# ChanghyeonKim93/bundle_adjustment_solver

Measured on AMD Instinct MI355X. Metric: lm_iterations_per_sec, higher is better.
Workload: dtype f64; 1 GPU; C4 stereo 6-DoF: 1000 poses / 500k landmarks / 5M obs; n_opt_poses=995, n_opt_landmarks=500000, n_observations=5000000, parallelism=single GPU, exchange=none

## Files before the change

bundle_adjustment_solver_amd/_lib.py:

```python
import ctypes as C
import os

_HERE = os.path.dirname(os.path.abspath(__file__))
LIB_PATH = os.environ.get("BA_HIP_LIB") or os.path.join(_HERE, "libba_hip.so")


class BaOptions(C.Structure):
    _fields_ = [
        ("threshold_step_size", C.c_float),
        ("threshold_cost_change", C.c_float),
        ("threshold_huber_loss", C.c_float),
        ("threshold_outlier_rejection", C.c_float),
        ("max_num_iterations", C.c_int),
        ("initial_lambda", C.c_float),
        ("decrease_ratio_lambda", C.c_float),
        ("increase_ratio_lambda", C.c_float),
        ("gauss_newton", C.c_int),
    ]


def make_options(max_iter=50, thr_step=1e-5, thr_cost=1e-5, huber=1.0,
                 outlier=2.0, lambda0=100.0, dec=0.33, inc=3.0,
                 gauss_newton=False):
    o = BaOptions()
# ... 75 lines not shown
    "ba_set_cameras": (C.c_int, [_P, C.c_int, _D, _D]),
    "ba_set_poses": (C.c_int, [_P, C.c_int, _D, _U8]),
    "ba_set_points": (C.c_int, [_P, C.c_int, _D, _U8]),
    "ba_set_observations": (C.c_int, [_P, C.c_int64, _I32, _I32, _I32, _D]),
    "ba_set_shard": (C.c_int, [_P, C.c_int, C.c_int]),
    "ba_finalize": (C.c_int, [_P]),
    "ba_update_values": (C.c_int, [_P, _D, _D]),
    "ba_set_relative": (C.c_int, [_P, C.c_int64, _I32, _I32, _D, _D]),
    "ba_update_relative": (C.c_int, [_P, _D, _D]),
    "ba_relative_check": (C.c_int, [C.c_int, _U8, C.c_int64, _I32, _I32, _D, _D]),
    "ba_relative_info": (C.c_int, [_P, _I64]),
    "ba_partition_points": (C.c_int, [C.c_int, _U8, C.c_int, _U8, C.c_int64,
                                      _I32, _I32, C.c_int, _I32]),
    "ba_set_allreduce": (C.c_int, [_P, ALLREDUCE_FN, _P]),
    "ba_reduce_buffer_size": (C.c_int64, [_P, C.c_int]),
    "ba_bind_reduce_buffer": (C.c_int, [_P, C.c_int, _P, C.c_int64]),
    "ba_gather_points": (C.c_int, [_P]),
    "ba_rccl_available": (C.c_int, []),
    "ba_rccl_get_unique_id": (C.c_int, [_U8]),
    "ba_rccl_comm_create": (C.c_int, [C.POINTER(_P), C.c_int, C.c_int, _U8, C.c_int]),
    "ba_rccl_comm_size": (C.c_int, [_P]),
    "ba_rccl_comm_calls": (C.c_int64, [_P]),
    "ba_rccl_comm_destroy": (None, [_P]),
    "ba_rccl_allreduce_hook": (C.c_int, [_P, C.c_int, _P, C.c_int64, _P]),
    "ba_stream_create": (C.c_int, [C.POINTER(_P), C.c_int, C.c_int, C.c_int64]),
    "ba_stream_destroy": (None, [_P]),
    "ba_stream_set_cameras": (C.c_int, [_P, C.c_int, _D, _D]),
    "ba_stream_set_poses": (C.c_int, [_P, C.c_int, _D, _U8]),
    "ba_stream_set_points": (C.c_int, [_P, C.c_int, _D, _U8]),
    "ba_stream_set_observations": (C.c_int, [_P, C.c_int64, _I32, _I32, _I32, _D]),
    "ba_stream_finalize": (C.c_int, [_P]),
    "ba_stream_solve": (C.c_int, [_P, C.POINTER(BaOptions), C.POINTER(BaIterInfo),
                                  C.c_int, C.POINTER(C.c_int), C.POINTER(C.c_int)]),
    "ba_stream_lm_begin": (C.c_int, [_P, C.POINTER(BaOptions)]),
    "ba_stream_lm_iterate": (C.c_int, [_P, C.c_int]),
    "ba_stream_lm_sync": (C.c_int, [_P, C.POINTER(BaIterInfo), C.c_int,
                                    C.POINTER(C.c_int), C.POINTER(C.c_int)]),
    "ba_stream_get_poses": (C.c_int, [_P, _D]),
    "ba_stream_get_points": (C.c_int, [_P, _D]),
    "ba_stream_info": (C.c_int, [_P, C.POINTER(C.c_int64)]),
    "ba_solve": (C.c_int, [_P, C.POINTER(BaOptions), C.POINTER(BaIterInfo),
                           C.c_int, C.POINTER(C.c_int), C.POINTER(C.c_int)]),
    "ba_lm_begin": (C.c_int, [_P, C.POINTER(BaOptions)]),
    "ba_lm_iterate": (C.c_int, [_P, C.c_int]),
    "ba_lm_sync": (C.c_int, [_P, C.POINTER(BaIterInfo), C.c_int,
                             C.POINTER(C.c_int), C.POINTER(C.c_int)]),
    "ba_gd_begin": (C.c_int, [_P, C.POINTER(BaOptions)]),
    "ba_gd_iterate": (C.c_int, [_P, C.c_int]),
    "ba_gd_sync": (C.c_int, [_P, C.POINTER(BaIterInfo), C.c_int,
                             C.POINTER(C.c_int), C.POINTER(C.c_int)]),
    "ba_solve_gd": (C.c_int, [_P, C.POINTER(BaOptions), C.POINTER(BaIterInfo),
                              C.c_int, C.POINTER(C.c_int), C.POINTER(C.c_int)]),
    "ba_gd_get_gradient": (C.c_int, [_P, _D, _D]),
    "ba_stage_cost": (C.c_int, [_P, _D]),
    "ba_stage_linearize": (C.c_int, [_P, C.c_double, C.c_double]),
    "ba_stage_schur": (C.c_int, [_P]),
    "ba_stage_solve_reduced": (C.c_int, [_P]),
    "ba_stage_backsub_update": (C.c_int, [_P]),
    "ba_stage_scalars": (C.c_int, [_P, _D, _D, _D, _D]),
    "ba_stage_commit": (C.c_int, [_P, C.c_int]),
    "ba_enable_stage_timing": (C.c_int, [_P, C.c_int]),
    "ba_get_stage_ms": (C.c_int, [_P, _D, C.c_int]),
    "ba_num_opt_poses": (C.c_int, [_P]),
    "ba_num_opt_points": (C.c_int, [_P]),
    "ba_num_pairs": (C.c_int64, [_P]),
    "ba_num_schur_blocks": (C.c_int64, [_P]),
    "ba_num_schur_triples": (C.c_int64, [_P]),
    "ba_get_poses": (C.c_int, [_P, _D]),
    "ba_get_points": (C.c_int, [_P, _D, _U8]),
    "ba_get_A": (C.c_int, [_P, _D, _D]),
    "ba_get_C": (C.c_int, [_P, _D, _D]),
    "ba_get_Cinv": (C.c_int, [_P, _D, _D]),
    "ba_get_pairs": (C.c_int, [_P, _I32, _I32, _D]),
    "ba_expand_pair_slim": (None, [_D, _D, _D, _D]),
    "ba_get_S": (C.c_int, [_P, _D, _D]),
    "ba_get_xy": (C.c_int, [_P, _D, _D]),
    "ba_kernel_count": (C.c_int, []),
    "ba_kernel_name": (C.c_char_p, [C.c_int]),
    "ba_get_kernel_ms": (C.c_int, [_P, _D, C.POINTER(C.c_int64), C.c_int]),
    "ba_get_dense_info": (C.c_int, [_P, _D]),
    "ba_get_schur_info": (C.c_int, [_P, C.POINTER(C.c_int64)]),
    "ba_get_lin_info": (C.c_int, [_P, C.POINTER(C.c_int64)]),
    "ba_get_pair_record_info": (C.c_int, [_P, C.POINTER(C.c_int64)]),
    "ba_get_mask_info": (C.c_int, [_P, C.POINTER(C.c_int64)]),
    "ba_get_dropped_pivots": (C.c_int, [_P, C.POINTER(C.c_int64), C.c_int]),
    "ba_dense_spd_solve": (C.c_int, [_P, C.c_int, _D, _D, _D, _D]),
    "ba_covariance": (C.c_int, [_P, C.c_double, C.c_int, _I32, _D, C.c_int, _I32, _D,
                                C.POINTER(C.c_int64)]),
    "ba_covariance_info": (C.c_int, [_P, C.POINTER(C.c_int64)]),
    "ba_covariance_check": (C.c_int, [C.c_int, C.c_int, C.c_int, C.c_int, _U8, C.c_int, _U8,
                                      C.c_int, _I32, _D, C.c_int, _I32, _D]),
    "ba_pose_only_mono6": (C.c_int, [_P, _F, _F, C.c_int, C.c_float, C.c_float,
                                     C.c_float, C.c_float, _F, _U8,
                                     C.POINTER(BaOptions), C.POINTER(BaPoIter),
                                     C.c_int, C.POINTER(C.c_int),
                                     C.POINTER(C.c_int), _F]),
    "ba_pose_only_stereo6": (C.c_int, [_P, _F, _F, _F, C.c_int, _F, _F, _F, _F,
                                       _U8, _U8, C.POINTER(BaOptions),
                                       C.POINTER(BaPoIter), C.c_int,
                                       C.POINTER(C.c_int), C.POINTER(C.c_int),
                                       _F]),
    "ba_pose_only_mono3": (C.c_int, [_P, _F, _F, C.c_int, C.c_float, C.c_float,
                                     C.c_float, C.c_float, _F, _F, _F, _U8,
                                     C.POINTER(BaOptions), C.POINTER(BaPoIter),
                                     C.c_int, C.POINTER(C.c_int),
                                     C.POINTER(C.c_int), _F]),
    "ba_pose_only_stereo3": (C.c_int, [_P, _F, _F, _F, C.c_int, _F, _F, _F, _F,
                                       _F, _F, _U8, _U8, C.POINTER(BaOptions),
                                       C.POINTER(BaPoIter), C.c_int,
                                       C.POINTER(C.c_int), C.POINTER(C.c_int),
                                       _F]),
    "ba_pose_only_mono6_batch": (C.c_int, [_P, C.c_int, _I32, _F, _F, _F, _F, _U8,
                                           C.POINTER(BaOptions), C.POINTER(BaPoIter),
                                           C.c_int, C.POINTER(BaPoResult), _F]),
    "ba_pose_only_stereo6_batch": (C.c_int, [_P, C.c_int, _I32, _F, _F, _F, _F, _F,
                                             _F, _F, _U8, _U8, C.POINTER(BaOptions),
                                             C.POINTER(BaPoIter), C.c_int,
                                             C.POINTER(BaPoResult), _F]),
    "ba_pose_only_mono6_batch_device": (C.c_int, [_P, C.c_int, _P, _P, _P, _P, _P, _P,
                                                  C.POINTER(BaOptions), _P, C.c_int,
                                                  _P, _P, _P]),
    "ba_pose_only_stereo6_batch_device": (C.c_int, [_P, C.c_int, _P, _P, _P, _P, _P, _P,
                                                    _P, _P, _P, C.POINTER(BaOptions),
                                                    _P, C.c_int, _P, _P, _P]),
    "ba_right_camera_record": (C.c_int, [_F, _F, _F]),
    "ba_pose_only_mono3_batch": (C.c_int, [_P, C.c_int, _I32, _F, _F, _F, _F, _F, _F, _U8,
                                           C.POINTER(BaOptions), C.POINTER(BaPoIter),
                                           C.c_int, C.POINTER(BaPoResult), _F]),
    "ba_pose_only_stereo3_batch": (C.c_int, [_P, C.c_int, _I32, _F, _F, _F, _F, _F, _F,
                                             _F, _F, _F, _U8, _U8, C.POINTER(BaOptions),
                                             C.POINTER(BaPoIter), C.c_int,
                                             C.POINTER(BaPoResult), _F]),
    "ba_pose_only_mono3_batch_device": (C.c_int, [_P, C.c_int, _P, _P, _P, _P, _P, _P, _P,
                                                  C.POINTER(BaOptions), _P, C.c_int,
                                                  _P, _P, _P]),
    "ba_pose_only_stereo3_batch_device": (C.c_int, [_P, C.c_int, _P, _P, _P, _P, _P, _P,
                                                    _P, _P, _P, C.POINTER(BaOptions),
                                                    _P, C.c_int, _P, _P, _P]),
    "ba_planar_record": (C.c_int, [_F, _F, _F, _F, _F, _F]),
    "ba_batch_create": (C.c_int, [C.POINTER(_P), _P, C.c_int, _I32, _I32, _I32, _I64,
                                  _D, _D, _D, _U8, _D, _U8, _I32, _I32, _I32, _D]),
    "ba_batch_destroy": (None, [_P]),
    "ba_batch_solve": (C.c_int, [_P, C.POINTER(BaOptions), C.POINTER(BaIterInfo),
                                 C.c_int, C.POINTER(BaBatchResult)]),
    "ba_batch_covariance": (C.c_int, [_P, C.c_double, _D, _D, C.POINTER(BaBatchCovResult)]),
    "ba_batch_marginalize": (C.c_int, [_P, C.c_double, _U8, _D, _D, _U8,
                                       C.POINTER(BaBatchMargResult)]),
    "ba_batch_marg_layout": (C.c_int, [_P, _U8, _I64, _I64]),
    "ba_batch_marg_plan_problem": (C.c_int, [C.c_int, _U8, _U8, C.c_int, _U8, C.c_int64,
                                             _I32, _I32, _I32, _U8]),
    "ba_batch_set_prior": (C.c_int, [_P, _I32, _I32, _D, _D, _D, _D]),
    "ba_batch_prior_check": (C.c_int, [C.c_int, _I32, _U8, _I32, _I32, _D, _D, _D, _D]),
    "ba_batch_prior_info": (C.c_int, [_P, _I64]),
    "ba_batch_set_relative": (C.c_int, [_P, _I32, _I32, _I32, _D, _D]),
    "ba_batch_relative_check": (C.c_int, [C.c_int, _I32, _U8, _I32, _I32, _I32, _D, _D]),
    "ba_batch_relative_info": (C.c_int, [_P, _I64]),
    "ba_batch_relative_marg_plan": (C.c_int, [_P, _U8, _U8]),
    "ba_batch_update_values": (C.c_int, [_P, _D, _D]),
    "ba_batch_get_poses": (C.c_int, [_P, _D]),
    "ba_batch_get_points": (C.c_int, [_P, _D]),
    "ba_batch_info": (C.c_int, [_P, _I64]),
    "ba_batch_scratch_bytes": (C.c_int, [_P, _I64]),
    "ba_batch_plan_problem": (C.c_int, [C.c_int, _U8, C.c_int, _U8, C.c_int64, _I32,
                                        _I32, _I32, _I32, _U8, _I32, _I32]),
    "ba_point_only": (C.c_int, [_P, C.c_int, _D, _D, C.c_int, _D, C.c_int, _I64, _I32, _I32,
                                _D, _U8, _D, C.POINTER(BaOptions), C.POINTER(BaIterInfo),
# ... 78 lines not shown
```

bundle_adjustment_solver_amd/csrc/ba_api.hip:

```cpp
#include <hip/hip_runtime.h>

#include <algorithm>
#include <chrono>
#include <cmath>
#include <cstdio>
#include <cstdlib>
#include <cstring>
#include <string>
#include <vector>

#include "ba_device_fn.h"
#include "ba_handle.h"
#include "ba_rel_host.h"

namespace {
thread_local std::string g_err;
}
void ba::set_last_error(const std::string &m) { g_err = m; }
int ba::fail(const std::string &m) {
  g_err = m;
  return -1;
}
using ba::fail;
using ba::Mem;
// ... 217 lines not shown
  if (h->upload(Mem::Resident, &d.cams, cams)) return -1;
  std::vector<double> poses((size_t)pl.n_pose * 12);
  for (int p = 0; p < pl.n_pose; ++p)
    std::memcpy(&poses[(size_t)p * 12], &h->pose_T[(size_t)pl.pose_user_of_int[p] * 12],
                12 * sizeof(double));
  if (h->upload(Mem::Resident, &d.poses[0], poses) || h->upload(Mem::Resident, &d.poses[1], poses)) return -1;
  std::vector<double> pts((size_t)pl.n_pt * 3);
  for (int q = 0; q < pl.n_pt; ++q)
    std::memcpy(&pts[(size_t)q * 3], &h->pt_X[(size_t)pl.pt_user_of_int[q] * 3],
                3 * sizeof(double));
  if (h->upload(Mem::ChunkState, &d.pts[0], pts) || h->upload(Mem::ChunkState, &d.pts[1], pts)) return -1;
  return 0;
}

std::vector<int32_t> make_blk_desc(const ba::Plan &pl) {
  std::vector<int32_t> bd((size_t)pl.B * 16, 0);
  for (int64_t bk = 0; bk < pl.B; ++bk) {
    int32_t *r = bd.data() + 16 * bk;
    const int64_t c0 = pl.blk_contrib_ptr[bk], c1 = pl.blk_contrib_ptr[bk + 1];
    r[0] = pl.sblk_j[bk];
    r[1] = pl.sblk_k[bk];
    r[2] = (int32_t)c0;
    r[3] = (int32_t)(c1 - c0);
    r[4] = pl.sblk_tchunk_ptr[bk];
    r[5] = pl.sblk_tchunk_ptr[bk + 1] - pl.sblk_tchunk_ptr[bk];
    for (int t = 0; t < 8; ++t) r[8 + t] = c0 + t < c1 ? pl.contrib_slot[c0 + t] : 0;
  }
  return bd;
}

std::vector<ba::DevProblem::LmChunk> make_lm_chunks(const ba::Plan &pl) {
  std::vector<ba::DevProblem::LmChunk> lc(pl.bchunk_lm.size() - 1);
  for (size_t c = 0; c < lc.size(); ++c) {
    const int l0 = pl.bchunk_lm[c], l1 = pl.bchunk_lm[c + 1];
    lc[c].pb = pl.lm_pair_ptr[l0];
    lc[c].ob = pl.lm_obs_ptr[l0];
    lc[c].l0 = l0;
    lc[c].nl = l1 - l0;
    lc[c].np = (int32_t)(pl.lm_pair_ptr[l1] - pl.lm_pair_ptr[l0]);
    lc[c].no = (int32_t)(pl.lm_obs_ptr[l1] - pl.lm_obs_ptr[l0]);
  }
  return lc;
}

int upload_observation_lists(ba_handle *h) {
  const ba::Plan &pl = h->plan;
  ba::DevProblem &d = h->d;
  static_assert(sizeof(int4) == 16 && sizeof(double2) == 16 && sizeof(int2) == 8, "layout");
  if (h->upload(Mem::ChunkConst, &d.obs_idx, pl.obs_idx.data(), (size_t)pl.n_obs) ||
      h->upload(Mem::ChunkConst, &d.obs_uv, pl.obs_uv.data(), (size_t)pl.n_obs))
    return -1;
  if (!pl.obs_cp.empty() && pl.n_obs > 0 && !h->knobs.run.cost_wide)
    if (h->upload(Mem::ChunkConst, &d.obs_cp, pl.obs_cp.data(), (size_t)pl.n_obs)) return -1;
  if (h->upload(Mem::ChunkConst, &d.pobs_idx, pl.pobs_idx.data(), (size_t)pl.n_pobs) ||
      h->upload(Mem::ChunkConst, &d.pobs_uv, pl.pobs_uv.data(), (size_t)pl.n_pobs) ||
      h->upload(Mem::ChunkConst, &d.lm_obs_ptr, pl.lm_obs_ptr) ||
      h->upload(Mem::ChunkConst, &d.lm_pair_ptr, pl.lm_pair_ptr) ||
      h->upload(Mem::ChunkConst, &d.pair_pose, pl.pair_pose) || h->upload(Mem::ChunkConst, &d.pair_lm, pl.pair_lm) ||
      h->upload(Mem::ChunkConst, &d.achunk_pose, pl.achunk_pose) ||
      h->upload(Mem::ChunkConst, &d.achunk_begin, pl.achunk_begin) ||
      h->upload(Mem::ChunkConst, &d.achunk_end, pl.achunk_end) ||
      h->upload(Mem::ChunkConst, &d.pose_achunk_ptr, pl.pose_achunk_ptr))
    return -1;
  if (h->upload(Mem::Resident, &d.sblk_j, pl.sblk_j) || h->upload(Mem::Resident, &d.diag_blk, pl.diag_blk) ||
      h->upload(Mem::Resident, &d.sblk_k, pl.sblk_k))
    return -1;
  if (pl.contrib_slot.size() >= (size_t)INT32_MAX) return fail("too many slot contributions for int32 indices");
  if (h->upload(Mem::ChunkConst, &d.tri_p, pl.tri_p) || h->upload(Mem::ChunkConst, &d.tri_q, pl.tri_q) ||
      h->upload(Mem::ChunkConst, &d.tchunk_blk, pl.tchunk_blk) ||
      h->upload(Mem::ChunkConst, &d.tchunk_begin, pl.tchunk_begin) ||
      h->upload(Mem::ChunkConst, &d.tchunk_end, pl.tchunk_end) ||
      h->upload(Mem::ChunkConst, &d.sblk_tchunk_ptr, pl.sblk_tchunk_ptr) ||
      h->upload(Mem::ChunkConst, &d.ltri, pl.ltri) || h->upload(Mem::ChunkConst, &d.chunk_sp, pl.chunk_sp) ||
      h->upload(Mem::ChunkConst, &d.sup_lane, pl.sup_lane) ||
      h->upload(Mem::ChunkConst, &d.blk_contrib_ptr, pl.blk_contrib_ptr) ||
      h->upload(Mem::ChunkConst, &d.contrib_slot, pl.contrib_slot) ||
      h->upload(Mem::ChunkConst, &d.blk_desc, make_blk_desc(pl)) ||
      h->upload(Mem::ChunkConst, &d.bchunk_lm, pl.bchunk_lm) ||
      h->upload(Mem::ChunkConst, &d.lm_chunk, make_lm_chunks(pl)))
    return -1;
  return 0;
}

int upload_descriptors_and_groups(ba_handle *h) {
  const ba::Plan &pl = h->plan;
  ba::DevProblem &d = h->d;
  d.n_sup = (int)pl.sup_desc.size();
  d.n_bchunk = (int)pl.bchunk_lm.size() - 1;
  d.n_slot = (int)pl.slot_blk.size();
  static_assert(sizeof(ba::Plan::SupDesc) == sizeof(ba::DevProblem::SupDesc), "desc layout");
  static_assert(sizeof(ba::Plan::ChunkDesc) == sizeof(ba::DevProblem::ChunkDesc), "desc layout");
  static_assert(sizeof(ba::Plan::GrpDesc) == sizeof(ba::DevProblem::GrpDesc) && sizeof(ba::Plan::GrpDesc) == 128,
                "group descriptor layout");
  static_assert(sizeof(ba::Plan::LinDesc) == sizeof(ba::DevProblem::LinDesc) && sizeof(ba::Plan::LinDesc) == 48,
                "group linearisation descriptor layout");
  d.n_grp32 = (int)pl.grp32.size();
  d.n_grp64 = (int)pl.grp64.size();
  d.n_grp128 = (int)pl.grp128.size();
  d.lin_chunk0 = pl.lin_groups ? pl.n_bchunk_grp : 0;
  d.n_lin_desc = (int)pl.lin_desc.size();
  d.n_lin_plain = pl.n_lin_plain;
  d.n_bs_grp = d.n_lin_desc;
  d.n_lm_part = d.n_bs_grp + (d.n_bchunk - d.lin_chunk0 + ba::kBsChunks - 1) / ba::kBsChunks;
  d.n_lin_cost = d.n_bchunk + d.n_lin_desc;
  d.pair_slim = h->knobs.layout.pair_slim && pl.lin_groups && d.n_lin_desc > 0 ? 1 : 0;
  d.P_slim = d.pair_slim ? pl.lm_pair_ptr[pl.M_grp] : 0;
  if (h->upload(Mem::ChunkConst, &d.sup_desc, pl.sup_desc.data(), pl.sup_desc.size()) ||
      h->upload(Mem::ChunkConst, &d.chunk_desc, pl.chunk_desc.data(), pl.chunk_desc.size()) ||
      h->dalloc(Mem::ChunkState, &d.spart2, (size_t)d.n_slot * ba::kSlotStride) ||
      h->upload(Mem::ChunkConst, &d.grp32, pl.grp32.data(), pl.grp32.size()) ||
      h->upload(Mem::ChunkConst, &d.grp64, pl.grp64.data(), pl.grp64.size()) ||
      h->upload(Mem::ChunkConst, &d.grp128, pl.grp128.data(), pl.grp128.size()) ||
      h->upload(Mem::ChunkConst, &d.lin_desc, pl.lin_desc.data(), pl.lin_desc.size()) ||
      h->upload(Mem::ChunkConst, &d.grp_pat, pl.grp_pat.data(), pl.grp_pat.size() / 2) ||
      h->upload(Mem::ChunkConst, &d.pose_gpart_ptr, pl.pose_gpart_ptr) ||
      h->upload(Mem::ChunkConst, &d.pose_gpart, pl.pose_gpart) ||
      h->dalloc(Mem::ChunkState, &d.Apart2, (size_t)pl.n_apart2 * 27) ||
      h->dalloc(Mem::ChunkState, &d.lin_dump, (size_t)ba::kLinDump))
    return -1;
  if (pl.n_apart2 > 0) HIP_TRY(hipMemset(d.Apart2, 0, (size_t)pl.n_apart2 * 27 * sizeof(double)));
  return 0;
}

int alloc_iteration_storage(ba_handle *h) {
  const ba::Plan &pl = h->plan;
  ba::DevProblem &d = h->d;
  for (int k = 0; k < 2; ++k) {
    if (h->dalloc(Mem::ChunkState, &d.Cu[k], (size_t)pl.M * 6) || h->dalloc(Mem::ChunkState, &d.b[k], (size_t)pl.M * 3) ||
        h->dalloc(Mem::ChunkState, &d.W[k], std::max<size_t>(2, (size_t)pl.P * ba::kWStride)) ||
        h->dalloc(Mem::Resident, &d.A[k], (size_t)pl.N * 36) || h->dalloc(Mem::Resident, &d.a[k], (size_t)pl.N * 6))
      return -1;
    HIP_TRY(hipMemset(d.W[k], 0, std::max<size_t>(1, (size_t)pl.P * ba::kWStride) * sizeof(double)));
    HIP_TRY(hipMemset(d.A[k], 0, std::max<size_t>(1, (size_t)pl.N * 36) * sizeof(double)));
    HIP_TRY(hipMemset(d.a[k], 0, std::max<size_t>(1, (size_t)pl.N * 6) * sizeof(double)));
  }
  d.n_obs_lm = pl.M > 0 ? pl.lm_obs_ptr[pl.M] : 0;
  if (h->dalloc(Mem::ChunkState, &d.Cd, (size_t)pl.M * 6) || h->dalloc(Mem::ChunkState, &d.Cinv, (size_t)pl.M * 6) ||
      h->dalloc(Mem::ChunkState, &d.lin_cost_part, (size_t)std::max(1, d.n_lin_cost)) ||
      h->dalloc(Mem::ChunkState, &d.Apart, (size_t)d.n_achunk * 27) ||
      h->dalloc(Mem::ChunkState, &d.spart, (size_t)d.n_tchunk * ba::kSlotStride) ||
      h->dalloc(Mem::ChunkState, &d.y, (size_t)pl.M * 3) ||
      h->dalloc(Mem::ChunkState, &d.lm_part, (size_t)std::max(1, d.n_lm_part) * 2))
    return -1;
  d.log_cap = 4096;
  if (h->dalloc(Mem::Resident, &d.x, (size_t)pl.N * 6 + 64) ||
      h->dalloc(Mem::Resident, &d.cost_part, (size_t)ba::kCostGrid) ||
      h->dalloc(Mem::Resident, &d.pose_part, (size_t)2 + 2 * ba::kPoseGrid) ||
      h->dalloc(Mem::Resident, &d.scal, (size_t)4) || h->dalloc(Mem::Resident, &d.ctrl, (size_t)1) ||
      h->dalloc(Mem::Resident, &d.log, (size_t)d.log_cap))
    return -1;
  HIP_TRY(hipMemset(d.lin_cost_part, 0, (size_t)std::max(1, d.n_lin_cost) * sizeof(double)));
  HIP_TRY(hipMemset(d.x, 0, ((size_t)pl.N * 6 + 64) * sizeof(double)));
  HIP_TRY(hipMemset(d.y, 0, std::max<size_t>(1, (size_t)pl.M * 3) * sizeof(double)));
  HIP_TRY(hipMemset(d.cost_part, 0, ba::kCostGrid * sizeof(double)));
  HIP_TRY(hipMemset(d.lm_part, 0, (size_t)std::max(1, d.n_lm_part) * 2 * sizeof(double)));
  HIP_TRY(hipMemset(d.pose_part, 0, (2 + 2 * ba::kPoseGrid) * sizeof(double)));
  HIP_TRY(hipMemset(d.scal, 0, 4 * sizeof(double)));
  return 0;
}

int alias_dense_owner(ba_handle *h) {
  const ba_handle *o = h->dense_owner;
  ba::DevProblem &d = h->d;
  if (!o->finalized || o->plan.N != h->plan.N || o->plan.B != h->plan.B)
    return fail("ba_finalize: the dense owner belongs to a different problem");
  h->sched = o->sched;
  h->ddev = o->ddev;
  h->pose_col_h = o->pose_col_h;
  d.nb = o->d.nb; d.npad = o->d.npad; d.ld = o->d.ld;
  d.L = o->d.L; d.Ldiag = o->d.Ldiag; d.pose_col = o->d.pose_col; d.col_x = o->d.col_x;
  d.zt_I = o->d.zt_I; d.zt_J = o->d.zt_J; d.n_zt = o->d.n_zt;
  d.x = o->d.x;
  return 0;
}

int build_dense_system(ba_handle *h) {
  const ba::Plan &pl = h->plan;
  ba::DevProblem &d = h->d;
  const ba::DenseKnobs &knobs = h->knobs.dense;
  ba::DenseSchedule cand[2];
  const int orders[2] = {32, 64};
  for (int k = 0; k < 2; ++k) {
    int ncb_k = 0;
    std::vector<uint8_t> adj;
    ba::tile_pattern(pl, ba::dense_poses_per_tile(orders[k]), ncb_k, adj);
    if (knobs.full) std::fill(adj.begin(), adj.end(), 1);
    ba::build_dense_schedule(ncb_k, adj, knobs.natural, orders[k], cand[k], knobs.order);
  }
  const bool stats = h->knobs.plan.stats;
// ... 885 lines not shown
  if (download(buf, h->d.pts[h->hc.cur], (size_t)h->plan.n_pt * 3, h->stream)) return -1;
  if (owned_mask) std::memset(owned_mask, 0, (size_t)h->plan.n_pt_global);
  for (int q = 0; q < h->plan.n_pt; ++q) {
    const int u = h->plan.pt_user_of_int[q];
    std::memcpy(X3 + (size_t)u * 3, &buf[(size_t)q * 3], 3 * sizeof(double));
    if (owned_mask) owned_mask[u] = 1;
  }
  return 0;
}

int ba_get_A(ba_handle *h, double *A36, double *a6) {
  if (!h || !h->finalized) return fail("ba_get_A: not finalized");
  if (use_device(h)) return -1;
  join_side(h);
  if (pull_ctrl(h)) return -1;
  const int lb = h->hc.lcur;
  if (A36) {
    HIP_TRY(hipMemcpy(A36, h->d.A[lb], (size_t)h->plan.N * 36 * sizeof(double), hipMemcpyDeviceToHost));
    const double lp1 = 1.0 + h->hc.lambda;
    for (int j = 0; j < h->plan.N; ++j)
      for (int r = 0; r < 6; ++r) A36[(size_t)j * 36 + r * 7] *= lp1;
  }
  if (a6) HIP_TRY(hipMemcpy(a6, h->d.a[lb], (size_t)h->plan.N * 6 * sizeof(double), hipMemcpyDeviceToHost));
  return 0;
}

static void expand_sym3(const double *s6, double *f9) {
  f9[0] = s6[0]; f9[1] = s6[1]; f9[2] = s6[2];
  f9[3] = s6[1]; f9[4] = s6[3]; f9[5] = s6[4];
  f9[6] = s6[2]; f9[7] = s6[4]; f9[8] = s6[5];
}

static int get_sym_vec(ba_handle *h, const double *dS6, const double *dV3,
                       double *out9, double *out3) {
  const ba::Plan &pl = h->plan;
  std::vector<double> s6, v3;
  if (download(s6, dS6, (size_t)pl.M * 6, h->stream)) return -1;
  if (download(v3, dV3, (size_t)pl.M * 3, h->stream)) return -1;
  for (int i = 0; i < pl.M; ++i) {
    const int g = pl.iopt_of_user[pl.pt_user_of_int[i]];
    if (out9) expand_sym3(&s6[(size_t)i * 6], out9 + (size_t)g * 9);
    if (out3) std::memcpy(out3 + (size_t)g * 3, &v3[(size_t)i * 3], 3 * sizeof(double));
  }
  return 0;
}

int ba_get_C(ba_handle *h, double *C9, double *b3) {
  if (!h || !h->finalized) return fail("ba_get_C: not finalized");
  if (use_device(h)) return -1;
  join_side(h);
  if (pull_ctrl(h)) return -1;
  ba::launch_damp_invert_export(h->d, h->stream);
  return get_sym_vec(h, h->d.Cd, h->d.b[h->hc.lcur], C9, b3);
}

int ba_get_Cinv(ba_handle *h, double *Cinv9, double *Cinvb3) {
  if (!h || !h->finalized) return fail("ba_get_Cinv: not finalized");
  if (use_device(h)) return -1;
  const ba::Plan &pl = h->plan;
  std::vector<double> s6, b3;
  join_side(h);
  if (pull_ctrl(h)) return -1;
  ba::launch_damp_invert_export(h->d, h->stream);
  if (download(s6, h->d.Cinv, (size_t)pl.M * 6, h->stream)) return -1;
  if (download(b3, h->d.b[h->hc.lcur], (size_t)pl.M * 3, h->stream)) return -1;
  for (int i = 0; i < pl.M; ++i) {
    const int g = pl.iopt_of_user[pl.pt_user_of_int[i]];
    const double *ci = &s6[(size_t)i * 6], *b = &b3[(size_t)i * 3];
    if (Cinv9) expand_sym3(ci, Cinv9 + (size_t)g * 9);
    if (Cinvb3) {
      double *o = Cinvb3 + (size_t)g * 3;
      o[0] = ci[0] * b[0] + ci[1] * b[1] + ci[2] * b[2];
      o[1] = ci[1] * b[0] + ci[3] * b[1] + ci[4] * b[2];
      o[2] = ci[2] * b[0] + ci[4] * b[1] + ci[5] * b[2];
    }
  }
  return 0;
}

void ba_expand_pair_slim(const double *rec8, const double *T12, const double *X3, double *k12) {
  ba::pair_from_G(rec8, rec8[6], T12, X3[0], X3[1], X3[2], k12, k12 + 9);
}

int ba_get_pairs(ba_handle *h, int32_t *pair_i, int32_t *pair_j, double *W18) {
  if (!h || !h->finalized) return fail("ba_get_pairs: not finalized");
  if (use_device(h)) return -1;
  const ba::Plan &pl = h->plan;
  auto padded = [&](int64_t p) { return !pl.pair_pad.empty() && pl.pair_pad[p]; };
  {
    int64_t o = 0;
    for (int64_t p = 0; p < pl.P; ++p) {
      if (padded(p)) continue;
      if (pair_i) pair_i[o] = pl.iopt_of_user[pl.pt_user_of_int[pl.pair_lm[p]]];
      if (pair_j) pair_j[o] = pl.pair_pose[p];
      ++o;
    }
  }
  if (W18) {
    if (pull_ctrl(h)) return -1;
    std::vector<double> w12((size_t)pl.P * ba::kWStride);
    if (pl.P > 0)
      HIP_TRY(hipMemcpy(w12.data(), h->d.W[h->hc.lcur], w12.size() * sizeof(double), hipMemcpyDeviceToHost));
    const int64_t P_slim = h->d.P_slim;
    std::vector<double> Th, Xh;
    if (P_slim > 0) {
      Th.resize((size_t)pl.n_pose * 12);
      Xh.resize((size_t)pl.M * 3);
      HIP_TRY(hipMemcpy(Th.data(), h->d.poses[h->hc.cur], Th.size() * sizeof(double), hipMemcpyDeviceToHost));
      HIP_TRY(hipMemcpy(Xh.data(), h->d.pts[h->hc.cur], Xh.size() * sizeof(double), hipMemcpyDeviceToHost));
    }
    int64_t o = 0;
    for (int64_t p = 0; p < pl.P; ++p) {
      if (padded(p)) continue;
      double k12[12];
      const double *k = &w12[(size_t)p * ba::kWStride];
      if (p < P_slim) {
        ba_expand_pair_slim(&w12[(size_t)p * ba::kWSlim], &Th[(size_t)pl.pair_pose[p] * 12], &Xh[(size_t)pl.pair_lm[p] * 3], k12);
        k = k12;
      }
      double *W = W18 + (size_t)o * 18;
      for (int e = 0; e < 9; ++e) W[e] = k[e];
      for (int c = 0; c < 3; ++c) {
        W[9 + c] = k[10] * k[6 + c] - k[11] * k[3 + c];
        W[12 + c] = k[11] * k[c] - k[9] * k[6 + c];
        W[15 + c] = k[9] * k[3 + c] - k[10] * k[c];
      }
      ++o;
    }
  }
  return 0;
}

int ba_get_S(ba_handle *h, double *S, double *rhs) {
  if (!h || !h->finalized) return fail("ba_get_S: not finalized");
  if (use_device(h)) return -1;
  const ba::DevProblem &d = h->d;
  const int n6 = 6 * h->plan.N;
  std::vector<double> L;
  ba::launch_scatter(d, h->stream);
  if (download(L, d.L, (size_t)d.npad * d.ld, h->stream)) return -1;
  auto colof = [&](int e) { return h->pose_col_h[e / 6] + e % 6; };
  for (int c = 0; c < n6; ++c) {
    for (int r = c; r < n6; ++r) {
      int rr = colof(r), cc = colof(c);
      if (rr < cc) std::swap(rr, cc);
      const double v = L[(size_t)cc * d.ld + rr];
      if (S) {
        S[(size_t)r * n6 + c] = v;
        S[(size_t)c * n6 + r] = v;
      }
    }
    if (rhs) rhs[c] = L[(size_t)colof(c) * d.ld + d.npad];
  }
  return 0;
}

int ba_get_xy(ba_handle *h, double *x6, double *y3) {
  if (!h || !h->finalized) return fail("ba_get_xy: not finalized");
  if (use_device(h)) return -1;
  const ba::Plan &pl = h->plan;
  HIP_TRY(hipStreamSynchronize(h->stream));
  if (x6 && pl.N > 0)
    HIP_TRY(hipMemcpy(x6, h->d.x, (size_t)pl.N * 6 * sizeof(double), hipMemcpyDeviceToHost));
  if (y3) {
    std::vector<double> y;
    if (download(y, h->d.y, (size_t)pl.M * 3, h->stream)) return -1;
    for (int i = 0; i < pl.M; ++i) {
      const int g = pl.iopt_of_user[pl.pt_user_of_int[i]];
      std::memcpy(y3 + (size_t)g * 3, &y[(size_t)i * 3], 3 * sizeof(double));
    }
  }
  return 0;
}

int ba_kernel_count(void) { return ba::K_COUNT; }

const char *ba_kernel_name(int id) {
  static const char *names[ba::K_COUNT] = {
      "k_cost", "k_lin_landmarks", "k_lin_poses", "k_pose_finalize", "k_dense_init",
      "k_schur_lds", "k_schur_partial", "k_schur_final", "k_scatter",
      "k_chol_diag", "k_chol_trsm", "k_chol_update", "k_chol_back", "k_chol_diag_trsm", "k_chol_tail", "k_backsub_update",
      "k_pose_update", "k_scalars", "k_control", "k_damp_invert", "k_schur_grp", "k_lin_grp",
      "k_rel_lin", "k_rel_gather", "k_rel_offdiag",
// ... 194 lines not shown
  out4[0] = bw;
  out4[1] = ba::kCovGroupCols;
  out4[2] = (int64_t)h->d.npad * bw * (int64_t)sizeof(double);
  out4[3] = h->cov_batches;
  return 0;
}

int ba_covariance(ba_handle *h, double huber, int n_pose_sel, const int32_t *pose_sel, double *cov_pose36,
                  int n_pt_sel, const int32_t *pt_sel, double *cov_pt9, int64_t *dropped_pivots) {
  if (!h) return fail("ba_covariance: null handle");
  if (ba_covariance_check(h->finalized, h->world > 1 || h->ar_fn != nullptr,
                          h->arena != nullptr || h->dense_owner != nullptr, h->n_pose,
                          h->pose_fixed.data(), h->n_pt, h->pt_fixed.data(), n_pose_sel, pose_sel,
                          cov_pose36, n_pt_sel, pt_sel, cov_pt9))
    return -1;
  if (use_device(h)) return -1;
  const ba::Plan &pl = h->plan;
  const ba::DevProblem &d = h->d;
  const ba::DenseSchedule &sc = h->sched;
  const int nb = d.nb, ncb = sc.ncb;
  struct Item {
    int t0, key, idx;
  };
  auto distinct = [](std::vector<Item> &v) {
    std::sort(v.begin(), v.end(), [](const Item &a, const Item &b) {
      return a.t0 != b.t0 ? a.t0 < b.t0 : a.key != b.key ? a.key < b.key : a.idx < b.idx;
    });
    v.erase(std::unique(v.begin(), v.end(), [](const Item &a, const Item &b) { return a.idx == b.idx; }), v.end());
  };
  std::vector<Item> poses, pts;
  for (int s = 0; s < n_pose_sel; ++s) {
    const int j = pl.jopt_of_user[pose_sel[s]];
    poses.push_back({h->pose_col_h[j] / nb, h->pose_col_h[j], j});
  }
  for (int s = 0; s < n_pt_sel; ++s) {
    const int i = pl.pt_int_of_user[pt_sel[s]];
    if (i < 0 || i >= pl.M) return fail("ba_covariance: pt_sel[" + std::to_string(s) + "] is not an optimisable point of this handle");
    int t0 = ncb;
    for (int64_t p = pl.lm_pair_ptr[i]; p < pl.lm_pair_ptr[i + 1]; ++p)
      t0 = std::min(t0, h->pose_col_h[pl.pair_pose[p]] / nb);
    pts.push_back({t0, i, i});
  }
  distinct(poses);
  distinct(pts);
  std::vector<int> slot_pose(pl.N, -1), slot_pt(pl.M, -1);
  std::vector<ba::CovGroup> groups;
  auto make_groups = [&](const std::vector<Item> &v, int kind, int per, std::vector<int> &slot) {
    for (size_t k = 0; k < v.size(); k += per) {
      ba::CovGroup g{};
      g.kind = kind;
      g.n = (int)std::min<size_t>(per, v.size() - k);
      g.t0 = v[k].t0;
      for (int a = 0; a < g.n; ++a) {
        g.item[a] = v[k + a].idx;
        g.slot[a] = slot[v[k + a].idx] = (int)(k + a);
      }
      groups.push_back(g);
    }
  };
  make_groups(poses, 0, 2, slot_pose);
  make_groups(pts, 1, 5, slot_pt);
  std::vector<int> trow_ptr((size_t)ncb + 1, 0), trow;
  {
    std::vector<std::vector<int>> by_row((size_t)ncb);
    for (int p = 0; p < ncb; ++p)
      for (int a = sc.row_ptr[p]; a < sc.row_ptr[p + 1]; ++a)
        if (sc.rows[a] < ncb) by_row[sc.rows[a]].push_back(p);
    for (int t = 0; t < ncb; ++t) {
      trow.insert(trow.end(), by_row[t].begin(), by_row[t].end());
      trow_ptr[t + 1] = (int)trow.size();
    }
  }
  join_side(h);
  if (pull_ctrl(h)) return -1;
  const ba::DevCtrl keep = h->hc;
  h->hc.done = 0;
  h->hc.lambda = 0.0;
  h->hc.huber = huber;
  if (push_ctrl(h)) return -1;
  int bad_keep = 0, bad_now = 0;
  HIP_TRY(hipMemcpy(&bad_keep, h->ddev.bad_pivots, sizeof(int), hipMemcpyDeviceToHost));
  HIP_TRY(hipMemsetAsync(h->ddev.bad_pivots, 0, sizeof(int), h->stream));
  enqueue_linearize(h, 0);
  if (h->rel.F > 0) {
    ba::launch_rel_lin(d, h->rel, 0, 1, h->stream);
    ba::launch_rel_gather(d, h->rel, 0, 1, h->stream);
  }
  ba::launch_damp_invert_export(d, h->stream);
  ba::launch_schur(d, false, true, h->stream);
  if (h->rel.F > 0) ba::launch_rel_offdiag(d, h->rel, false, h->stream);
  ba::launch_scatter(d, h->stream);
  {
    const ba::DenseDev &dd = h->ddev;
    ba::dense_factor_solve(d.L, d.npad, d.ld, d.Ldiag, d.x, &d.ctrl->done, sc, dd,
                           ba::dense_launch_plan_no_tail(sc, h->knobs.dense, dd.flow_ok, dd.plan[1], h->knobs.cone.want), h->stream);
  }
  HIP_TRY(hipStreamSynchronize(h->stream));
  HIP_TRY(hipMemcpy(&bad_now, h->ddev.bad_pivots, sizeof(int), hipMemcpyDeviceToHost));
  HIP_TRY(hipMemcpy(h->ddev.bad_pivots, &bad_keep, sizeof(int), hipMemcpyHostToDevice));
  h->hc = keep;
  if (push_ctrl(h)) return -1;
  ba::ScratchAllocs scratch(h);
  const int bw_max = cov_batch_cols(d.npad, h->knobs.run);
  const int gpb = bw_max / ba::kCovGroupCols;
  const int bw = (int)std::min<size_t>(gpb, std::max<size_t>(1, groups.size())) * ba::kCovGroupCols;
  int *d_trow_ptr = nullptr, *d_trow = nullptr;
  ba::CovGroup *d_groups = nullptr;
  double *Zw = nullptr, *d_pose = nullptr, *d_pt = nullptr;
  if (h->upload(Mem::Resident, &d_trow_ptr, trow_ptr) || h->upload(Mem::Resident, &d_trow, trow) ||
      h->upload(Mem::Resident, &d_groups, groups) ||
      h->dalloc(Mem::Resident, &Zw, (size_t)d.npad * bw) || h->dalloc(Mem::Resident, &d_pose, poses.size() * 36) ||
      h->dalloc(Mem::Resident, &d_pt, pts.size() * 9))
    return -1;
  h->cov_batches = 0;
  for (size_t g0 = 0; g0 < groups.size(); g0 += gpb) {
    const int ng = (int)std::min<size_t>(gpb, groups.size() - g0);
    ba::launch_cov_batch(d, keep.lcur, keep.cur, ncb, d_trow_ptr, d_trow, d_groups + g0, ng, Zw, bw, d_pose, d_pt, h->stream);
    ++h->cov_batches;
  }
  std::vector<double> hp, hq;
  if (download(hp, d_pose, poses.size() * 36, h->stream) || download(hq, d_pt, pts.size() * 9, h->stream)) return -1;
  HIP_TRY(hipStreamSynchronize(h->stream));
  HIP_TRY(hipGetLastError());
  if (bad_now >= ba::kFlowTimeout) return fail("ba_covariance: a dataflow hand-off of the factorisation timed out");
  for (int s = 0; s < n_pose_sel; ++s)
    std::memcpy(cov_pose36 + (size_t)s * 36, &hp[(size_t)slot_pose[pl.jopt_of_user[pose_sel[s]]] * 36], 36 * sizeof(double));
  for (int s = 0; s < n_pt_sel; ++s)
    std::memcpy(cov_pt9 + (size_t)s * 9, &hq[(size_t)slot_pt[pl.pt_int_of_user[pt_sel[s]]] * 9], 9 * sizeof(double));
  if (dropped_pivots) *dropped_pivots = bad_now;
  return 0;
}

}

namespace {
struct PoLayout {
  size_t X, uv, uvr, camr, T, mask, maskr, gsw, h2d_end, meta, iters, dbg, end;
};
PoLayout po_layout(int n, int icap, bool stereo) {
  auto al = [](size_t v) { return (v + 15) & ~(size_t)15; };
  PoLayout L;
  size_t o = 0;
  L.X = o;      o = al(o + (size_t)n * 3 * sizeof(float));
  L.uv = o;     o = al(o + (size_t)n * 2 * sizeof(float));
  L.uvr = o;    o = al(o + (stereo ? (size_t)n * 2 * sizeof(float) : 0));
  L.camr = o;   o = al(o + 16 * sizeof(float));
  L.T = o;      o = al(o + 12 * sizeof(float));
  L.mask = o;   o = al(o + (size_t)n);
  L.maskr = o;  o = al(o + (stereo ? (size_t)n : 0));
  L.gsw = o;    o = al(o + sizeof(int) * (size_t)ba::pose_only_sync_ints());
  L.h2d_end = o;
  L.meta = o;   o = al(o + 4 * sizeof(int));
  L.iters = o;  o = al(o + (size_t)icap * sizeof(ba::PoIter));
  L.dbg = o;    o = al(o + (size_t)icap * 12 * sizeof(float));
  L.end = o;
  return L;
}

int po_reserve(ba_handle *h, size_t bytes) {
  if (bytes <= h->po_cap) return 0;
  if (h->po_dev) (void)hipFree(h->po_dev);
  if (h->po_host) (void)hipHostFree(h->po_host);
  h->po_dev = h->po_host = nullptr;
  h->po_cap = 0;
  HIP_TRY(hipMalloc((void **)&h->po_dev, bytes));
  HIP_TRY(hipHostMalloc((void **)&h->po_host, bytes, hipHostMallocDefault));
// ... 457 lines not shown
```

bundle_adjustment_solver_amd/csrc/ba_device.h:

```cpp
#ifndef BA_DEVICE_H_
#define BA_DEVICE_H_

#include <hip/hip_runtime.h>
#include <stdint.h>
#include <stdlib.h>

#include <vector>

#include "ba_dense_sched.h"

namespace ba {

struct DevCtrl {
  double lambda;
  double prev_cost;
  double huber;
  double thr_step;
  double thr_cost;
  double dec_ratio;
  double inc_ratio;
  unsigned long long t_last;
  int cur;
  int done;
  int iter;
  int converged;
  int max_iter;
  int gn;
  int lcur;
  int tcur, tlcur;
  int pad_;
};

struct DevIterRec {
  double cost, cost_change, average_reprojection_error, abs_gradient, abs_step,
      damping_term, iter_time_ms;
  int iteration_status, pad_;
  double rho, model_change, trial_cost;
};

constexpr int kWStride = 12;
constexpr int kWSlim = 8;

struct DevProblem {
  int n_cam, n_pose, N, n_pt, M, M_global;
  int64_t n_obs, n_obs_opt, n_obs_global, P, n_pobs, T, B;
  int n_achunk, n_tchunk;
  double *cams;
  double *poses[2];
  double *pts[2];
  int4 *obs_idx;
  double2 *obs_uv;
  int64_t *lm_obs_ptr;
  int64_t *lm_pair_ptr;
  int32_t *pair_pose;
  int32_t *pair_lm;
  int2 *pobs_idx;
  int2 *obs_cp;
  double2 *pobs_uv;
  int32_t *achunk_pose;
  int64_t *achunk_begin, *achunk_end;
  int32_t *pose_achunk_ptr;
  int32_t *sblk_j, *sblk_k;
  int32_t *diag_blk;
  int64_t *tri_p, *tri_q;
  int32_t *tchunk_blk;
  int64_t *tchunk_begin, *tchunk_end;
  int32_t *sblk_tchunk_ptr;
  int n_sup, n_slot;
  struct SupDesc {
    int32_t s0, ns, chunk_begin, chunk_end;
  };
  struct ChunkDesc {
    int64_t p0, tb, sp;
    int32_t l0, nl, np, nt;
  };
  struct GrpDesc {
    int64_t p0;
    int32_t l0, nl, d, s0;
    int32_t pose[20];
    int32_t pad_[6];
  };
  struct LinDesc {
    int64_t p0, o0;
    int32_t l0, nl, d, no;
    int32_t pat0;
    int32_t apart0, cost_idx;
    int32_t pad_;
  };
  LinDesc *lin_desc;
  int n_lin_desc;
  int n_lin_plain;
  GrpDesc *grp32, *grp64, *grp128;
  int n_grp32, n_grp64, n_grp128;
  int2 *grp_pat;
  double *Apart2;
  double *lin_dump;
  int32_t *pose_gpart_ptr, *pose_gpart;
  int lin_chunk0;
  int n_lin_cost;
  int n_bs_grp;
  int n_lm_part;
  int pair_slim;
  int64_t P_slim;
  SupDesc *sup_desc;
  uint32_t *sup_lane;
  ChunkDesc *chunk_desc;
  uint16_t *chunk_sp;
  uint32_t *ltri;
  int64_t *blk_contrib_ptr;
  int32_t *contrib_slot;
  int32_t *blk_desc;
  double *spart2;
  double *Cu[2];
  double *b[2];
  double *W[2];
  double *A[2];
  double *a[2];
  double *Cinv;
  double *Cd;
  double *Apart;
  double *spart;
  double *x;
  double *y;
  double *cost_part;
  double *lin_cost_part;
  int64_t n_obs_lm;
  double *lm_part;
  double *pose_part;
  double *scal;
  DevCtrl *ctrl;
  DevIterRec *log;
  int log_cap;
  double *Spk;
  double *L;
  int npad, ld;
  double *Ldiag;
  int nb;
  int *pose_col;
  int *col_x;
  int32_t *bchunk_lm;
  struct LmChunk {
    int64_t pb, ob;
    int32_t l0, nl, np, no;
  };
  LmChunk *lm_chunk;
  int n_bchunk;
  int *zt_I, *zt_J;
  int n_zt;
};

constexpr int kLinDump = 64 * 4 * 4;
constexpr int kFlowTimeout = 1 << 20;
constexpr int kBsChunks = 4;
constexpr int kCostGrid = 1792;
constexpr int kLmGrid = 1024;
constexpr int kPoseGrid = 16;
constexpr int kGdFixGrid = 1024;
constexpr int kGdChunk = 512;
constexpr int kSlotStride = 42;

enum KernelId {
  K_COST = 0, K_LIN_LANDMARKS, K_LIN_POSES, K_POSE_FINALIZE, K_DENSE_INIT,
  K_SCHUR_LDS, K_SCHUR_PARTIAL, K_SCHUR_FINAL, K_SCATTER,
  K_CHOL_DIAG, K_CHOL_TRSM, K_CHOL_UPDATE, K_CHOL_BACK, K_CHOL_DIAG_TRSM, K_CHOL_TAIL, K_BACKSUB_UPDATE,
  K_POSE_UPDATE, K_SCALARS, K_CONTROL, K_DAMP_INVERT, K_SCHUR_GRP, K_LIN_GRP,
  K_REL_LIN, K_REL_GATHER, K_REL_OFFDIAG,
  K_PG_LIN_ROBUST, K_PG_ASSEMBLE_ROBUST,
  K_PG_LIN, K_PG_ASSEMBLE, K_PG_TRIAL, K_PG_CONTROL, K_COUNT
};
struct KernelTimer {
  bool on = false;
  std::vector<hipEvent_t> pool;
  std::vector<int> ids;
  double ms[K_COUNT] = {0};
  long calls[K_COUNT] = {0};
  void begin(int id, hipStream_t s);
  void end(hipStream_t s);
  void collect();
  void reset();
};
extern thread_local KernelTimer *g_ktimer;
#define BA_LAUNCH(id, kernel, grid, block, stream, ...)                     \
  do {                                                                      \
    if (::ba::g_ktimer && ::ba::g_ktimer->on) ::ba::g_ktimer->begin(id, stream); \
    hipLaunchKernelGGL(kernel, grid, block, 0, stream, __VA_ARGS__);        \
    if (::ba::g_ktimer && ::ba::g_ktimer->on) ::ba::g_ktimer->end(stream);  \
  } while (0)

#define BA_KEEP_S(x) asm volatile("" ::"s"(x))

void launch_cost(const DevProblem &d, int sel, int64_t begin, hipStream_t s);
void launch_lin_poses(const DevProblem &d, int sel, hipStream_t s);
void launch_lin_landmarks(const DevProblem &d, int sel, hipStream_t s);
void launch_damp_invert(const DevProblem &d, hipStream_t s);
void launch_schur(const DevProblem &d, bool direct, bool with_init, hipStream_t s);
void launch_schur_accumulate(const DevProblem &d, hipStream_t s);
void launch_schur_final(const DevProblem &d, bool direct, hipStream_t s);
void launch_backsub_update(const DevProblem &d, hipStream_t s, bool zero_tiles = false);
void launch_scatter(const DevProblem &d, hipStream_t s);
void launch_scalars_cost_only(const DevProblem &d, int cost_src, hipStream_t s);
void launch_scalars(const DevProblem &d, int cost_src, hipStream_t s);
void launch_scalars_and_control(const DevProblem &d, int cost_src, hipStream_t s,
                                int finalize_sel = -1);
void launch_control(const DevProblem &d, hipStream_t s);
void launch_init_ctrl_cost(const DevProblem &d, hipStream_t s);

constexpr int kRelFpb = 64;
constexpr int kRelScrDoubles = 126;
struct RelDev {
  int F;
  int nblk;
  int n_part;
  int pad_;
  const int4 *jk;
  const double *val;
  const int32_t *pptr, *plist;
  const int32_t *blk;
  const int32_t *bptr, *blist;
  double *scr[2];
  double *part;
};
void launch_rel_lin(const DevProblem &d, const RelDev &r, int sel, int mode, hipStream_t s);
void launch_rel_gather(const DevProblem &d, const RelDev &r, int sel, int flags, hipStream_t s);
void launch_rel_offdiag(const DevProblem &d, const RelDev &r, bool direct, hipStream_t s);

struct PgCtrl {
  double lambda;
  double chi2;
  double thr_step, thr_cost, dec_ratio, inc_ratio;
  double aux;
  unsigned long long t_last;
  int cur;
  int done;
  int iter, converged, max_iter, gn;
  int relin;
  int pad_;
};
constexpr int kPgFpb = 64;
constexpr int kPgRec = 84;
constexpr int kPgOr = 0, kPgGk = 6, kPgOA = 12, kPgBk = 48;
struct PgDev {
  int n_pose, N, F, nblk;
  int n_part;
  int n_tpart;
  int npad, ld;
  double *poses[2];
  const int4 *jk;
  const double *val;
  const int32_t *pptr, *plist;
  const int2 *blk;
  const int32_t *bptr, *blist;
  const int32_t *opt_pose;
  const int *pose_col;
  double *rec;
  double *dH, *g;
  double *x;
  double *part[2];
  double *tpart;
  double *L;
  PgCtrl *ctrl;
  DevIterRec *log;
  int log_cap;
};
struct PgRobust {
  const int32_t *kind;
  const double *scale;
  double *s, *w;
};
void launch_pg_lin(const PgDev &p, int cost_only, hipStream_t s);
void launch_pg_lin_robust(const PgDev &p, const PgRobust &rb, int cost_only, hipStream_t s);
void launch_pg_assemble_robust(const PgDev &p, const PgRobust &rb, double *Hout, double *gout, hipStream_t s);
void launch_pg_assemble(const PgDev &p, double *Hout, double *gout, hipStream_t s);
void launch_pg_trial(const PgDev &p, hipStream_t s);
void launch_pg_control(const PgDev &p, int mode, hipStream_t s);

struct GdDev {
  int2 *pobs;
// ... 107 lines not shown
```

bundle_adjustment_solver_amd/csrc/ba_device_fn.h:

```cpp
#ifndef BA_DEVICE_FN_H_
#define BA_DEVICE_FN_H_

#include "ba_device.h"

namespace ba {

template <int CTRL>
__device__ __forceinline__ double dpp_f64(double v) {
  union { double d; int i[2]; } u, r;
  u.d = v;
  r.i[0] = __builtin_amdgcn_update_dpp(0, u.i[0], CTRL, 0xf, 0xf, false);
  r.i[1] = __builtin_amdgcn_update_dpp(0, u.i[1], CTRL, 0xf, 0xf, false);
  return r.d;
}
__device__ __forceinline__ double lane_f64(double v, int src) {
  union { double d; int i[2]; } u;
  u.d = v;
  u.i[0] = __builtin_amdgcn_readlane(u.i[0], src);
  u.i[1] = __builtin_amdgcn_readlane(u.i[1], src);
  return u.d;
}
__device__ __forceinline__ double wave_sum(double v) {
  v += dpp_f64<0xB1>(v);
  v += dpp_f64<0x4E>(v);
// ... 57 lines not shown
    g.Xc[r] = (Rc[r * 3 + 0] * g.Xij[0] + Rc[r * 3 + 1] * g.Xij[1] +
               Rc[r * 3 + 2] * g.Xij[2]) +
              tc[r];
  const double invz = 1.0 / g.Xc[2];
  g.r0 = cam[0] * (g.Xc[0] * invz) + cam[2] - u;
  g.r1 = cam[1] * (g.Xc[1] * invz) + cam[3] - v;
}

__device__ __forceinline__ void weight_and_G(const double *__restrict__ cam,
                                             const ObsGeom &g, double huber,
                                             double &w, double G[6]) {
#pragma clang fp contract(fast)
  const double invz = 1.0 / g.Xc[2];
  const double fxinvz = cam[0] * invz, fyinvz = cam[1] * invz;
  const double xinvz = g.Xc[0] * invz, yinvz = g.Xc[1] * invz;
  const double fx_xinvz2 = fxinvz * xinvz, fy_yinvz2 = fyinvz * yinvz;
  const double absr = fabs(g.r0) + fabs(g.r1);
  w = (absr > huber) ? (huber / absr) : 1.0;
  const double *Rc = cam + 4;
  G[0] = fxinvz * Rc[0] + (-fx_xinvz2) * Rc[6];
  G[1] = fxinvz * Rc[1] + (-fx_xinvz2) * Rc[7];
  G[2] = fxinvz * Rc[2] + (-fx_xinvz2) * Rc[8];
  G[3] = fyinvz * Rc[3] + (-fy_yinvz2) * Rc[6];
  G[4] = fyinvz * Rc[4] + (-fy_yinvz2) * Rc[7];
  G[5] = fyinvz * Rc[5] + (-fy_yinvz2) * Rc[8];
}

__device__ __forceinline__ void make_Q(const double G[6], const double Xij[3],
                                       double Q[12]) {
#pragma clang fp contract(fast)
#pragma unroll
  for (int r = 0; r < 2; ++r) {
    const double g0 = G[r * 3 + 0], g1 = G[r * 3 + 1], g2 = G[r * 3 + 2];
    Q[r * 6 + 0] = g0;
    Q[r * 6 + 1] = g1;
    Q[r * 6 + 2] = g2;
    Q[r * 6 + 3] = g2 * Xij[1] - g1 * Xij[2];
    Q[r * 6 + 4] = g0 * Xij[2] - g2 * Xij[0];
    Q[r * 6 + 5] = g1 * Xij[0] - g0 * Xij[1];
  }
}

__device__ __forceinline__ void make_R(const double G[6],
                                       const double *__restrict__ T,
                                       double Rm[6]) {
#pragma clang fp contract(fast)
#pragma unroll
  for (int r = 0; r < 2; ++r)
#pragma unroll
    for (int c = 0; c < 3; ++c)
      Rm[r * 3 + c] = G[r * 3 + 0] * T[0 * 3 + c] + G[r * 3 + 1] * T[1 * 3 + c] +
                      G[r * 3 + 2] * T[2 * 3 + c];
}

__device__ __forceinline__ void expand_W(const double *__restrict__ k12, double W[18]) {
#pragma unroll
  for (int e = 0; e < 9; ++e) W[e] = k12[e];
  const double X0 = k12[9], X1 = k12[10], X2 = k12[11];
#pragma unroll
  for (int c = 0; c < 3; ++c) {
    W[9 + c] = X1 * k12[6 + c] - X2 * k12[3 + c];
    W[12 + c] = X2 * k12[c] - X0 * k12[6 + c];
    W[15 + c] = X0 * k12[3 + c] - X1 * k12[c];
  }
}

__host__ __device__ __forceinline__ void pair_from_G(const double G[6], const double w, const double *__restrict__ T,
                                                     const double X0, const double X1, const double X2, double K[9],
                                                     double Xij[3]) {
#pragma clang fp contract(off)
#pragma unroll
  for (int r = 0; r < 3; ++r)
    Xij[r] = fma(T[r * 3 + 2], X2, fma(T[r * 3 + 0], X0, T[r * 3 + 1] * X1)) + T[9 + r];
  double wR[6];
#pragma unroll
  for (int m = 0; m < 2; ++m)
#pragma unroll
    for (int c = 0; c < 3; ++c)
      wR[m * 3 + c] = w * fma(G[m * 3 + 2], T[6 + c], fma(G[m * 3 + 0], T[c], G[m * 3 + 1] * T[3 + c]));
#pragma unroll
  for (int r = 0; r < 3; ++r)
#pragma unroll
    for (int c = 0; c < 3; ++c) K[r * 3 + c] = fma(G[r], wR[c], G[3 + r] * wR[3 + c]);
}

__device__ __forceinline__ void ldlt3_inverse(const double c[6], double o[6]) {
  double a00 = c[0], a01 = c[1], a02 = c[2], a11 = c[3], a12 = c[4], a22 = c[5];
  int s0 = 0;
  {
    double m = fabs(a00);
    if (fabs(a11) > m) {
      m = fabs(a11);
      s0 = 1;
    }
    if (fabs(a22) > m) s0 = 2;
  }
  double t;
  if (s0 == 1) {
    t = a00; a00 = a11; a11 = t;
    t = a02; a02 = a12; a12 = t;
  } else if (s0 == 2) {
    t = a00; a00 = a22; a22 = t;
    t = a01; a01 = a12; a12 = t;
  }
  const bool s1 = fabs(a22) > fabs(a11);
  if (s1) {
    t = a11; a11 = a22; a22 = t;
    t = a01; a01 = a02; a02 = t;
  }
  double b00 = 0, b01 = 0, b02 = 0, b11 = 0, b12 = 0, b22 = 0;
  const double d0 = a00;
  if (fabs(d0) > 0.0) {
    const double l10 = a01 / d0, l20 = a02 / d0;
    const double tmp0 = d0 * l10;
    const double d1 = a11 - l10 * tmp0;
    double l21 = a12 - l20 * tmp0;
    if (fabs(d1) > 0.0) l21 /= d1;
    const double d2 = a22 - (l20 * (d0 * l20) + l21 * (d1 * l21));
    const double tol = 2.2250738585072014e-308;
    const double i0 = (fabs(d0) > tol) ? 1.0 / d0 : 0.0;
    const double i1 = (fabs(d1) > tol) ? 1.0 / d1 : 0.0;
    const double i2 = (fabs(d2) > tol) ? 1.0 / d2 : 0.0;
    {
      const double z0 = 1.0, z1 = -l10 * z0, z2 = -l20 * z0 - l21 * z1;
      const double w0 = z0 * i0, w1 = z1 * i1, w2 = z2 * i2;
      const double x2 = w2, x1 = w1 - l21 * x2, x0 = w0 - l10 * x1 - l20 * x2;
      b00 = x0;
      (void)x1;
      (void)x2;
    }
    {
      const double z1 = 1.0, z2 = -l21 * z1;
      const double w1 = z1 * i1, w2 = z2 * i2;
      const double x2 = w2, x1 = w1 - l21 * x2, x0 = -l10 * x1 - l20 * x2;
      b01 = x0;
      b11 = x1;
    }
    {
      const double w2 = i2;
      const double x2 = w2, x1 = -l21 * x2, x0 = -l10 * x1 - l20 * x2;
      b02 = x0;
      b12 = x1;
      b22 = x2;
    }
  }
  if (s1) {
    t = b11; b11 = b22; b22 = t;
    t = b01; b01 = b02; b02 = t;
  }
  if (s0 == 1) {
    t = b00; b00 = b11; b11 = t;
    t = b02; b02 = b12; b12 = t;
  } else if (s0 == 2) {
    t = b00; b00 = b22; b22 = t;
    t = b01; b01 = b12; b12 = t;
  }
  o[0] = b00; o[1] = b01; o[2] = b02; o[3] = b11; o[4] = b12; o[5] = b22;
}

__device__ __forceinline__ double rcp_newton(double d) {
  double r = __builtin_amdgcn_rcp(d);
  r = fma(fma(-d, r, 1.0), r, r);
  r = fma(fma(-d, r, 1.0), r, r);
  return r;
}
__device__ __forceinline__ void spd3_inverse(const double c[6], double o[6]) {
// ... 155 lines not shown
```

bundle_adjustment_solver_amd/csrc/ba_kernels.hip:

```cpp
#include "ba_device.h"
#include "ba_device_fn.h"
#include "ba_plan.h"

#if defined(__HIP_DEVICE_COMPILE__) && !defined(__gfx950__) && !defined(__gfx942__) && !defined(__gfx90a__)
#error "ba_kernels.hip relies on gfx9-family behaviour (LDS-only barriers): build for gfx950"
#endif

namespace ba {

thread_local KernelTimer *g_ktimer = nullptr;

void KernelTimer::begin(int id, hipStream_t s) {
  const size_t k = ids.size();
  while (pool.size() < 2 * (k + 1)) {
    hipEvent_t e;
    if (hipEventCreate(&e) != hipSuccess) return;
    pool.push_back(e);
  }
  ids.push_back(id);
  (void)hipEventRecord(pool[2 * k], s);
}
void KernelTimer::end(hipStream_t s) {
  if (ids.empty()) return;
  (void)hipEventRecord(pool[2 * (ids.size() - 1) + 1], s);
// ... 230 lines not shown
      }
    }
    LL_STAMP()
    __syncthreads();
    LL_STAMP()
    {
      const int o0 = (int)(t0 - ob);
#pragma unroll
      for (int k = 0; k < kSumIt; ++k) {
        const int t = tid + k * kBlock;
        if (t < lc.nl * 9) {
          const int li = t / 9, v = t - li * 9;
          const int a = max(lq[li], o0), b = min(lq[li + 1], o0 + kBlock);
          double sacc = 0.0;
          const double *cp = Cb + (a - o0) * 9 + v;
          int n = b - a;
          for (; n >= 4; n -= 4, cp += 36) {
            const double v0 = cp[0], v1 = cp[9], v2 = cp[18], v3 = cp[27];
            sacc = (((sacc + v0) + v1) + v2) + v3;
          }
          for (; n > 0; --n, cp += 9) sacc += cp[0];
          csum[k] += sacc;
        }
      }
    }
    LL_STAMP()
    __syncthreads();
    LL_STAMP()
  }
#pragma unroll
  for (int k = 0; k < kSumIt; ++k) {
    const int t = tid + k * kBlock;
    if (t < lc.nl * 9) Cb[t] = csum[k];
  }
  __syncthreads();
  double c00 = 0, c01 = 0, c02 = 0, c11 = 0, c12 = 0, c22 = 0;
  double b0 = 0, b1 = 0, b2 = 0;
  if (own) {
    const double *cs = Cb + tid * 9;
    c00 = cs[0]; c01 = cs[1]; c02 = cs[2];
    c11 = cs[3]; c12 = cs[4]; c22 = cs[5];
    b0 = -cs[6]; b1 = -cs[7]; b2 = -cs[8];
  }
  {
    const int n2 = min(npair, kSchurPairs) * (kWStride / 2);
    const double2 *src = (const double2 *)Wst;
    double2 *dst = (double2 *)(Wg + (size_t)pb * kWStride);
    constexpr int kIt = (kSchurPairs * (kWStride / 2) + kBlock - 1) / kBlock;
    double2 wv[kIt];
#pragma unroll
    for (int k = 0; k < kIt; ++k) {
      const int t = tid + k * kBlock;
      wv[k] = src[t < n2 ? t : 0];
    }
#pragma unroll
    for (int k = 0; k < kIt; ++k) {
      const int t = tid + k * kBlock;
      if (t < n2) dst[t] = wv[k];
    }
  }
  LL_STAMP()
#ifdef BA_LL_DBG
  if (ll_on) { for (int q = 0; q < 32; ++q) g_ll_dbg[q] = q < ll_n ? ll_s[q] : 0; }
#endif
  {
    const double tot = block_sum(cost_acc, smc);
    if (tid == 0) d.lin_cost_part[chunk] = tot;
  }
  if (!own) return;
  double *Co = d.Cu[lb] + (size_t)i * 6;
  Co[0] = c00; Co[1] = c01; Co[2] = c02; Co[3] = c11; Co[4] = c12; Co[5] = c22;
  double *bo = d.b[lb] + (size_t)i * 3;
  bo[0] = b0;
  bo[1] = b1;
  bo[2] = b2;
}

#ifdef BA_LG_DBG
__device__ long long g_lg_dbg[64];
#define LG_STAMP() { if (lg_on && lg_n < 64) lg_s[lg_n++] = clock64(); }
#else
#define LG_STAMP()
#endif
template <bool SLIM>
constexpr int kLgArea = 64 * 9 + 7 * 10 * (SLIM ? kWSlim : kWStride);
template <bool LDSCAM, bool MASKED, bool SLIM>
__device__ __forceinline__ void lin_grp_body(const DevProblem &d, const int sel, const int bid, double *red,
                                             double *cams_s, double *smc, int *slot_b, int *slot_e) {
#ifdef BA_LG_DBG
  __shared__ long long lg_s[64];
  const bool lg_on = blockIdx.x == 300 && threadIdx.x == 0;
  int lg_n = 0;
#endif
  LG_STAMP()
  const DevProblem::LinDesc *gp = d.lin_desc + bid;
  const int64_t p0 = gp->p0, o0 = gp->o0;
  const int l0 = gp->l0, nl = gp->nl, dd = gp->d, no = gp->no, pat0 = gp->pat0;
  const int apart0 = gp->apart0, cost_idx = gp->cost_idx;
  const int done = d.ctrl->done;
  const int buf = sel ? d.ctrl->tcur : d.ctrl->cur;
  const int lb = sel ? d.ctrl->tlcur : d.ctrl->lcur;
  const double huber = d.ctrl->huber;
  if (LDSCAM) stage_cams(d, cams_s);
  const int tid = threadIdx.x, lane = tid & 63;
  const int wv = __builtin_amdgcn_readfirstlane(tid >> 6);
  const int nlw = 64 / no < 7 ? 64 / no : 7;
  const int ilw = lane / no, oo = lane - ilw * no;
  const bool lane_on = ilw < nlw;
  const int2 pat = d.grp_pat[pat0 + oo];
  if (done) return;
  const int cam_id = pat.y & 0xffff, jj = (pat.y >> 16) & 0xff;
  const bool opt = (pat.y >> 29) & 1, lastw = (pat.y >> 30) & 1;
  {
    const int pose_prev = __shfl_up(pat.x, 1), pose_next = __shfl_down(pat.x, 1);
    if (tid < no && opt) {
      if (oo == 0 || pose_prev != pat.x) slot_b[jj] = oo;
      if (oo == no - 1 || pose_next != pat.x) slot_e[jj] = oo + 1;
    }
  }
  const double *__restrict__ pts = d.pts[buf];
#define LING_LDX(p_) (*(p_))
  double T[12], cam[16];
  {
    const double *Tp = d.poses[buf] + (size_t)pat.x * 12;
#pragma unroll
    for (int k = 0; k < 12; ++k)
      T[k] = Tp[k];
  }
  __syncthreads();
  load_cam<LDSCAM>(d, cams_s, cam_id, cam);
  unsigned later_bits = 0u, pose_bits = 0u;
  if (MASKED && opt) {
    const int sb_l = slot_b[jj], se_l = slot_e[jj];
    const unsigned upto_e = se_l >= 32 ? 0xffffffffu : ((1u << se_l) - 1u);
    pose_bits = upto_e & ~((1u << sb_l) - 1u);
    later_bits = oo + 1 >= 32 ? 0u : (upto_e & ~((1u << (oo + 1)) - 1u));
  }
  double *__restrict__ Wg = d.W[lb];
  double *__restrict__ Cg = d.Cu[lb];
  double *__restrict__ bg = d.b[lb];
  double *cbw = red + wv * kLgArea<SLIM>;
  double acc[27];
#pragma unroll
  for (int k = 0; k < 27; ++k) acc[k] = 0.0;
  double cost_acc = 0.0;
  const int per_step = 4 * nlw;
  const int nstep = (nl + per_step - 1) / per_step;
  auto il_of = [&](int st) { return (st * 4 + wv) * nlw + ilw; };
  auto clampi = [&](int il) { return min(il, nl - 1); };
  double2 uvq[3];
  double Xq[3][3];
#pragma unroll
  for (int u = 0; u < 2; ++u) {
    const int ilc = clampi(il_of(u));
    uvq[u] = d.obs_uv[o0 + (int64_t)ilc * no + oo];
    const double *Xp = pts + (size_t)(l0 + ilc) * 3;
    Xq[u][0] = LING_LDX(&Xp[0]);
    Xq[u][1] = LING_LDX(&Xp[1]);
    Xq[u][2] = LING_LDX(&Xp[2]);
  }
  const int sum_li = lane / 9, sum_v = lane - sum_li * 9;
  const bool sum_on = lane < nlw * 9, sum_neg = sum_v >= 6;
  const double *sum_p = cbw + (sum_on ? sum_li * no * 9 + sum_v : 0);
  double *sum_g = sum_v < 6 ? Cg + (size_t)l0 * 6 + sum_v : bg + (size_t)l0 * 3 + (sum_v - 6);
  const int sum_stride = sum_v < 6 ? 6 : 3;
  double2 *dumpW = (double2 *)(d.lin_dump + (size_t)((bid & 63) * 4 + wv) * 4);
  double *dumpC = (double *)dumpW + 2;
  constexpr int RW = (SLIM ? kWSlim : kWStride) / 2;
  double2 *stgW = (double2 *)(cbw + 64 * 9);
  double2 *stgW_mine = stgW + (ilw * dd + jj) * RW;
  constexpr int kLgPass = (7 * 10 * RW + 63) / 64;
  int il0p = nl;
  double vv[8];
  double2 wvv[kLgPass];
  int lastp = 0;
  double2 *dstWp = dumpW;
#define LING_FLUSH_ISSUE()                                                          \
  {                                                                                 \
    _Pragma("unroll") for (int u_ = 0; u_ < 8; ++u_) vv[u_] = sum_p[(u_ < no ? u_ : 0) * 9]; \
    const int nls_ = nl - il0p < nlw ? nl - il0p : nlw;                             \
    const int n2_ = nls_ * dd * RW;                                                 \
    dstWp = n2_ > 0 ? (double2 *)(Wg + (size_t)(p0 + (int64_t)il0p * dd) * (2 * RW)) : dumpW; \
    lastp = n2_ > 0 ? n2_ - 1 : 0;                                                  \
    _Pragma("unroll") for (int k_ = 0; k_ < kLgPass; ++k_) wvv[k_] = stgW[min(lane + 64 * k_, lastp)]; \
  }
#define LING_FLUSH_FINISH()                                                         \
  {                                                                                 \
    double sacc_ = 0.0;                                                             \
    _Pragma("unroll") for (int u_ = 0; u_ < 8; ++u_) sacc_ += (u_ < no) ? vv[u_] : 0.0; \
    for (int q_ = 8; q_ < no; ++q_) sacc_ += sum_p[q_ * 9];                         \
    const int ils_ = il0p + sum_li;                                                 \
    double *dst_ = (sum_on && ils_ < nl) ? sum_g + (size_t)ils_ * sum_stride : dumpC; \
    *dst_ = sum_neg ? -sacc_ : sacc_;                                               \
    _Pragma("unroll") for (int k_ = 0; k_ < kLgPass; ++k_) dstWp[min(lane + 64 * k_, lastp)] = wvv[k_]; \
  }
#define LING_STEP(CUR, NXT2)                                                        \
  {                                                                                 \
    _Pragma("clang fp contract(fast)")                                              \
    LG_STAMP()                                                                      \
    LING_FLUSH_ISSUE()                                                              \
    {                                                                               \
      const int ilc_ = clampi(il_of(st + 2));                                       \
      uvq[NXT2] = d.obs_uv[o0 + (int64_t)ilc_ * no + oo];                           \
      const double *Xp_ = pts + (size_t)(l0 + ilc_) * 3;                            \
      Xq[NXT2][0] = LING_LDX(&Xp_[0]);                                              \
      Xq[NXT2][1] = LING_LDX(&Xp_[1]);                                              \
      Xq[NXT2][2] = LING_LDX(&Xp_[2]);                                              \
    }                                                                               \
    const int il0_ = (st * 4 + wv) * nlw;                                           \
    const int il_ = il0_ + ilw;                                                     \
    const bool valid_ = lane_on && il_ < nl && (!MASKED || uvq[CUR].x == uvq[CUR].x); \
    bool wr_ = lastw;                                                               \
    if (MASKED) {                                                                   \
      const unsigned long long vb_ = __ballot(valid_);                              \
      const unsigned mine_ = (unsigned)(vb_ >> (lane - oo));                        \
      wr_ = opt && (valid_ ? (mine_ & later_bits) == 0u : (lastw && (mine_ & pose_bits) == 0u)); \
    }                                                                               \
    ObsGeom g;                                                                      \
    project(cam, T, Xq[CUR][0], Xq[CUR][1], Xq[CUR][2], uvq[CUR].x, uvq[CUR].y, g); \
    if (MASKED) {                                                                   \
      g.r0 = valid_ ? g.r0 : 0.0;                                                   \
      g.r1 = valid_ ? g.r1 : 0.0;                                                   \
    }                                                                               \
    cost_acc += valid_ ? sqrt(g.r0 * g.r0 + g.r1 * g.r1) : 0.0;                     \
    double w, G[6], Rm[6], Q[12], cbv[9], kk[12];                                   \
    weight_and_G(cam, g, huber, w, G);                                              \
    w = valid_ ? w : 0.0;                                                           \
    make_R(G, T, Rm);                                                               \
    {                                                                               \
                      \
      double wR[6];                                                                 \
      _Pragma("unroll") for (int e_ = 0; e_ < 6; ++e_) wR[e_] = w * Rm[e_];         \
      cbv[0] = Rm[0] * wR[0] + Rm[3] * wR[3];                                       \
      cbv[1] = Rm[0] * wR[1] + Rm[3] * wR[4];                                       \
      cbv[2] = Rm[0] * wR[2] + Rm[3] * wR[5];                                       \
      cbv[3] = Rm[1] * wR[1] + Rm[4] * wR[4];                                       \
      cbv[4] = Rm[1] * wR[2] + Rm[4] * wR[5];                                       \
      cbv[5] = Rm[2] * wR[2] + Rm[5] * wR[5];                                       \
      cbv[6] = wR[0] * g.r0 + wR[3] * g.r1;                                         \
      cbv[7] = wR[1] * g.r0 + wR[4] * g.r1;                                         \
      cbv[8] = wR[2] * g.r0 + wR[5] * g.r1;                                         \
       \
       \
       \
      if (SLIM) {                                                                   \
        _Pragma("unroll") for (int e_ = 0; e_ < 6; ++e_) kk[e_] = (!MASKED || valid_) ? G[e_] : 0.0; \
        kk[6] = w;                                                                  \
        kk[7] = 0.0;                                                                \
      } else {                                                                      \
        _Pragma("unroll") for (int r = 0; r < 3; ++r)                               \
        _Pragma("unroll") for (int c = 0; c < 3; ++c)                               \
          kk[r * 3 + c] = G[r] * wR[c] + G[3 + r] * wR[3 + c];                      \
        _Pragma("unroll") for (int r = 0; r < 3; ++r) kk[9 + r] = g.Xij[r];         \
      }                                                                             \
    }                                                                               \
    {                                                                               \
             \
      const double wq = opt ? w : 0.0;                                              \
      make_Q(G, g.Xij, Q);                                                          \
      int k = 0;                                                                    \
      _Pragma("unroll") for (int r = 0; r < 6; ++r) {                               \
        const double q0 = wq * Q[r], q1 = wq * Q[6 + r];                            \
        _Pragma("unroll") for (int c = r; c < 6; ++c)                               \
          { acc[k] = fma(q0, Q[c], fma(q1, Q[6 + c], acc[k])); ++k; }               \
      }                                                                             \
      const double ar0 = wq * g.r0, ar1 = wq * g.r1;                                \
      _Pragma("unroll") for (int c = 0; c < 6; ++c)                                 \
        acc[21 + c] = fma(Q[c], ar0, fma(Q[6 + c], ar1, acc[21 + c]));              \
    }                                                                               \
    LG_STAMP()                                                                      \
    LING_FLUSH_FINISH()                                                             \
    LG_STAMP()                                                                      \
                           \
    __builtin_amdgcn_fence(__ATOMIC_RELEASE, "wavefront");                          \
    __builtin_amdgcn_wave_barrier();                                                \
    __builtin_amdgcn_fence(__ATOMIC_ACQUIRE, "wavefront");                          \
    {                                                                               \
      double *cb = cbw + lane * 9;                                                  \
      _Pragma("unroll") for (int e_ = 0; e_ < 9; ++e_) cb[e_] = cbv[e_];            \
      if (wr_ && lane_on) {                                                         \
        _Pragma("unroll") for (int r = 0; r < RW; ++r)                              \
          stgW_mine[r] = make_double2(kk[2 * r], kk[2 * r + 1]);                    \
      }                                                                             \
    }                                                                               \
    il0p = il0_;                                                                    \
    __builtin_amdgcn_fence(__ATOMIC_RELEASE, "wavefront");                          \
    __builtin_amdgcn_wave_barrier();                                                \
    __builtin_amdgcn_fence(__ATOMIC_ACQUIRE, "wavefront");                          \
  }
  int st = 0;
  while (st < nstep) {
    LING_STEP(0, 2)
    if (++st >= nstep) break;
    LING_STEP(1, 0)
    if (++st >= nstep) break;
    LING_STEP(2, 1)
    ++st;
  }
  LING_FLUSH_ISSUE()
  LING_FLUSH_FINISH()
#undef LING_STEP
#undef LING_LDX
#undef LING_FLUSH_ISSUE
#undef LING_FLUSH_FINISH
  LG_STAMP()
  {
    const double tot = block_sum(cost_acc, smc);
    if (tid == 0) d.lin_cost_part[cost_idx] = tot;
  }
#pragma unroll
  for (int half = 0; half < 2; ++half) {
    __syncthreads();
#pragma unroll
    for (int k = 0; k < 14; ++k)
      if (half * 14 + k < 27) cbw[k * 64 + lane] = acc[half * 14 + k];
    __syncthreads();
    for (int t = tid; t < dd * 14; t += kBlock) {
      const int pj = t / 14, k = t - pj * 14, e = half * 14 + k;
      if (e >= 27) continue;
      const int sb = slot_b[pj], se = slot_e[pj];
      double sacc = 0.0;
      for (int w4 = 0; w4 < 4; ++w4)
        for (int li = 0; li < nlw; ++li)
          for (int q = sb; q < se; ++q) sacc += red[w4 * kLgArea<SLIM> + k * 64 + li * no + q];
      d.Apart2[(size_t)(apart0 + pj) * 27 + e] = sacc;
    }
  }
  LG_STAMP()
#ifdef BA_LG_DBG
  if (lg_on) { for (int q = 0; q < 64; ++q) g_lg_dbg[q] = q < lg_n ? lg_s[q] : 0; }
#endif
}

template <bool LDSCAM, bool MASKED, bool SLIM>
__global__ __launch_bounds__(kBlock, 2) void k_lin_grp(DevProblem d, int sel, int piece0) {
  __shared__ __attribute__((aligned(16))) double red[4 * kLgArea<SLIM>];
  __shared__ double cams_s[kCamLds * 16];
  __shared__ double smc[4];
  __shared__ int slot_b[kGrpMaxPoses], slot_e[kGrpMaxPoses];
  lin_grp_body<LDSCAM, MASKED, SLIM>(d, sel, piece0 + blockIdx.x, red, cams_s, smc, slot_b, slot_e);
}

__global__ __launch_bounds__(kBlock) void k_damp_invert(DevProblem d, int store_cd) {
  const int i = blockIdx.x * kBlock + threadIdx.x;
  const int ic = i < d.M ? i : 0;
  const double lp1 = 1.0 + d.ctrl->lambda;
  const int lb = d.ctrl->lcur;
  const int done = d.ctrl->done;
  const double *c = d.Cu[lb] + (size_t)ic * 6;
  double cd[6];
#pragma unroll
  for (int k = 0; k < 6; ++k) cd[k] = c[k];
  if (done || i >= d.M) return;
  cd[0] *= lp1;
  cd[3] *= lp1;
  cd[5] *= lp1;
  double ci[6];
  spd3_inverse(cd, ci);
  double *Io = d.Cinv + (size_t)i * 6;
#pragma unroll
  for (int k = 0; k < 6; ++k) Io[k] = ci[k];
  if (store_cd) {
    double *Do = d.Cd + (size_t)i * 6;
#pragma unroll
    for (int k = 0; k < 6; ++k) Do[k] = cd[k];
  }
}

#define LINP_STEP(XC, XN)                                                       \
  {                                                                             \
    const double *Xp_ = pts + (size_t)idn.y * 3;                                \
    _Pragma("unroll") for (int k_ = 0; k_ < 3; ++k_) XN[k_] = Xp_[k_];          \
    const int ncam_ = idn.x;                                                    \
    const double2 nuv_ = uvn;                                                   \
    {                                                                           \
      const int64_t s2_ = s + 128 < e ? s + 128 : e - 1;                        \
      idn = d.pobs_idx[s2_];                                                    \
      uvn = d.pobs_uv[s2_];                                                     \
    }                                                                           \
    double cam_[16];                                                            \
    load_cam<LDSCAM>(d, cams_s, ccam, cam_);                                    \
    ObsGeom g;                                                                  \
    project(cam_, Tl, XC[0], XC[1], XC[2], cuv.x, cuv.y, g);                    \
    double w, G[6], Q[12];                                                      \
    weight_and_G(cam_, g, huber, w, G);                                         \
    make_Q(G, g.Xij, Q);                                                        \
                                                        \
    int k = 0;                                                                  \
    _Pragma("unroll") for (int r = 0; r < 6; ++r)                               \
    _Pragma("unroll") for (int c = r; c < 6; ++c)                               \
      { acc[k] = fma(w * Q[r], Q[c], fma(w * Q[6 + r], Q[6 + c], acc[k])); ++k; } \
    const double wr0 = w * g.r0, wr1 = w * g.r1;                                \
    _Pragma("unroll") for (int c = 0; c < 6; ++c)                               \
      acc[21 + c] = fma(Q[c], wr0, fma(Q[6 + c], wr1, acc[21 + c]));            \
    ccam = ncam_;                                                               \
    cuv = nuv_;                                                                 \
  }

template <bool LDSCAM>
__global__ __launch_bounds__(kBlock) void k_lin_poses(DevProblem d, int sel) {
  __shared__ double cams_s[kCamLds * 16];
  if (LDSCAM) stage_cams(d, cams_s);
  const int lane = threadIdx.x & 63;
  const int ch = __builtin_amdgcn_readfirstlane(blockIdx.x * (kBlock / 64) + (threadIdx.x >> 6));
  const bool live = ch < d.n_achunk;
  const int chc = live ? ch : 0;
  const int64_t b = d.achunk_begin[chc], e = d.achunk_end[chc];
  const int j = d.achunk_pose[chc];
  const int done = d.ctrl->done;
  const int buf = sel ? d.ctrl->tcur : d.ctrl->cur;
  const double huber = d.ctrl->huber;
  BA_KEEP_S(__builtin_amdgcn_readfirstlane((int)b));
  BA_KEEP_S(__builtin_amdgcn_readfirstlane(j));
  BA_KEEP_S(done);
  __syncthreads();
  if (done || !live || b >= e) {
    if (!done && live) {
      for (int k = lane; k < 27; k += 64) d.Apart[(size_t)ch * 27 + k] = 0.0;
    }
    return;
  }
  const double *__restrict__ pts = d.pts[buf];
  const double *T = d.poses[buf] + (size_t)j * 12;
// ... 239 lines not shown
    }
    DBG_STAMP()
    __syncthreads();
    DBG_STAMP()
    if (owner) {
      const int t1 = (int)Sp[slot + 1];
      int t = (int)Sp[slot] + sub2;
      uint32_t pq = Ts[t < kSchurTri ? t : kSchurTri - 1];
      while (t < t1) {
        const int tn = t + tps2;
        const uint32_t pqn = Ts[tn < kSchurTri ? tn : kSchurTri - 1];
        __builtin_amdgcn_sched_barrier(0);
        const uint32_t pp = pq >> 16, qq = pq & 0xffu;
        const double *vp = Vs + pp * 18 + h * 9;
        const double2 *wp = (const double2 *)(Ws + qq * kWLds);
        const double *bp = Bs + ((pq >> 8) & 0xffu) * 3;
        const double bm = (pp == qq) ? 1.0 : 0.0;
        const double b0 = bp[0] * bm, b1 = bp[1] * bm, b2 = bp[2] * bm;
        double w[12];
#pragma unroll
        for (int k = 0; k < 6; ++k) {
          const double2 b2 = wp[k];
          w[2 * k] = b2.x;
          w[2 * k + 1] = b2.y;
        }
        const double X0 = w[9], X1 = w[10], X2 = w[11];
#pragma unroll
        for (int r = 0; r < 3; ++r) {
          const double v0 = vp[r * 3 + 0], v1 = vp[r * 3 + 1], v2 = vp[r * 3 + 2];
          const double t0 = fma(v2, w[2], fma(v1, w[1], v0 * w[0]));
          const double t1 = fma(v2, w[5], fma(v1, w[4], v0 * w[3]));
          const double t2 = fma(v2, w[8], fma(v1, w[7], v0 * w[6]));
          acc[r * 6 + 0] += t0;
          acc[r * 6 + 1] += t1;
          acc[r * 6 + 2] += t2;
          acc[r * 6 + 3] = fma(-X2, t1, fma(X1, t2, acc[r * 6 + 3]));
          acc[r * 6 + 4] = fma(-X0, t2, fma(X2, t0, acc[r * 6 + 4]));
          acc[r * 6 + 5] = fma(-X1, t0, fma(X0, t1, acc[r * 6 + 5]));
          racc[r] = fma(v2, b2, fma(v1, b1, fma(v0, b0, racc[r])));
        }
        pq = pqn;
        t = tn;
      }
    }
    DBG_STAMP()
    __syncthreads();
    DBG_STAMP()
  }
  DBG_STAMP()
#pragma unroll
  for (int k = 0; k < 21; ++k) {
    double a2 = k < 18 ? acc[k] : racc[k - 18];
    int w = tps2;
#pragma unroll
    for (int off = 8; off >= 1; off >>= 1) {
      const double o2 = __shfl_down(a2, 2 * off, 64);
      if (sub2 + off < w) a2 += o2;
      w = w < off ? w : off;
    }
    if (k < 18) acc[k] = a2; else racc[k - 18] = a2;
  }
#ifdef BA_SCHUR_DBG
  if (dbg_on)
    for (int k = 0; k < 160; ++k) g_schur_dbg[dbg_slot][k] = k < dbg_n ? dbg_s[k] : 0;
#endif
  if (owner && sub2 == 0) {
    double *o = d.spart2 + (size_t)(sd.s0 + slot) * kSlotStride;
#pragma unroll
    for (int k = 0; k < 18; ++k) o[h * 18 + k] = acc[k];
#pragma unroll
    for (int k = 0; k < 3; ++k) o[36 + h * 3 + k] = racc[k];
  }
}

#ifndef BA_GRP_KRW
#define BA_GRP_KRW 36
#endif
#ifdef BA_GRP_DBG
__device__ long long g_grp_dbg[256];
#define GRP_STAMP() { if (gdbg_on && gdbg_n < 256) gdbg_s[gdbg_n++] = clock64(); }
#else
#define GRP_STAMP()
#endif
template <int NT, bool SLIM>
__global__ __launch_bounds__(kBlock, (NT == 2 && BA_GRP_KRW <= 24) ? 3 : 2) void k_schur_grp(DevProblem d, const DevProblem::GrpDesc *grps) {
  constexpr int TW = 16 * NT;
#ifndef BA_GRP_KRW
#define BA_GRP_KRW 36
#endif
  constexpr int KRW = NT == 2 ? BA_GRP_KRW : 20;
  constexpr int NTILE = NT * (NT + 1) / 2;
  constexpr int RS = 2 * TW + (NT == 2 ? 6 : 0);
  constexpr int IMG = (KRW / 2) * RS;
  __shared__ __attribute__((aligned(16))) double VA[4][IMG];
  __shared__ __attribute__((aligned(16))) double WB[4][IMG];
  static_assert(IMG >= 256, "the final reduction uses VA as 4 x 256 doubles");
#ifdef BA_GRP_DBG
  __shared__ long long gdbg_s[256];
  const bool gdbg_on = blockIdx.x == 600 && threadIdx.x == 0;
  int gdbg_n = 0;
#endif
  const int tid = threadIdx.x, lane = tid & 63, wv = tid >> 6;
  const int lr = lane & 15, lk = lane >> 4;
  const DevProblem::GrpDesc gd = grps[blockIdx.x];
  const int done = d.ctrl->done;
  const int lb = d.ctrl->lcur;
  BA_KEEP_S(gd.l0);
  BA_KEEP_S(done);
  if (done) return;
  const double *__restrict__ Wg = d.W[lb];
  const double *__restrict__ bg = d.b[lb];
  const double *__restrict__ Cug = d.Cu[lb];
  const double lp1 = 1.0 + d.ctrl->lambda;
  const int dd = gd.d;
  const int nlw = min(64 / dd, KRW / 3);
  const int il = lane / dd, jj = lane - il * dd;
  const int nch = (gd.nl + nlw - 1) / nlw;
  double *va = VA[wv], *wb = WB[wv];
  for (int e = lane; e < IMG; e += 64) {
    va[e] = 0.0;
    wb[e] = 0.0;
  }
  constexpr int RD = (SLIM && NT == 4) ? 1 : 2;
  constexpr int RW = (SLIM ? kWSlim : kWStride) / 2;
  double2 rw[2][6], rc[2][3];
  double rb[2][3], rx[2][3];
  double T[12];
  const double *__restrict__ ptg = d.pts[d.ctrl->cur];
  if (SLIM) {
    const double *Tp = d.poses[d.ctrl->cur] + (size_t)grps[blockIdx.x].pose[jj] * 12;
#pragma unroll
    for (int k = 0; k < 12; ++k) T[k] = Tp[k];
  }
#define GRP_PREFETCH(B, ch_)                                                        \
  {                                                                                 \
    const int c0_ = (ch_) * nlw;                                                    \
    const bool on_ = il < min(nlw, gd.nl - c0_);                                    \
    const double2 *wp_ = (const double2 *)(Wg + (size_t)(gd.p0 + (int64_t)c0_ * dd + (on_ ? lane : 0)) * (2 * RW)); \
    const int lm_ = gd.l0 + c0_ + (on_ ? il : 0);                                   \
    const double2 *cp_ = (const double2 *)(Cug + (size_t)lm_ * 6);                  \
    _Pragma("unroll") for (int k_ = 0; k_ < RW; ++k_) rw[B][k_] = wp_[k_];          \
    _Pragma("unroll") for (int k_ = 0; k_ < 3; ++k_) rc[B][k_] = cp_[k_];           \
    _Pragma("unroll") for (int k_ = 0; k_ < 3; ++k_) rb[B][k_] = bg[(size_t)lm_ * 3 + k_]; \
    if (SLIM) {                                                                     \
      _Pragma("unroll") for (int k_ = 0; k_ < 3; ++k_) rx[B][k_] = ptg[(size_t)lm_ * 3 + k_]; \
    }                                                                               \
  }
  v4f64 acc[NTILE];
#pragma unroll
  for (int t = 0; t < NTILE; ++t) acc[t] = (v4f64){0.0, 0.0, 0.0, 0.0};
  if (wv < nch) GRP_PREFETCH(0, wv)
  if (RD == 2 && wv + 4 < nch) GRP_PREFETCH(1, wv + 4)
#define GRP_IDX(k_, col_) (((k_) >> 1) * RS + (col_) * 2 + ((k_) & 1))
#define GRP_STAGE(B)                                                                \
  if (ch < nch) {                                                                   \
    GRP_STAMP()                                                                     \
    const int nlc = min(nlw, gd.nl - ch * nlw);                                     \
    if (il < nlc) {                                                                 \
       \
      _Pragma("clang fp contract(fast)")                                            \
      double k9[9], xij[3];                                                         \
      if (SLIM) {                                                                   \
        const double G_[6] = {rw[B][0].x, rw[B][0].y, rw[B][1].x, rw[B][1].y, rw[B][2].x, rw[B][2].y}; \
        pair_from_G(G_, rw[B][3].x, T, rx[B][0], rx[B][1], rx[B][2], k9, xij);      \
      } else {                                                                      \
        k9[0] = rw[B][0].x; k9[1] = rw[B][0].y; k9[2] = rw[B][1].x; k9[3] = rw[B][1].y; k9[4] = rw[B][2].x; \
        k9[5] = rw[B][2].y; k9[6] = rw[B][3].x; k9[7] = rw[B][3].y; k9[8] = rw[B][4].x; \
        xij[0] = rw[B][4].y; xij[1] = rw[B][5].x; xij[2] = rw[B][5].y;              \
      }                                                                             \
      const double x0 = xij[0], x1 = xij[1], x2 = xij[2];                           \
          \
      const double cd_[6] = {rc[B][0].x * lp1, rc[B][0].y, rc[B][1].x, rc[B][1].y * lp1, rc[B][2].x, rc[B][2].y * lp1}; \
      double c6[6];                                                                 \
      spd3_inverse(cd_, c6);                                                        \
      double w[18];                                                                 \
      _Pragma("unroll") for (int e = 0; e < 9; ++e) w[e] = k9[e];                   \
      _Pragma("unroll") for (int c = 0; c < 3; ++c) {                               \
        w[9 + c] = x1 * k9[6 + c] - x2 * k9[3 + c];                                 \
        w[12 + c] = x2 * k9[c] - x0 * k9[6 + c];                                    \
        w[15 + c] = x0 * k9[3 + c] - x1 * k9[c];                                    \
      }                                                                             \
      const int kb = 3 * il, cb = 6 * jj;                                           \
      const int i0 = GRP_IDX(kb, cb), i1 = GRP_IDX(kb + 1, cb), i2 = GRP_IDX(kb + 2, cb); \
      _Pragma("unroll") for (int r = 0; r < 6; ++r) {                               \
        const double w0 = w[r * 3], w1 = w[r * 3 + 1], w2 = w[r * 3 + 2];           \
        va[i0 + 2 * r] = w0 * c6[0] + w1 * c6[1] + w2 * c6[2];                      \
        va[i1 + 2 * r] = w0 * c6[1] + w1 * c6[3] + w2 * c6[4];                      \
        va[i2 + 2 * r] = w0 * c6[2] + w1 * c6[4] + w2 * c6[5];                      \
        wb[i0 + 2 * r] = w0;                                                        \
        wb[i1 + 2 * r] = w1;                                                        \
        wb[i2 + 2 * r] = w2;                                                        \
      }                                                                             \
      if (jj == 0) {                           \
        wb[GRP_IDX(kb, 6 * dd)] = rb[B][0];                                         \
        wb[GRP_IDX(kb + 1, 6 * dd)] = rb[B][1];                                     \
        wb[GRP_IDX(kb + 2, 6 * dd)] = rb[B][2];                                     \
      }                                                                             \
    }                                                                               \
    const int nks = (3 * nlc + 3) >> 2;                                             \
    if (nlc < nlw) {  \
      for (int e = lane; e < (4 * nks - 3 * nlc) * TW; e += 64) {                   \
        const int k_ = 3 * nlc + e / TW, c_ = e - (e / TW) * TW;                    \
        va[GRP_IDX(k_, c_)] = 0.0;                                                  \
        wb[GRP_IDX(k_, c_)] = 0.0;                                                  \
      }                                                                             \
    }                                                                               \
    GRP_STAMP()                                                                     \
    if (ch + 4 * RD < nch) GRP_PREFETCH(B, ch + 4 * RD)                             \
    GRP_STAMP()                                                                     \
    __builtin_amdgcn_fence(__ATOMIC_RELEASE, "wavefront");                          \
    __builtin_amdgcn_wave_barrier();                                                \
    __builtin_amdgcn_fence(__ATOMIC_ACQUIRE, "wavefront");                          \
    {                                                                               \
       \
      const double *ap = va + (lk >> 1) * RS + lr * 2 + (lk & 1);                   \
      const double *bp = wb + (lk >> 1) * RS + lr * 2 + (lk & 1);                   \
      double a[NT], b[NT], an[NT], bn[NT];                                          \
      _Pragma("unroll") for (int t = 0; t < NT; ++t) {                              \
        a[t] = ap[32 * t];                                                          \
        b[t] = bp[32 * t];                                                          \
      }                                                                             \
      for (int ks = 0; ks < nks; ++ks) {                                            \
        const int kn = ks + 1 < nks ? ks + 1 : ks;  \
        _Pragma("unroll") for (int t = 0; t < NT; ++t) {                            \
          an[t] = ap[kn * 2 * RS + 32 * t];                                         \
          bn[t] = bp[kn * 2 * RS + 32 * t];                                         \
        }                                                                           \
        int tile = 0;                                                               \
        _Pragma("unroll") for (int ti = 0; ti < NT; ++ti)                           \
        _Pragma("unroll") for (int tj = ti; tj < NT; ++tj) {                        \
          acc[tile] = __builtin_amdgcn_mfma_f64_16x16x4f64(a[ti], b[tj], acc[tile], 0, 0, 0); \
          ++tile;                                                                   \
        }                                                                           \
        _Pragma("unroll") for (int t = 0; t < NT; ++t) {                            \
          a[t] = an[t];                                                             \
          b[t] = bn[t];                                                             \
        }                                                                           \
      }                                                                             \
    }                                                                               \
    __builtin_amdgcn_fence(__ATOMIC_RELEASE, "wavefront");                          \
    __builtin_amdgcn_wave_barrier();                                                \
    __builtin_amdgcn_fence(__ATOMIC_ACQUIRE, "wavefront");                          \
    GRP_STAMP()                                                                     \
    ch += 4;                                                                        \
  }
// ... 557 lines not shown
        const int npn = r_np < kSchurPairs ? r_np : kSchurPairs;
        BACKSUB_ISSUE(r_pb, npn)
      }
      BS_STAMP()
      __syncthreads();
      BS_STAMP()
      for (int t = tid; t < np * 3; t += kBlock) {
        const int lp = t / 3, c = t - lp * 3;
        const double *xj = Xs + lp * 6;
        const double *w = Ws + lp * kWStride;
        const double X0 = w[9], X1 = w[10], X2 = w[11];
        const double e0 = xj[0] + (xj[4] * X2 - xj[5] * X1);
        const double e1 = xj[1] + (xj[5] * X0 - xj[3] * X2);
        const double e2 = xj[2] + (xj[3] * X1 - xj[4] * X0);
        Us[t] = fma(w[6 + c], e2, fma(w[3 + c], e1, w[c] * e0));
      }
      BS_STAMP()
      __syncthreads();
      BS_STAMP()
      if (own) {
        const int64_t a = max(q0, t0), b = min(q1, t0 + np);
        for (int64_t p = a; p < b; ++p) {
          const double *u = Us + (p - t0) * 3;
          bx0 += u[0];
          bx1 += u[1];
          bx2 += u[2];
        }
      }
      BS_STAMP()
      if (last_tile) break;
      t0 += kSchurPairs;
      np = (int)min((int64_t)kSchurPairs, pe - t0);
      __syncthreads();
      BACKSUB_ISSUE(t0, np)
      BACKSUB_GATHER(np)
    }
    if (k + 1 < nk) {
      const int npn = r_np < kSchurPairs ? r_np : kSchurPairs;
      BACKSUB_GATHER(npn)
    }
    double est = 0.0, nrm = 0.0;
    if (own) {
      {
        const double cdm[6] = {C[0] * lp1, C[1], C[2], C[3] * lp1, C[4], C[5] * lp1};
        ldlt3_inverse(cdm, ci);
      }
      const double cb0 = ci[0] * bi[0] + ci[1] * bi[1] + ci[2] * bi[2];
      const double cb1 = ci[1] * bi[0] + ci[3] * bi[1] + ci[4] * bi[2];
      const double cb2 = ci[2] * bi[0] + ci[4] * bi[1] + ci[5] * bi[2];
      const double y0 = cb0 - (ci[0] * bx0 + ci[1] * bx1 + ci[2] * bx2);
      const double y1 = cb1 - (ci[1] * bx0 + ci[3] * bx1 + ci[4] * bx2);
      const double y2 = cb2 - (ci[2] * bx0 + ci[4] * bx1 + ci[5] * bx2);
      double *yo = d.y + (size_t)i * 3;
      yo[0] = y0; yo[1] = y1; yo[2] = y2;
      double *Xo = Xt + (size_t)i * 3;
      Xo[0] = Xi[0] + y0;
      Xo[1] = Xi[1] + y1;
      Xo[2] = Xi[2] + y2;
      const double C0 = C[0] * lp1, C3 = C[3] * lp1, C5 = C[5] * lp1;
      double e = bi[0] * y0 + bi[1] * y1 + bi[2] * y2;
      const double r0 = y0 * C0 + y1 * C[1] + y2 * C[2];
      const double r1 = y0 * C[1] + y1 * C3 + y2 * C[4];
      const double r2 = y0 * C[2] + y1 * C[4] + y2 * C5;
      e += r0 * y0 + r1 * y1 + r2 * y2;
      e += 2.0 * (y0 * bx0 + y1 * bx1 + y2 * bx2);
      est = e;
      nrm = sqrt(y0 * y0 + y1 * y1 + y2 * y2);
    }
    BS_STAMP()
    est_acc += est;
    nrm_acc += nrm;
  }
  block_sum2(est_acc, nrm_acc, sm);
  if (tid == 0) {
    d.lm_part[2 * part + 0] = est_acc;
    d.lm_part[2 * part + 1] = nrm_acc;
  }
  BS_STAMP()
#ifdef BA_BS_DBG
  if (bs_on) for (int q = 0; q < 96; ++q) g_bs_dbg[q] = q < bs_n ? bs_s[q] : 0;
#endif
}

template <bool SLIM>
__device__ __forceinline__ void backsub_grp_body(const DevProblem &d, const int piece, const int part, double *lds,
                                                 double *sm) {
  const DevProblem::LinDesc *gp = d.lin_desc + piece;
  const int64_t p0 = gp->p0;
  const int l0 = gp->l0, nl = gp->nl, dd = gp->d;
  const int done = d.ctrl->done;
  const int cur = d.ctrl->cur;
  const int lbs = d.ctrl->lcur;
  const double lp1 = 1.0 + d.ctrl->lambda;
  const int tid = threadIdx.x, lane = tid & 63, wv = tid >> 6;
  const int ddv = dd > 0 ? dd : 1;
  const int nlwb = 64 / ddv < kBgLm ? 64 / ddv : kBgLm;
  const int ilw = lane / ddv, jj = lane - ilw * ddv;
  const bool lane_on = dd > 0 && ilw < nlwb;
  const int pose = dd > 0 ? d.pair_pose[p0 + jj] : 0;
  if (done) return;
  double xj[6];
  {
    const double2 *xp = (const double2 *)(d.x + (size_t)pose * 6);
    const double2 a0 = xp[0], a1 = xp[1], a2 = xp[2];
    xj[0] = a0.x; xj[1] = a0.y; xj[2] = a1.x; xj[3] = a1.y; xj[4] = a2.x; xj[5] = a2.y;
  }
  double *__restrict__ Xt = d.pts[cur ^ 1];
  const double2 *__restrict__ Wg2 = (const double2 *)d.W[lbs];
  constexpr int RW = (SLIM ? kWSlim : kWStride) / 2;
  double T[12];
  if (SLIM) {
    const double *Tp = d.poses[cur] + (size_t)pose * 12;
#pragma unroll
    for (int k = 0; k < 12; ++k) T[k] = Tp[k];
  }
  double *Wim = lds + wv * kBgArea;
  double *Us = Wim + 64 * 2 * RW;
  double *Lm = Us + 64 * 3;
  double *Bx = Lm + 64 * 12;
  const int S = 64 / nlwb;
  const int per_step = 4 * nlwb;
  const int nstep = (nl + per_step - 1) / per_step;
  auto il0_of = [&](int st) { return (st * 4 + wv) * nlwb; };
  const double *lm_p[3];
  int lm_l[3], lm_e[3], lm_m[3], lm_q[3];
#pragma unroll
  for (int k = 0; k < 3; ++k) {
    const int q = min(lane + 64 * k, nlwb * 12 - 1);
    const int nc = nlwb * 6, nb = nlwb * 9;
    const int a = q < nc ? 0 : (q < nb ? 1 : 2);
    const int r = q - (a == 0 ? 0 : (a == 1 ? nc : nb));
    lm_m[k] = a == 0 ? 6 : 3;
    lm_l[k] = r / lm_m[k];
    lm_e[k] = r - lm_l[k] * lm_m[k];
    lm_p[k] = (a == 0 ? d.Cu[lbs] : (a == 1 ? d.b[lbs] : d.pts[cur])) + (size_t)l0 * lm_m[k] + lm_e[k];
    lm_q[k] = q;
  }
  double2 rwA0, rwA1, rwA2, rwA3, rwA4, rwA5, rwB0, rwB1, rwB2, rwB3, rwB4, rwB5;
  double lmA0, lmA1, lmA2, lmB0, lmB1, lmB2;
#define BSG_ISSUE(R, L, ST)                                                         \
  {                                                                                 \
    const int il0_ = il0_of(ST);                                                    \
    const int nls_ = max(0, min(nlwb, nl - il0_));                                  \
    const int last_ = max(0, nls_ * dd * RW - 1);                                   \
    const int ilb_ = nls_ > 0 ? il0_ : 0;                                           \
    const int lml_ = max(0, nls_ - 1);                                              \
    const double2 *src_ = Wg2 + (dd > 0 ? (size_t)(p0 + (int64_t)ilb_ * dd) * RW : (size_t)0); \
    R##0 = src_[min(lane, last_)];                                                  \
    R##1 = src_[min(lane + 64, last_)];                                             \
    R##2 = src_[min(lane + 128, last_)];                                            \
    R##3 = src_[min(lane + 192, last_)];                                            \
    if (!SLIM) {                                                                    \
      R##4 = src_[min(lane + 256, last_)];                                          \
      R##5 = src_[min(lane + 320, last_)];                                          \
    }                                                                               \
    L##0 = lm_p[0][(size_t)(ilb_ + min(lm_l[0], lml_)) * lm_m[0]];                  \
    L##1 = lm_p[1][(size_t)(ilb_ + min(lm_l[1], lml_)) * lm_m[1]];                  \
    L##2 = lm_p[2][(size_t)(ilb_ + min(lm_l[2], lml_)) * lm_m[2]];                  \
  }
#define BSG_WAVE_SYNC()                                                             \
  {                                                                                 \
    __builtin_amdgcn_fence(__ATOMIC_RELEASE, "wavefront");                          \
    __builtin_amdgcn_wave_barrier();                                                \
    __builtin_amdgcn_fence(__ATOMIC_ACQUIRE, "wavefront");                          \
  }
  double est_acc = 0.0, nrm_acc = 0.0;
  double *dump = d.lin_dump + (size_t)((blockIdx.x & 63) * 4 + wv) * 4;
  int sb = 0, st_b0 = 0;
  const int ls_ = lane / nlwb, lli = lane - ls_ * nlwb;
  const int sli = lane / 3, slc = lane - sli * 3;
#define BSG_STEP(R, L, TAG)                                                         \
  {                                                                                 \
                                  \
    asm volatile("; k_backsub_update group step " TAG);                             \
                                   \
    ((double2 *)Wim)[lane] = R##0;                                                  \
    ((double2 *)Wim)[lane + 64] = R##1;                                             \
    ((double2 *)Wim)[lane + 128] = R##2;                                            \
    ((double2 *)Wim)[lane + 192] = R##3;                                            \
    if (!SLIM) {                                                                    \
      ((double2 *)Wim)[lane + 256] = R##4;                                          \
      ((double2 *)Wim)[lane + 320] = R##5;                                          \
    }                                                                               \
    Lm[sb * nlwb * 12 + lm_q[0]] = L##0;                                            \
    Lm[sb * nlwb * 12 + lm_q[1]] = L##1;                                            \
    Lm[sb * nlwb * 12 + lm_q[2]] = L##2;                                            \
    BSG_ISSUE(R, L, st + 2)                                                         \
    BSG_WAVE_SYNC()                                                                 \
    if (SLIM && lane_on) {                                                          \
       \
      const double2 *w2 = (const double2 *)(Wim + lane * kWSlim);                   \
      const double2 g01 = w2[0], g23 = w2[1], g45 = w2[2], w_ = w2[3];              \
      const double G_[6] = {g01.x, g01.y, g23.x, g23.y, g45.x, g45.y};              \
      const double *Xi_ = Lm + sb * nlwb * 12 + nlwb * 9 + ilw * 3;                 \
      double k_[9], x_[3];                                                          \
      pair_from_G(G_, w_.x, T, Xi_[0], Xi_[1], Xi_[2], k_, x_);                     \
      const double X0 = x_[0], X1 = x_[1], X2 = x_[2];                              \
      const double e0 = xj[0] + (xj[4] * X2 - xj[5] * X1);                          \
      const double e1 = xj[1] + (xj[5] * X0 - xj[3] * X2);                          \
      const double e2 = xj[2] + (xj[3] * X1 - xj[4] * X0);                          \
      double *u = Us + lane * 3;                                                    \
      u[0] = fma(k_[6], e2, fma(k_[3], e1, k_[0] * e0));                            \
      u[1] = fma(k_[7], e2, fma(k_[4], e1, k_[1] * e0));                            \
      u[2] = fma(k_[8], e2, fma(k_[5], e1, k_[2] * e0));                            \
    }                                                                               \
    if (!SLIM && lane_on) {                                                         \
                   \
      const double2 *w2 = (const double2 *)(Wim + lane * kWStride);                 \
      const double2 k01 = w2[0], k23 = w2[1], k45 = w2[2], k67 = w2[3], k8x = w2[4], xx = w2[5]; \
      const double X0 = k8x.y, X1 = xx.x, X2 = xx.y;                                \
      const double e0 = xj[0] + (xj[4] * X2 - xj[5] * X1);                          \
      const double e1 = xj[1] + (xj[5] * X0 - xj[3] * X2);                          \
      const double e2 = xj[2] + (xj[3] * X1 - xj[4] * X0);                          \
      double *u = Us + lane * 3;                                                    \
      u[0] = fma(k67.x, e2, fma(k23.y, e1, k01.x * e0));                            \
      u[1] = fma(k67.y, e2, fma(k45.x, e1, k01.y * e0));                            \
      u[2] = fma(k8x.x, e2, fma(k45.y, e1, k23.x * e0));                            \
    }                                                                               \
    BSG_WAVE_SYNC()                                                                 \
         \
    if (lane < nlwb * 3) {                                                          \
      const double *u = Us + sli * dd * 3 + slc;                                    \
      double bx_ = 0.0;                                                             \
      for (int q_ = 0; q_ < dd; ++q_) bx_ += u[q_ * 3];                             \
      Bx[(sb * nlwb + sli) * 3 + slc] = bx_;                                        \
    }                                                                               \
    BSG_WAVE_SYNC()                                                                 \
     \
     \
     \
     \
    const bool do_lm_ = (sb + 1 == S) || (st + 1 >= nstep);                         \
    double y0 = 0.0, y1 = 0.0, y2 = 0.0, xn0 = 0.0, xn1 = 0.0, xn2 = 0.0;           \
    bool lm_on_ = false;                                                            \
    size_t i_ = 0;                                                                  \
    if (do_lm_) {                                                                   \
      const int il_ = il0_of(st_b0 + ls_) + lli;                                    \
      lm_on_ = ls_ <= sb && il_ < nl;                                               \
      i_ = (size_t)l0 + il_;                                                        \
      const double *lmp = Lm + ls_ * nlwb * 12;                                     \
      double C[6], bi[3], Xi[3];                                                    \
      _Pragma("unroll") for (int e_ = 0; e_ < 6; ++e_) C[e_] = lmp[lli * 6 + e_];   \
      _Pragma("unroll") for (int e_ = 0; e_ < 3; ++e_) bi[e_] = lmp[nlwb * 6 + lli * 3 + e_]; \
      _Pragma("unroll") for (int e_ = 0; e_ < 3; ++e_) Xi[e_] = lmp[nlwb * 9 + lli * 3 + e_]; \
      const double bx0 = Bx[lane * 3], bx1 = Bx[lane * 3 + 1], bx2 = Bx[lane * 3 + 2]; \
      double ci[6];                                                                 \
      {                                                                             \
        const double cdm[6] = {C[0] * lp1, C[1], C[2], C[3] * lp1, C[4], C[5] * lp1}; \
        spd3_inverse(cdm, ci);                                                      \
      }                                                                             \
      const double cb0 = ci[0] * bi[0] + ci[1] * bi[1] + ci[2] * bi[2];             \
      const double cb1 = ci[1] * bi[0] + ci[3] * bi[1] + ci[4] * bi[2];             \
      const double cb2 = ci[2] * bi[0] + ci[4] * bi[1] + ci[5] * bi[2];             \
      y0 = cb0 - (ci[0] * bx0 + ci[1] * bx1 + ci[2] * bx2);                         \
      y1 = cb1 - (ci[1] * bx0 + ci[3] * bx1 + ci[4] * bx2);                         \
      y2 = cb2 - (ci[2] * bx0 + ci[4] * bx1 + ci[5] * bx2);                         \
      xn0 = Xi[0] + y0;                                                             \
      xn1 = Xi[1] + y1;                                                             \
      xn2 = Xi[2] + y2;                                                             \
            \
      const double C0 = C[0] * lp1, C3 = C[3] * lp1, C5 = C[5] * lp1;               \
      double e = bi[0] * y0 + bi[1] * y1 + bi[2] * y2;                              \
      const double r0 = y0 * C0 + y1 * C[1] + y2 * C[2];                            \
      const double r1 = y0 * C[1] + y1 * C3 + y2 * C[4];                            \
      const double r2 = y0 * C[2] + y1 * C[4] + y2 * C5;                            \
      e += r0 * y0 + r1 * y1 + r2 * y2;                                             \
      e += 2.0 * (y0 * bx0 + y1 * bx1 + y2 * bx2);                                  \
      est_acc += lm_on_ ? e : 0.0;                                                  \
      nrm_acc += lm_on_ ? sqrt(y0 * y0 + y1 * y1 + y2 * y2) : 0.0;                  \
    }                                                                               \
    {                                                                               \
      double *yo = lm_on_ ? d.y + i_ * 3 : dump;                                    \
      yo[0] = y0; yo[1] = y1; yo[2] = y2;                                           \
      double *Xo = lm_on_ ? Xt + i_ * 3 : dump;                                     \
      Xo[0] = xn0; Xo[1] = xn1; Xo[2] = xn2;                                        \
    }                                                                               \
    if (do_lm_) {                                                                   \
      sb = 0;                                                                       \
      st_b0 = st + 1;                                                               \
    } else {                                                                        \
      ++sb;                                                                         \
    }                                                                               \
    BSG_WAVE_SYNC()                                                                 \
  }
  BSG_ISSUE(rwA, lmA, 0)
  BSG_ISSUE(rwB, lmB, 1)
  int st = 0;
  while (st < nstep) {
    BSG_STEP(rwA, lmA, "A")
    if (++st >= nstep) break;
    BSG_STEP(rwB, lmB, "B")
    ++st;
  }
#undef BSG_STEP
#undef BSG_ISSUE
#undef BSG_WAVE_SYNC
  block_sum2(est_acc, nrm_acc, sm);
  if (tid == 0) {
    d.lm_part[2 * part + 0] = est_acc;
    d.lm_part[2 * part + 1] = nrm_acc;
  }
}

template <bool GROUPS, bool SLIM>
__global__ __launch_bounds__(kBlock, GROUPS ? 2 : 4) void k_backsub_update(DevProblem d) {
  __shared__ __attribute__((aligned(16))) double lds[GROUPS ? kBsLds : kSchurPairs * (kWStride + 6 + 3)];
  __shared__ double sm[8];
  __shared__ int recs[kBsChunks * 8];
  if (blockIdx.x < kPoseGrid) {
    if (d.ctrl->done) return;
    pose_update_body(d, blockIdx.x, sm);
    return;
  }
  const int part = blockIdx.x - kPoseGrid;
  if (part >= d.n_lm_part) {
    if (d.ctrl->done) return;
    const int z = part - d.n_lm_part;
    const int I = d.zt_I[z], J = d.zt_J[z], nb = d.nb;
    for (int e = threadIdx.x; e < nb * nb; e += kBlock) {
      const int c = J * nb + e / nb, r = I * nb + e % nb;
      d.L[(size_t)c * d.ld + r] = (r == c && d.col_x[c] < 0) ? 1.0 : 0.0;
    }
    return;
  }
  if (GROUPS && part < d.n_bs_grp)
    backsub_grp_body<SLIM>(d, part, part, lds, sm);
  else
    backsub_chunk_body(d, part - d.n_bs_grp, part, lds, sm, recs);
}

#ifdef BA_BS_DBG
extern "C" int ba_debug_read_bs(long long *out) {
  return (int)hipMemcpyFromSymbol(out, HIP_SYMBOL(g_bs_dbg), sizeof(long long) * 96);
}
#endif

__device__ void control_step(const DevProblem &d);
__device__ void control_step_vals(const DevProblem &d, double current_cost, double model_est, double sum_y, double sum_x);

constexpr int kScalBlock = 1024;
__global__ __launch_bounds__(kScalBlock) void k_scalars(DevProblem d, int mode, int cost_src, int fin_sel) {
  if (blockIdx.x > 0) {
    pose_finalize_body(d, fin_sel, (blockIdx.x - 1) * kScalBlock + threadIdx.x);
    return;
  }
  if (d.ctrl->done) return;
  double c = 0.0, e = 0.0, n = 0.0, pe = 0.0, pn = 0.0;
  if (cost_src == 0 || d.n_obs_lm < d.n_obs) {
    static_assert(kCostGrid <= 2 * kScalBlock, "two loads per thread");
    const int k1 = threadIdx.x + kScalBlock;
    const double c0 = d.cost_part[threadIdx.x < kCostGrid ? threadIdx.x : 0];
    const double c1 = d.cost_part[k1 < kCostGrid ? k1 : 0];
    c = (threadIdx.x < kCostGrid ? c0 : 0.0) + (k1 < kCostGrid ? c1 : 0.0);
  }
  if (cost_src == 1) {
    const double *lp = d.lin_cost_part;
    for (int k0 = threadIdx.x; k0 < d.n_lin_cost; k0 += 8 * kScalBlock) {
      double v[8];
#pragma unroll
      for (int u = 0; u < 8; ++u) {
        const int k = k0 + u * kScalBlock;
        v[u] = k < d.n_lin_cost ? lp[k] : 0.0;
      }
#pragma unroll
      for (int u = 0; u < 8; ++u) c += v[u];
    }
  }
  if (mode >= 1) {
    const double2 *lp = (const double2 *)d.lm_part;
    const int n_lp = d.n_lm_part;
    for (int k0 = threadIdx.x; k0 < n_lp; k0 += 8 * kScalBlock) {
      double2 v[8];
#pragma unroll
      for (int u = 0; u < 8; ++u) {
        const int k = k0 + u * kScalBlock;
        v[u] = k < n_lp ? lp[k] : make_double2(0.0, 0.0);
      }
#pragma unroll
      for (int u = 0; u < 8; ++u) {
        e += v[u].x;
        n += v[u].y;
      }
    }
    if (threadIdx.x < kPoseGrid) {
      pe = d.pose_part[2 + 2 * threadIdx.x + 0];
      pn = d.pose_part[2 + 2 * threadIdx.x + 1];
    }
  }
  __shared__ double sm5[5][kScalBlock / 64];
  {
    const double w0 = wave_sum(c), w1 = wave_sum(e), w2 = wave_sum(n), w3 = wave_sum(pe),
                 w4 = wave_sum(pn);
    const int lane = threadIdx.x & 63, wv = threadIdx.x >> 6;
    if (lane == 0) {
      sm5[0][wv] = w0;
      sm5[1][wv] = w1;
      sm5[2][wv] = w2;
      sm5[3][wv] = w3;
      sm5[4][wv] = w4;
    }
  }
  __syncthreads();
  double tc = 0.0, te = 0.0, tn = 0.0, tpe = 0.0, tpn = 0.0;
  if (threadIdx.x == 0) {
    for (int w = 0; w < kScalBlock / 64; ++w) {
      tc += sm5[0][w];
      te += sm5[1][w];
      tn += sm5[2][w];
      tpe += sm5[3][w];
      tpn += sm5[4][w];
    }
// ... 240 lines not shown
  DevCtrl *ctl = d.ctrl;
  if (ctl->done) return;
  double c = 0.0, sp = 0.0, sq = 0.0;
  for (int k = threadIdx.x; k < gd.n_cost_part; k += kGdCtrlBlock) c += gd.cost_part[k];
  if (mode == 1)
    for (int k = threadIdx.x; k < gd.n_upd_blk; k += kGdCtrlBlock) {
      sp += gd.step_part[2 * k + 0];
      sq += gd.step_part[2 * k + 1];
    }
  __shared__ double sm3[3][kGdCtrlBlock / 64];
  {
    const double w0 = wave_sum(c), w1 = wave_sum(sp), w2 = wave_sum(sq);
    const int lane = threadIdx.x & 63, wv = threadIdx.x >> 6;
    if (lane == 0) {
      sm3[0][wv] = w0;
      sm3[1][wv] = w1;
      sm3[2][wv] = w2;
    }
  }
  __syncthreads();
  if (threadIdx.x != 0) return;
  double cost = 0.0, sum_a = 0.0, sum_b = 0.0;
  for (int w = 0; w < kGdCtrlBlock / 64; ++w) {
    cost += sm3[0][w];
    sum_a += sm3[1][w];
    sum_b += sm3[2][w];
  }
  const unsigned long long now = wall_clock64();
  if (mode == 0) {
    ctl->prev_cost = cost;
    ctl->t_last = now;
    return;
  }
  const double previous_cost = ctl->prev_cost;
  const double n_obs = (double)d.n_obs_global;
  const double cost_change = fabs(cost - previous_cost);
  const double step_pose = 0.01 + sum_a, step_point = 0.01 + sum_b;
  const double avg_step = (step_point + step_pose) / (double)(d.N + d.M_global);
  bool conv = (avg_step < ctl->thr_step) || (cost_change < ctl->thr_cost);
  if (ctl->iter >= ctl->max_iter - 1) conv = false;
  if (ctl->iter < d.log_cap) {
    DevIterRec &I = d.log[ctl->iter];
    I.cost = cost;
    I.cost_change = cost_change;
    I.average_reprojection_error = cost / n_obs;
    I.abs_gradient = 0.0;
    I.abs_step = avg_step;
    I.damping_term = ctl->lambda;
    I.iter_time_ms = (double)(now - ctl->t_last) * 1e-5;
    I.iteration_status = 0;
    I.pad_ = 0;
    I.rho = 0.0;
    I.model_change = 0.0;
    I.trial_cost = cost;
  }
  ctl->t_last = now;
  ctl->prev_cost = cost;
  ctl->iter += 1;
  ctl->converged = conv ? 1 : 0;
  if (conv || ctl->iter >= ctl->max_iter) ctl->done = 1;
}

inline int cdiv(int64_t a, int64_t b) { return (int)((a + b - 1) / b); }

}

void launch_cost(const DevProblem &d, int sel, int64_t begin, hipStream_t s) {
  if (begin >= d.n_obs) return;
  const bool lds = d.n_cam <= kCamLds, slim = d.obs_cp != nullptr;
  if (lds && slim) {
    BA_LAUNCH(K_COST, (k_cost<true, true>), dim3(kCostGrid), dim3(kBlock), s, d, sel, begin);
  } else if (lds) {
    BA_LAUNCH(K_COST, (k_cost<true, false>), dim3(kCostGrid), dim3(kBlock), s, d, sel, begin);
  } else if (slim) {
    BA_LAUNCH(K_COST, (k_cost<false, true>), dim3(kCostGrid), dim3(kBlock), s, d, sel, begin);
  } else {
    BA_LAUNCH(K_COST, (k_cost<false, false>), dim3(kCostGrid), dim3(kBlock), s, d, sel, begin);
  }
}

void launch_lin_landmarks(const DevProblem &d, int sel, hipStream_t s) {
  if (d.lin_chunk0 > 0) {
    const int n_plain = d.n_lin_plain, n_mask = d.n_lin_desc - d.n_lin_plain;
#define BA_LIN_GRP_LAUNCH(LDS, SLIM)                                                                                  \
  {                                                                                                                   \
    if (n_plain > 0) BA_LAUNCH(K_LIN_GRP, (k_lin_grp<LDS, false, SLIM>), dim3(n_plain), dim3(kBlock), s, d, sel, 0);   \
    if (n_mask > 0) BA_LAUNCH(K_LIN_GRP, (k_lin_grp<LDS, true, SLIM>), dim3(n_mask), dim3(kBlock), s, d, sel, n_plain); \
  }
    if (d.n_cam <= kCamLds) {
      if (d.pair_slim) BA_LIN_GRP_LAUNCH(true, true) else BA_LIN_GRP_LAUNCH(true, false)
    } else {
      if (d.pair_slim) BA_LIN_GRP_LAUNCH(false, true) else BA_LIN_GRP_LAUNCH(false, false)
    }
#undef BA_LIN_GRP_LAUNCH
  }
  const int nch = d.n_bchunk - d.lin_chunk0;
  if (nch <= 0) return;
  if (d.n_cam <= kCamLds)
    BA_LAUNCH(K_LIN_LANDMARKS, k_lin_landmarks<true>, dim3(nch), dim3(kBlock), s, d, sel);
  else
    BA_LAUNCH(K_LIN_LANDMARKS, k_lin_landmarks<false>, dim3(nch), dim3(kBlock), s, d, sel);
}

void launch_lin_poses(const DevProblem &d, int sel, hipStream_t s) {
  if (d.n_achunk > 0) {
    if (d.n_cam <= kCamLds)
      BA_LAUNCH(K_LIN_POSES, k_lin_poses<true>, dim3(cdiv(d.n_achunk, kBlock / 64)), dim3(kBlock), s, d, sel);
    else
      BA_LAUNCH(K_LIN_POSES, k_lin_poses<false>, dim3(cdiv(d.n_achunk, kBlock / 64)), dim3(kBlock), s, d, sel);
  }
  if (d.N > 0)
    BA_LAUNCH(K_POSE_FINALIZE, k_pose_finalize, dim3(cdiv((int64_t)d.N * 27, kBlock)), dim3(kBlock), s, d, sel);
}

void launch_damp_invert(const DevProblem &d, hipStream_t s) {
  if (d.M > 0 && (d.n_sup > 0 || d.n_tchunk > 0))
    BA_LAUNCH(K_DAMP_INVERT, k_damp_invert, dim3(cdiv(d.M, kBlock)), dim3(kBlock), s, d, 0);
}
void launch_damp_invert_export(const DevProblem &d, hipStream_t s) {
  if (d.M > 0)
    hipLaunchKernelGGL(k_damp_invert, dim3(cdiv(d.M, kBlock)), dim3(kBlock), 0, s, d, 1);
}

#ifdef BA_LL_DBG
extern "C" int ba_debug_read_ll(long long *out) {
  return (int)hipMemcpyFromSymbol(out, HIP_SYMBOL(g_ll_dbg), sizeof(long long) * 32);
}
#endif
#ifdef BA_LG_DBG
extern "C" int ba_debug_read_lg(long long *out) {
  return (int)hipMemcpyFromSymbol(out, HIP_SYMBOL(g_lg_dbg), sizeof(long long) * 64);
}
#endif
#ifdef BA_GRP_DBG
extern "C" int ba_debug_read_grp(long long *out) {
  return (int)hipMemcpyFromSymbol(out, HIP_SYMBOL(g_grp_dbg), sizeof(long long) * 256);
}
#endif
#ifdef BA_SCHUR_DBG
extern "C" int ba_debug_read(long long *out) {
  return (int)hipMemcpyFromSymbol(out, HIP_SYMBOL(g_schur_dbg), sizeof(long long) * 4 * 160);
}
#endif
void launch_schur_accumulate(const DevProblem &d, hipStream_t s) {
  if (d.pair_slim) {
    if (d.n_grp32 > 0)
      BA_LAUNCH(K_SCHUR_GRP, (k_schur_grp<2, true>), dim3(d.n_grp32), dim3(kBlock), s, d, d.grp32);
    if (d.n_grp64 > 0)
      BA_LAUNCH(K_SCHUR_GRP, (k_schur_grp<4, true>), dim3(d.n_grp64), dim3(kBlock), s, d, d.grp64);
    if (d.n_grp128 > 0)
      BA_LAUNCH(K_SCHUR_GRP, k_schur_grp_wide<true>, dim3(d.n_grp128), dim3(kBlock), s, d, d.grp128);
  } else {
    if (d.n_grp32 > 0)
      BA_LAUNCH(K_SCHUR_GRP, (k_schur_grp<2, false>), dim3(d.n_grp32), dim3(kBlock), s, d, d.grp32);
    if (d.n_grp64 > 0)
      BA_LAUNCH(K_SCHUR_GRP, (k_schur_grp<4, false>), dim3(d.n_grp64), dim3(kBlock), s, d, d.grp64);
    if (d.n_grp128 > 0)
      BA_LAUNCH(K_SCHUR_GRP, k_schur_grp_wide<false>, dim3(d.n_grp128), dim3(kBlock), s, d, d.grp128);
  }
  if (d.n_sup > 0)
    BA_LAUNCH(K_SCHUR_LDS, k_schur_lds, dim3(d.n_sup), dim3(kBlock), s, d);
  if (d.n_tchunk > 0)
    BA_LAUNCH(K_SCHUR_PARTIAL, k_schur_partial, dim3(d.n_tchunk), dim3(64), s, d);
}

void launch_schur_final(const DevProblem &d, bool direct, hipStream_t s) {
  if (d.B <= 0) return;
  if (direct)
    BA_LAUNCH(K_SCHUR_FINAL, k_schur_final_direct, dim3((unsigned)d.B), dim3(kBlock), s, d);
  else
    BA_LAUNCH(K_SCHUR_FINAL, k_schur_final, dim3((unsigned)d.B), dim3(kBlock), s, d);
}

void launch_schur(const DevProblem &d, bool direct, bool with_init, hipStream_t s) {
  if (with_init)
    launch_dense_init(d.L, d.ld, d.col_x, d.zt_I, d.zt_J, d.n_zt, d.nb, &d.ctrl->done, s);
  launch_schur_accumulate(d, s);
  launch_schur_final(d, direct, s);
}

void launch_scatter(const DevProblem &d, hipStream_t s) {
  const int64_t n = d.B * 36 + 6 * (int64_t)d.N;
  if (n > 0)
    BA_LAUNCH(K_SCATTER, k_scatter, dim3(cdiv(n, kBlock)), dim3(kBlock), s, d);
}

void launch_backsub_update(const DevProblem &d, hipStream_t s, bool zero_tiles) {
  const dim3 grid(kPoseGrid + d.n_lm_part + (zero_tiles ? d.n_zt : 0));
  if (d.n_bs_grp > 0 && d.pair_slim)
    BA_LAUNCH(K_BACKSUB_UPDATE, (k_backsub_update<true, true>), grid, dim3(kBlock), s, d);
  else if (d.n_bs_grp > 0)
    BA_LAUNCH(K_BACKSUB_UPDATE, (k_backsub_update<true, false>), grid, dim3(kBlock), s, d);
  else
    BA_LAUNCH(K_BACKSUB_UPDATE, (k_backsub_update<false, false>), grid, dim3(kBlock), s, d);
}

void launch_scalars(const DevProblem &d, int cost_src, hipStream_t s) {
  BA_LAUNCH(K_SCALARS, k_scalars, dim3(1), dim3(kScalBlock), s, d, 1, cost_src, -1);
}

void launch_scalars_and_control(const DevProblem &d, int cost_src, hipStream_t s, int finalize_sel) {
  const int nfin = finalize_sel >= 0 ? cdiv((int64_t)d.N * 27, kScalBlock) : 0;
  BA_LAUNCH(K_SCALARS, k_scalars, dim3(1 + nfin), dim3(kScalBlock), s, d, 2, cost_src, finalize_sel);
}

void launch_control(const DevProblem &d, hipStream_t s) {
  BA_LAUNCH(K_CONTROL, k_control, dim3(1), dim3(64), s, d);
}

void launch_init_ctrl_cost(const DevProblem &d, hipStream_t s) {
  BA_LAUNCH(K_CONTROL, k_init_ctrl_cost, dim3(1), dim3(64), s, d);
}

void launch_scalars_cost_only(const DevProblem &d, int cost_src, hipStream_t s) {
  BA_LAUNCH(K_SCALARS, k_scalars, dim3(1), dim3(kScalBlock), s, d, 0, cost_src, -1);
}

void launch_gd_pass(const DevProblem &d, const GdDev &g, hipStream_t s) {
  const bool lds = d.n_cam <= kCamLds;
  const int nb = d.n_bchunk + g.n_fix_blk;
  if (nb > 0) {
    if (lds)
      hipLaunchKernelGGL(k_gd_points<true>, dim3(nb), dim3(kBlock), 0, s, d, g);
    else
      hipLaunchKernelGGL(k_gd_points<false>, dim3(nb), dim3(kBlock), 0, s, d, g);
  }
  if (g.n_chunk > 0) {
    const dim3 grid(cdiv(g.n_chunk, kBlock / 64));
    if (lds)
      hipLaunchKernelGGL(k_gd_poses<true>, grid, dim3(kBlock), 0, s, d, g);
    else
      hipLaunchKernelGGL(k_gd_poses<false>, grid, dim3(kBlock), 0, s, d, g);
  }
}

void launch_gd_control(const DevProblem &d, const GdDev &g, int mode, hipStream_t s) {
  hipLaunchKernelGGL(k_gd_control, dim3(1 + cdiv((int64_t)d.N * 6, kGdCtrlBlock)), dim3(kGdCtrlBlock), 0, s, d, g,
                     mode);
}

void launch_gd_update(const DevProblem &d, const GdDev &g, hipStream_t s) {
  if (g.n_upd_blk > 0) hipLaunchKernelGGL(k_gd_update, dim3(g.n_upd_blk), dim3(kBlock), 0, s, d, g);
}

}
```

bundle_adjustment_solver_amd/csrc/ba_knobs.h:

```cpp
#ifndef BA_KNOBS_H_
#define BA_KNOBS_H_

#include <algorithm>
#include <cstdlib>

#include "ba_dense_sched.h"

namespace ba {

struct PlanKnobs {
  bool groups = true;
  bool lin_groups = true;
  bool superset = true;
  bool interleave = true;
  bool split = true;
  int sup_cap = 0;
  int lin_steps = 0;
  int threads = 0;
  bool stats = false;
  bool times = false;
};

struct RunKnobs {
  bool force_side = false;
  bool overlap = true;
  bool graph = false;
  bool cost_wide = false;
  int cov_batch = 0;
  bool stream_sync = false;
};

struct LayoutKnobs {
  bool pair_slim = true;
};

struct Knobs {
  PlanKnobs plan;
  DenseKnobs dense;
  ConeKnobs cone;
  RunKnobs run;
  LayoutKnobs layout;
  static Knobs from_env();
};

inline Knobs Knobs::from_env() {
  auto is_one = [](const char *name) { const char *v = getenv(name); return v && v[0] == '1'; };
  auto is_set = [](const char *name) { return getenv(name) != nullptr; };
  auto number = [](const char *name, long long lo, long long hi) {
    const char *v = getenv(name);
    return v ? (int)std::max(lo, std::min(hi, atoll(v))) : 0;
  };
  Knobs k;
  k.plan.groups = !is_one("BA_NO_GROUPS");
  k.plan.lin_groups = !is_one("BA_NO_LINGRP");
  k.plan.superset = !is_one("BA_NO_SUPERSET");
  k.plan.interleave = !is_one("BA_NO_INTERLEAVE");
  k.plan.split = !is_one("BA_NO_SPLIT");
  k.plan.sup_cap = number("BA_SUP_CAP", 1, 1 << 30);
  k.plan.lin_steps = number("BA_LIN_STEPS", 1, 1 << 30);
  k.plan.threads = number("BA_PLAN_THREADS", 1, 16);
  k.plan.stats = is_set("BA_PLAN_STATS");
  k.plan.times = is_set("BA_PLAN_TIMES");
  k.dense = DenseKnobs::from_env();
  k.cone = ConeKnobs::from_env();
  k.run.force_side = is_one("BA_FORCE_SIDE");
  k.run.overlap = !is_one("BA_NO_OVERLAP");
  k.run.graph = is_one("BA_GRAPH");
  k.run.cost_wide = is_one("BA_COST_WIDE");
  k.run.cov_batch = number("BA_COV_BATCH", 1, 1 << 30);
  k.run.stream_sync = is_one("BA_STREAM_SYNC");
  {
    const char *v = getenv("BA_PAIR_SLIM");
    k.layout.pair_slim = !(v && v[0] == '0');
  }
  return k;
}

}
#endif
```

bundle_adjustment_solver_amd/solver.py:

```python
import ctypes as C
import enum
import sys
import time

import numpy as np

from . import _lib
from ._lib import (BaIterInfo, BaOptions, BaPointResult, BaPoIter, BaPoResult,
                   check)

SCALER = 0.01
INVERSE_SCALER = 1.0 / SCALER


class SolverType(enum.IntEnum):
    UNDEFINED = -1
    GRADIENT_DESCENT = 0
    GAUSS_NEWTON = 1
    LEVENBERG_MARQUARDT = 2


class IterationStatus(enum.IntEnum):
    UNDEFINED = -1
    UPDATE = 0
# ... 470 lines not shown
        return out

    def get_points(self, into=None):
        out = np.zeros((self.n_pt, 3)) if into is None else into
        mask = np.zeros(self.n_pt, np.uint8)
        check(self.lib.ba_get_points(self.h, _dp(out), _up(mask)),
              "ba_get_points")
        return out, mask.astype(bool)

    def get_A(self):
        A = np.zeros((self.N, 6, 6))
        a = np.zeros((self.N, 6))
        check(self.lib.ba_get_A(self.h, _dp(A), _dp(a)), "ba_get_A")
        return A, a

    def get_C(self):
        Cm = np.zeros((self.M_global, 3, 3))
        b = np.zeros((self.M_global, 3))
        check(self.lib.ba_get_C(self.h, _dp(Cm), _dp(b)), "ba_get_C")
        return Cm, b

    def get_Cinv(self):
        Ci = np.zeros((self.M_global, 3, 3))
        cb = np.zeros((self.M_global, 3))
        check(self.lib.ba_get_Cinv(self.h, _dp(Ci), _dp(cb)), "ba_get_Cinv")
        return Ci, cb

    def get_pairs(self):
        P = int(self.P)
        pi = np.zeros(P, np.int32)
        pj = np.zeros(P, np.int32)
        W = np.zeros((P, 6, 3))
        check(self.lib.ba_get_pairs(self.h, _ip(pi), _ip(pj), _dp(W)),
              "ba_get_pairs")
        return pi, pj, W

    def get_S(self):
        n6 = 6 * self.N
        S = np.zeros((n6, n6))
        rhs = np.zeros(n6)
        check(self.lib.ba_get_S(self.h, _dp(S), _dp(rhs)), "ba_get_S")
        return S, rhs

    def get_xy(self):
        x = np.zeros((self.N, 6))
        y = np.zeros((self.M_global, 3))
        check(self.lib.ba_get_xy(self.h, _dp(x), _dp(y)), "ba_get_xy")
        return x, y

    def get_kernel_ms(self, reset=True):
        n = self.lib.ba_kernel_count()
        ms = np.zeros(n)
        calls = np.zeros(n, np.int64)
        check(self.lib.ba_get_kernel_ms(
            self.h, _dp(ms), calls.ctypes.data_as(C.POINTER(C.c_int64)),
            int(reset)), "ba_get_kernel_ms")
        return {self.lib.ba_kernel_name(k).decode(): (float(ms[k]), int(calls[k]))
                for k in range(n)}

    def get_dense_info(self):
        out = np.zeros(4)
        check(self.lib.ba_get_dense_info(self.h, _dp(out)),
              "ba_get_dense_info")
        return dict(fill=out[0], flops=out[1], levels=int(out[2]),
                    npad=int(out[3]))

    def get_schur_info(self):
        v = (C.c_int64 * 8)()
        check(self.lib.ba_get_schur_info(self.h, v), "ba_get_schur_info")
        return dict(groups32=int(v[0]), groups64=int(v[1]), grouped_landmarks=int(v[2]),
                    super_runs=int(v[3]), grouped_pairs=int(v[4]), grouped_triples=int(v[5]),
                    group_mfma=int(v[6]), list_triples=int(v[7]))

    def get_lin_info(self):
        v = (C.c_int64 * 4)()
        check(self.lib.ba_get_lin_info(self.h, v), "ba_get_lin_info")
        return dict(group_pieces=int(v[0]), group_observations=int(v[1]), chunks=int(v[2]),
                    pose_major_observations=int(v[3]))

    def get_pair_record_info(self):
        v = (C.c_int64 * 2)()
        check(self.lib.ba_get_pair_record_info(self.h, v), "ba_get_pair_record_info")
        return dict(slim_pairs=int(v[0]), pairs=int(v[1]))

    def get_mask_info(self):
        v = (C.c_int64 * 4)()
        check(self.lib.ba_get_mask_info(self.h, v), "ba_get_mask_info")
        return dict(masked_pieces=int(v[0]), masked_landmarks=int(v[1]),
                    padded_observation_slots=int(v[2]), padded_pairs=int(v[3]))

    def get_dropped_pivots(self, reset=False):
        v = C.c_int64(0)
        check(self.lib.ba_get_dropped_pivots(self.h, C.byref(v), int(reset)),
              "ba_get_dropped_pivots")
        return int(v.value)

    def covariance(self, pose_sel, pt_sel, huber):
        ps = np.ascontiguousarray(pose_sel, np.int32).reshape(-1)
        qs = np.ascontiguousarray(pt_sel, np.int32).reshape(-1)
        cp = np.zeros((ps.size, 6, 6))
        cq = np.zeros((qs.size, 3, 3))
        dropped = C.c_int64(0)
        check(self.lib.ba_covariance(self.h, float(huber), ps.size, _ip(ps) if ps.size else None,
                                     _dp(cp) if ps.size else None, qs.size,
                                     _ip(qs) if qs.size else None, _dp(cq) if qs.size else None,
                                     C.byref(dropped)), "ba_covariance")
        return cp, cq, int(dropped.value)

    def covariance_info(self):
        v = (C.c_int64 * 4)()
        check(self.lib.ba_covariance_info(self.h, v), "ba_covariance_info")
        return dict(batch_cols=int(v[0]), cols_per_wave=int(v[1]), workspace_bytes=int(v[2]),
                    last_batches=int(v[3]))

    def dense_spd_solve(self, A, b):
        A = np.ascontiguousarray(A, np.float64)
        b = np.ascontiguousarray(b, np.float64)
        n = A.shape[0]
        x = np.zeros(n)
        ms = C.c_double(0)
        check(self.lib.ba_dense_spd_solve(self.h, n, _dp(A), _dp(b), _dp(x),
                                          C.byref(ms)), "ba_dense_spd_solve")
        return x, ms.value

    def pose_only_mono6(self, X3, uv2, fx, fy, cx, cy, T12, mask, opt,
                        cap=None, want_debug=False):
        X = np.ascontiguousarray(X3, np.float32).reshape(-1, 3)
        uv = np.ascontiguousarray(uv2, np.float32).reshape(-1, 2)
        n = X.shape[0]
        T = np.ascontiguousarray(T12, np.float32).reshape(12).copy()
        m = np.ascontiguousarray(mask, np.uint8).copy()
        cap = cap or max(1, opt.max_num_iterations)
        rows = (BaPoIter * cap)()
        n_it = C.c_int(0)
        conv = C.c_int(0)
        dbg = np.zeros((cap, 12), np.float32) if want_debug else None
        rc = check(self.lib.ba_pose_only_mono6(
            self.h, _fp(X), _fp(uv), n, fx, fy, cx, cy, _fp(T), _up(m),
            C.byref(opt), rows, cap, C.byref(n_it), C.byref(conv),
            _fp(dbg) if want_debug else None), "ba_pose_only_mono6")
        nrows = n_it.value - 1 if conv.value else n_it.value
        nrows = max(0, min(nrows, cap))
        return dict(T12=T, mask=m.astype(bool), n_iter=n_it.value,
                    converged=bool(conv.value), success=(rc == 0),
                    rows=[(rows[i].cost, rows[i].cost_change,
                           rows[i].abs_step) for i in range(nrows)],
                    debug=dbg[:min(n_it.value, cap)] if want_debug else None)


    def pose_only_stereo6(self, X3, uvl2, uvr2, intr_l, intr_r, T_lr12, T12,
                          mask_l, mask_r, opt, cap=None, want_debug=False):
        X = np.ascontiguousarray(X3, np.float32).reshape(-1, 3)
        ul = np.ascontiguousarray(uvl2, np.float32).reshape(-1, 2)
        ur = np.ascontiguousarray(uvr2, np.float32).reshape(-1, 2)
        if ul.shape[0] != X.shape[0] or ur.shape[0] != X.shape[0]:
            raise RuntimeError(
                "In PoseOnlyBundleAdjustmentSolver::"
                "SolveStereoPoseOnlyBundleAdjustment6Dof(), "
                "world_position_list.size() != current_pixel_list.size()")
        n = X.shape[0]
        il = np.ascontiguousarray(intr_l, np.float32).reshape(4)
        ir = np.ascontiguousarray(intr_r, np.float32).reshape(4)
        Tlr = np.ascontiguousarray(T_lr12, np.float32).reshape(12)
        T = np.ascontiguousarray(T12, np.float32).reshape(12).copy()
        ml = np.ascontiguousarray(mask_l, np.uint8).copy()
        mr = np.ascontiguousarray(mask_r, np.uint8).copy()
# ... 1944 lines not shown
```

include/ba_hip.h:

```cpp
#ifndef BA_HIP_H_
#define BA_HIP_H_

#include <stdint.h>

#ifdef __cplusplus
extern "C" {
#endif

typedef struct ba_handle ba_handle;

typedef struct {
  float threshold_step_size;
  float threshold_cost_change;
  float threshold_huber_loss;
  float threshold_outlier_rejection;
  int max_num_iterations;
  float initial_lambda;
  float decrease_ratio_lambda;
  float increase_ratio_lambda;
  int gauss_newton;
} ba_options;

typedef struct {
  double cost;
// ... 34 lines not shown
int ba_update_relative(ba_handle *h, const double *Z12, const double *Omega36);
int ba_relative_check(int n_pose, const uint8_t *pose_fixed, int64_t n_rel, const int32_t *rel_j,
                      const int32_t *rel_k, const double *Z12, const double *Omega36);
int ba_relative_info(ba_handle *h, int64_t out4[4]);

int ba_partition_points(int n_pose, const uint8_t *pose_fixed, int n_pt,
                        const uint8_t *pt_fixed, int64_t n_obs,
                        const int32_t *obs_pose, const int32_t *obs_pt,
                        int world, int32_t *owner_out);

typedef int (*ba_allreduce_fn)(void *user, int which, void *dev_ptr,
                               int64_t n_doubles, void *hip_stream);
int ba_set_allreduce(ba_handle *h, ba_allreduce_fn fn, void *user);
int64_t ba_reduce_buffer_size(ba_handle *h, int which);
int ba_bind_reduce_buffer(ba_handle *h, int which, void *dev_ptr,
                          int64_t n_doubles);

int ba_gather_points(ba_handle *h);

typedef struct ba_rccl_comm ba_rccl_comm;
int ba_rccl_available(void);
int ba_rccl_get_unique_id(uint8_t id128[128]);
int ba_rccl_comm_create(ba_rccl_comm **out, int rank, int world,
                        const uint8_t id128[128], int device_id);
int ba_rccl_comm_size(ba_rccl_comm *c);
int64_t ba_rccl_comm_calls(ba_rccl_comm *c);
void ba_rccl_comm_destroy(ba_rccl_comm *c);
int ba_rccl_allreduce_hook(void *user, int which, void *dev_ptr,
                           int64_t n_doubles, void *hip_stream);

int ba_solve(ba_handle *h, const ba_options *opt, ba_iter_info *out, int cap,
             int *n_iter, int *converged);
int ba_lm_begin(ba_handle *h, const ba_options *opt);
int ba_lm_iterate(ba_handle *h, int n);
int ba_lm_sync(ba_handle *h, ba_iter_info *out, int cap, int *n_iter,
               int *converged);

int ba_gd_begin(ba_handle *h, const ba_options *opt);
int ba_gd_iterate(ba_handle *h, int n);
int ba_gd_sync(ba_handle *h, ba_iter_info *out, int cap, int *n_iter,
               int *converged);
int ba_solve_gd(ba_handle *h, const ba_options *opt, ba_iter_info *out,
                int cap, int *n_iter, int *converged);
int ba_gd_get_gradient(ba_handle *h, double *a6, double *b3);

int ba_stage_cost(ba_handle *h, double *cost);
int ba_stage_linearize(ba_handle *h, double lambda,
                       double huber);
int ba_stage_schur(ba_handle *h);
int ba_stage_solve_reduced(ba_handle *h);
int ba_stage_backsub_update(ba_handle *h);
int ba_stage_scalars(ba_handle *h, double *trial_cost, double *model_change,
                     double *pose_step_sum, double *point_step_sum);
int ba_stage_commit(ba_handle *h, int accept);

int ba_enable_stage_timing(ba_handle *h, int on);
int ba_get_stage_ms(ba_handle *h, double out8[8], int reset);

int ba_num_opt_poses(ba_handle *h);
int ba_num_opt_points(ba_handle *h);
int64_t ba_num_pairs(ba_handle *h);
int64_t ba_num_schur_blocks(ba_handle *h);
int64_t ba_num_schur_triples(ba_handle *h);
int ba_get_poses(ba_handle *h, double *T_jw12 );
int ba_get_points(ba_handle *h, double *X3 , uint8_t *owned_mask);
int ba_get_A(ba_handle *h, double *A36, double *a6);
int ba_get_C(ba_handle *h, double *C9, double *b3);
int ba_get_Cinv(ba_handle *h, double *Cinv9, double *Cinvb3);
int ba_get_pairs(ba_handle *h, int32_t *pair_i, int32_t *pair_j, double *W18);
void ba_expand_pair_slim(const double *rec8, const double *T12, const double *X3, double *k12);
int ba_get_S(ba_handle *h, double *S, double *rhs);
int ba_get_xy(ba_handle *h, double *x6, double *y3);

int ba_kernel_count(void);
const char *ba_kernel_name(int id);
int ba_get_kernel_ms(ba_handle *h, double *ms_out, int64_t *calls_out, int reset);

int ba_get_dense_info(ba_handle *h, double out4[4]);

int ba_get_schur_info(ba_handle *h, int64_t out8[8]);

int ba_get_lin_info(ba_handle *h, int64_t out4[4]);
int ba_get_pair_record_info(ba_handle *h, int64_t out2[2]);

int ba_get_mask_info(ba_handle *h, int64_t out4[4]);

int ba_get_dropped_pivots(ba_handle *h, int64_t *count, int reset);

typedef struct ba_stream ba_stream;
int ba_stream_create(ba_stream **out, int device_id, int n_chunks, int64_t arena_bytes);
void ba_stream_destroy(ba_stream *s);
int ba_stream_set_cameras(ba_stream *s, int n_cam, const double *intr4, const double *T_cj12);
int ba_stream_set_poses(ba_stream *s, int n_pose, const double *T_jw12, const uint8_t *fixed);
int ba_stream_set_points(ba_stream *s, int n_pt, const double *X3, const uint8_t *fixed);
int ba_stream_set_observations(ba_stream *s, int64_t n_obs, const int32_t *cam, const int32_t *pose,
                               const int32_t *point, const double *uv2);
int ba_stream_finalize(ba_stream *s);
int ba_stream_solve(ba_stream *s, const ba_options *opt, ba_iter_info *out, int cap,
                    int *n_iter, int *converged);
int ba_stream_lm_begin(ba_stream *s, const ba_options *opt);
int ba_stream_lm_iterate(ba_stream *s, int n);
int ba_stream_lm_sync(ba_stream *s, ba_iter_info *out, int cap, int *n_iter, int *converged);
int ba_stream_get_poses(ba_stream *s, double *T_jw12);
int ba_stream_get_points(ba_stream *s, double *X3);
int ba_stream_info(ba_stream *s, int64_t out6[6]);

int ba_dense_spd_solve(ba_handle *h, int n, const double *A, const double *b,
                       double *x, double *ms);

int ba_covariance(ba_handle *h, double huber,
                  int n_pose_sel, const int32_t *pose_sel, double *cov_pose36,
                  int n_pt_sel, const int32_t *pt_sel, double *cov_pt9,
                  int64_t *dropped_pivots);
int ba_covariance_info(ba_handle *h, int64_t out4[4]);
int ba_covariance_check(int finalized, int sharded, int streamed, int n_pose,
                        const uint8_t *pose_fixed, int n_pt, const uint8_t *pt_fixed,
                        int n_pose_sel, const int32_t *pose_sel, const double *cov_pose36,
                        int n_pt_sel, const int32_t *pt_sel, const double *cov_pt9);

typedef struct {
  float cost, cost_change, abs_step;
} ba_po_iter;
int ba_pose_only_mono6(ba_handle *h, const float *X3, const float *uv2, int n,
                       float fx, float fy, float cx, float cy, float *T12,
                       uint8_t *mask, const ba_options *opt, ba_po_iter *iters,
                       int cap, int *n_iter, int *converged,
                       float *debug_T12);

int ba_pose_only_stereo6(ba_handle *h, const float *X3, const float *uvl2,
                         const float *uvr2, int n, const float *intr_l4,
                         const float *intr_r4, const float *T_lr12, float *T12,
                         uint8_t *mask_l, uint8_t *mask_r, const ba_options *opt,
                         ba_po_iter *iters, int cap, int *n_iter, int *converged,
                         float *debug_T12);

int ba_pose_only_mono3(ba_handle *h, const float *X3, const float *uv2, int n,
                       float fx, float fy, float cx, float cy,
                       const float *T_bc12, const float *T_wl12, float *T12,
                       uint8_t *mask, const ba_options *opt, ba_po_iter *iters,
                       int cap, int *n_iter, int *converged,
                       float *debug_T12);
int ba_pose_only_stereo3(ba_handle *h, const float *X3, const float *uvl2,
                         const float *uvr2, int n, const float *intr_l4,
                         const float *intr_r4, const float *T_bc12,
                         const float *T_lr12, const float *T_wl12, float *T12,
                         uint8_t *mask_l, uint8_t *mask_r, const ba_options *opt,
                         ba_po_iter *iters, int cap, int *n_iter, int *converged,
                         float *debug_T12);

typedef struct {
  int n_iter, converged, n_rows, status;
} ba_po_result;
int ba_pose_only_mono6_batch(ba_handle *h, int B, const int32_t *offsets,
                             const float *X3, const float *uv2,
                             const float *intr4, float *T12, uint8_t *mask,
                             const ba_options *opt, ba_po_iter *iters, int cap,
                             ba_po_result *res, float *debug_T12);
int ba_pose_only_stereo6_batch(ba_handle *h, int B, const int32_t *offsets,
                               const float *X3, const float *uvl2,
                               const float *uvr2, const float *intr_l4,
                               const float *intr_r4, const float *T_lr12,
                               float *T12, uint8_t *mask_l, uint8_t *mask_r,
                               const ba_options *opt, ba_po_iter *iters,
                               int cap, ba_po_result *res, float *debug_T12);
int ba_pose_only_mono6_batch_device(ba_handle *h, int B, const int32_t *offsets,
                                    const float *X3, const float *uv2,
// ... 150 lines not shown
```

Measured before the change: 2472 it/s.

## Recompute slim pair records from observations instead of storing them

```diff
diff --git a/bundle_adjustment_solver_amd/_lib.py b/bundle_adjustment_solver_amd/_lib.py
--- a/bundle_adjustment_solver_amd/_lib.py
+++ b/bundle_adjustment_solver_amd/_lib.py
@@ -181,6 +181,9 @@
     "ba_get_schur_info": (C.c_int, [_P, C.POINTER(C.c_int64)]),
     "ba_get_lin_info": (C.c_int, [_P, C.POINTER(C.c_int64)]),
     "ba_get_pair_record_info": (C.c_int, [_P, C.POINTER(C.c_int64)]),
+    "ba_get_pair_form": (C.c_int, [_P]),
+    "ba_get_slim_records": (C.c_int, [_P, _I32, _I32, _I32, _D, _D]),
+    "ba_pair_G_from_obs": (None, [_D, _D, _D, _D, C.c_double, _D]),
     "ba_get_mask_info": (C.c_int, [_P, C.POINTER(C.c_int64)]),
     "ba_get_dropped_pivots": (C.c_int, [_P, C.POINTER(C.c_int64), C.c_int]),
     "ba_dense_spd_solve": (C.c_int, [_P, C.c_int, _D, _D, _D, _D]),
diff --git a/bundle_adjustment_solver_amd/csrc/ba_api.hip b/bundle_adjustment_solver_amd/csrc/ba_api.hip
--- a/bundle_adjustment_solver_amd/csrc/ba_api.hip
+++ b/bundle_adjustment_solver_amd/csrc/ba_api.hip
@@ -323,6 +323,61 @@
   return 0;
 }
 
+int choose_pair_obs(ba_handle *h) {
+  const ba::Plan &pl = h->plan;
+  ba::DevProblem &d = h->d;
+  d.pair_obs = 0;
+  if (!d.pair_slim || !h->knobs.layout.pair_obs || h->arena || !pl.grp64.empty() || !pl.grp128.empty() ||
+      pl.n_lin_plain != (int)pl.lin_desc.size() || pl.grp32.empty())
+    return 0;
+  std::vector<ba::PairObs> lin_obs(pl.lin_desc.size()), grp_obs(pl.grp32.size());
+  std::vector<int> by_l0(pl.lin_desc.size());
+  for (size_t k = 0; k < pl.lin_desc.size(); ++k) {
+    const auto &g = pl.lin_desc[k];
+    if (g.d > ba::kPairObsPoses || g.no > 255) return 0;
+    ba::PairObs &po = lin_obs[k];
+    po.o0 = g.o0;
+    po.no = g.no;
+    for (int jj = 0; jj < ba::kPairObsPoses; ++jj) po.sc[jj] = -1;
+    for (int oo = 0; oo < g.no; ++oo) {
+      const int y = pl.grp_pat[2 * ((size_t)g.pat0 + oo) + 1];
+      if (!((y >> 30) & 1)) continue;
+      const int jj = (y >> 16) & 0xff;
+      if (jj >= g.d) return 0;
+      po.sc[jj] = oo | (y & 0xffff) << 8;
+    }
+    for (int jj = 0; jj < ba::kPairObsPoses; ++jj) {
+      if (jj < g.d && po.sc[jj] < 0) return 0;
+      if (jj >= g.d) po.sc[jj] = 0;
+    }
+    by_l0[k] = (int)k;
+  }
+  std::sort(by_l0.begin(), by_l0.end(), [&](int a, int b) { return pl.lin_desc[a].l0 < pl.lin_desc[b].l0; });
+  auto piece_of = [&](int l) {
+    auto it = std::upper_bound(by_l0.begin(), by_l0.end(), l, [&](int v, int k) { return v < pl.lin_desc[k].l0; });
+    if (it == by_l0.begin()) return -1;
+    const int k = *(it - 1);
+    return l < pl.lin_desc[k].l0 + pl.lin_desc[k].nl ? k : -1;
+  };
+  for (size_t k = 0; k < pl.grp32.size(); ++k) {
+    const auto &g = pl.grp32[k];
+    const int ka = piece_of(g.l0), kb = piece_of(g.l0 + g.nl - 1);
+    if (ka < 0 || kb < 0) return 0;
+    const auto &a = pl.lin_desc[ka], &b = pl.lin_desc[kb];
+    if (a.pat0 != b.pat0 || a.d != g.d || a.no != b.no || g.p0 != a.p0 + (int64_t)(g.l0 - a.l0) * a.d ||
+        b.o0 != a.o0 + (int64_t)(b.l0 - a.l0) * a.no)
+      return 0;
+    grp_obs[k] = lin_obs[ka];
+    grp_obs[k].o0 = a.o0 + (int64_t)(g.l0 - a.l0) * a.no;
+  }
+  static_assert(sizeof(ba::PairObs) == 32, "side array layout");
+  if (h->upload(Mem::ChunkConst, &d.lin_obs, lin_obs.data(), lin_obs.size()) ||
+      h->upload(Mem::ChunkConst, &d.grp_obs, grp_obs.data(), grp_obs.size()))
+    return -1;
+  d.pair_obs = 1;
+  return 0;
+}
+
 int upload_descriptors_and_groups(ba_handle *h) {
   const ba::Plan &pl = h->plan;
   ba::DevProblem &d = h->d;
@@ -346,6 +401,7 @@
   d.n_lin_cost = d.n_bchunk + d.n_lin_desc;
   d.pair_slim = h->knobs.layout.pair_slim && pl.lin_groups && d.n_lin_desc > 0 ? 1 : 0;
   d.P_slim = d.pair_slim ? pl.lm_pair_ptr[pl.M_grp] : 0;
+  if (choose_pair_obs(h)) return -1;
   if (h->upload(Mem::ChunkConst, &d.sup_desc, pl.sup_desc.data(), pl.sup_desc.size()) ||
       h->upload(Mem::ChunkConst, &d.chunk_desc, pl.chunk_desc.data(), pl.chunk_desc.size()) ||
       h->dalloc(Mem::ChunkState, &d.spart2, (size_t)d.n_slot * ba::kSlotStride) ||
@@ -1397,6 +1453,54 @@
   ba::pair_from_G(rec8, rec8[6], T12, X3[0], X3[1], X3[2], k12, k12 + 9);
 }
 
+void ba_pair_G_from_obs(const double *cam16, const double *T12, const double *X3, const double *uv2, double huber,
+                        double *rec8) {
+  ba::pair_G_from_obs(cam16, T12, X3[0], X3[1], X3[2], uv2[0], uv2[1], huber, rec8, rec8[6]);
+  rec8[7] = 0.0;
+}
+
+int ba_get_pair_form(ba_handle *h) {
+  if (!h || !h->finalized) return fail("ba_get_pair_form: not finalized");
+  return h->d.pair_obs ? 2 : (h->d.pair_slim ? 1 : 0);
+}
+
+int ba_get_slim_records(ba_handle *h, int32_t *pose, int32_t *lm, int32_t *cam, double *uv2, double *rec8) {
+  if (!h || !h->finalized) return fail("ba_get_slim_records: not finalized");
+  if (use_device(h)) return -1;
+  const ba::Plan &pl = h->plan;
+  const int64_t n = h->d.P_slim;
+  if (pull_ctrl(h)) return -1;
+  if (rec8 && n > 0) {
+    if (h->d.pair_obs) {
+      ba::launch_pair_records(h->d, h->stream);
+      HIP_TRY(hipStreamSynchronize(h->stream));
+    }
+    HIP_TRY(hipMemcpy(rec8, h->d.W[h->hc.lcur], (size_t)n * ba::kWSlim * sizeof(double), hipMemcpyDeviceToHost));
+  }
+  for (int64_t p = 0; p < n; ++p) {
+    if (pose) pose[p] = pl.pose_user_of_int[pl.pair_pose[p]];
+    if (lm) lm[p] = pl.pt_user_of_int[pl.pair_lm[p]];
+  }
+  if (cam || uv2) {
+    for (const auto &g : pl.lin_desc)
+      for (int oo = 0; oo < g.no; ++oo) {
+        const int y = pl.grp_pat[2 * ((size_t)g.pat0 + oo) + 1];
+        if (!((y >> 30) & 1)) continue;
+        const int jj = (y >> 16) & 0xff;
+        for (int il = 0; il < g.nl; ++il) {
+          const int64_t p = g.p0 + (int64_t)il * g.d + jj, o = g.o0 + (int64_t)il * g.no + oo;
+          if (p >= n) continue;
+          if (cam) cam[p] = y & 0xffff;
+          if (uv2) {
+            uv2[2 * p] = pl.obs_uv[2 * o];
+            uv2[2 * p + 1] = pl.obs_uv[2 * o + 1];
+          }
+        }
+      }
+  }
+  return 0;
+}
+
 int ba_get_pairs(ba_handle *h, int32_t *pair_i, int32_t *pair_j, double *W18) {
   if (!h || !h->finalized) return fail("ba_get_pairs: not finalized");
   if (use_device(h)) return -1;
@@ -1414,6 +1518,10 @@
   if (W18) {
     if (pull_ctrl(h)) return -1;
     std::vector<double> w12((size_t)pl.P * ba::kWStride);
+    if (h->d.pair_obs) {
+      ba::launch_pair_records(h->d, h->stream);
+      HIP_TRY(hipStreamSynchronize(h->stream));
+    }
     if (pl.P > 0)
       HIP_TRY(hipMemcpy(w12.data(), h->d.W[h->hc.lcur], w12.size() * sizeof(double), hipMemcpyDeviceToHost));
     const int64_t P_slim = h->d.P_slim;
@@ -1774,6 +1882,7 @@
   HIP_TRY(hipMemcpy(&bad_keep, h->ddev.bad_pivots, sizeof(int), hipMemcpyDeviceToHost));
   HIP_TRY(hipMemsetAsync(h->ddev.bad_pivots, 0, sizeof(int), h->stream));
   enqueue_linearize(h, 0);
+  ba::launch_pair_records(d, h->stream);
   if (h->rel.F > 0) {
     ba::launch_rel_lin(d, h->rel, 0, 1, h->stream);
     ba::launch_rel_gather(d, h->rel, 0, 1, h->stream);
diff --git a/bundle_adjustment_solver_amd/csrc/ba_device.h b/bundle_adjustment_solver_amd/csrc/ba_device.h
--- a/bundle_adjustment_solver_amd/csrc/ba_device.h
+++ b/bundle_adjustment_solver_amd/csrc/ba_device.h
@@ -40,6 +40,12 @@
 
 constexpr int kWStride = 12;
 constexpr int kWSlim = 8;
+constexpr int kPairObsPoses = 5;
+struct PairObs {
+  int64_t o0;
+  int32_t no;
+  int32_t sc[kPairObsPoses];
+};
 
 struct DevProblem {
   int n_cam, n_pose, N, n_pt, M, M_global;
@@ -102,6 +108,8 @@
   int n_lm_part;
   int pair_slim;
   int64_t P_slim;
+  int pair_obs;
+  PairObs *lin_obs, *grp_obs;
   SupDesc *sup_desc;
   uint32_t *sup_lane;
   ChunkDesc *chunk_desc;
@@ -193,6 +201,7 @@
 void launch_lin_poses(const DevProblem &d, int sel, hipStream_t s);
 void launch_lin_landmarks(const DevProblem &d, int sel, hipStream_t s);
 void launch_damp_invert(const DevProblem &d, hipStream_t s);
+void launch_pair_records(const DevProblem &d, hipStream_t s);
 void launch_schur(const DevProblem &d, bool direct, bool with_init, hipStream_t s);
 void launch_schur_accumulate(const DevProblem &d, hipStream_t s);
 void launch_schur_final(const DevProblem &d, bool direct, hipStream_t s);
diff --git a/bundle_adjustment_solver_amd/csrc/ba_device_fn.h b/bundle_adjustment_solver_amd/csrc/ba_device_fn.h
--- a/bundle_adjustment_solver_amd/csrc/ba_device_fn.h
+++ b/bundle_adjustment_solver_amd/csrc/ba_device_fn.h
@@ -163,6 +163,34 @@
   for (int r = 0; r < 3; ++r)
 #pragma unroll
     for (int c = 0; c < 3; ++c) K[r * 3 + c] = fma(G[r], wR[c], G[3 + r] * wR[3 + c]);
+}
+
+__host__ __device__ __forceinline__ void pair_G_from_obs(const double *__restrict__ cam, const double *__restrict__ T,
+                                                         const double X0, const double X1, const double X2,
+                                                         const double u, const double v, const double huber,
+                                                         double G[6], double &w) {
+#pragma clang fp contract(off)
+  double Xij[3], Xc[3];
+#pragma unroll
+  for (int r = 0; r < 3; ++r)
+    Xij[r] = fma(T[r * 3 + 2], X2, fma(T[r * 3 + 0], X0, T[r * 3 + 1] * X1)) + T[9 + r];
+  const double *Rc = cam + 4;
+#pragma unroll
+  for (int r = 0; r < 3; ++r)
+    Xc[r] = fma(Rc[r * 3 + 2], Xij[2], fma(Rc[r * 3 + 0], Xij[0], Rc[r * 3 + 1] * Xij[1])) + cam[13 + r];
+  const double invz = 1.0 / Xc[2];
+  const double xinvz = Xc[0] * invz, yinvz = Xc[1] * invz;
+  const double r0 = fma(cam[0], xinvz, cam[2]) - u;
+  const double r1 = fma(cam[1], yinvz, cam[3]) - v;
+  const double absr = fabs(r0) + fabs(r1);
+  w = (absr > huber) ? (huber / absr) : 1.0;
+  const double fxinvz = cam[0] * invz, fyinvz = cam[1] * invz;
+  const double nx = -(fxinvz * xinvz), ny = -(fyinvz * yinvz);
+#pragma unroll
+  for (int c = 0; c < 3; ++c) {
+    G[c] = fma(fxinvz, Rc[c], nx * Rc[6 + c]);
+    G[3 + c] = fma(fyinvz, Rc[3 + c], ny * Rc[6 + c]);
+  }
 }
 
 __device__ __forceinline__ void ldlt3_inverse(const double c[6], double o[6]) {
diff --git a/bundle_adjustment_solver_amd/csrc/ba_kernels.hip b/bundle_adjustment_solver_amd/csrc/ba_kernels.hip
--- a/bundle_adjustment_solver_amd/csrc/ba_kernels.hip
+++ b/bundle_adjustment_solver_amd/csrc/ba_kernels.hip
@@ -336,11 +336,13 @@
 #else
 #define LG_STAMP()
 #endif
-template <bool SLIM>
-constexpr int kLgArea = 64 * 9 + 7 * 10 * (SLIM ? kWSlim : kWStride);
-template <bool LDSCAM, bool MASKED, bool SLIM>
+template <int REC>
+constexpr int kLgArea = REC == 2 ? 14 * 64 : 64 * 9 + 7 * 10 * (REC == 1 ? kWSlim : kWStride);
+template <bool LDSCAM, bool MASKED, int REC>
 __device__ __forceinline__ void lin_grp_body(const DevProblem &d, const int sel, const int bid, double *red,
                                              double *cams_s, double *smc, int *slot_b, int *slot_e) {
+  constexpr bool SLIM = REC == 1;
+  static_assert(REC != 2 || !MASKED, "a masked piece keeps its records");
 #ifdef BA_LG_DBG
   __shared__ long long lg_s[64];
   const bool lg_on = blockIdx.x == 300 && threadIdx.x == 0;
@@ -393,7 +395,7 @@
   double *__restrict__ Wg = d.W[lb];
   double *__restrict__ Cg = d.Cu[lb];
   double *__restrict__ bg = d.b[lb];
-  double *cbw = red + wv * kLgArea<SLIM>;
+  double *cbw = red + wv * kLgArea<REC>;
   double acc[27];
 #pragma unroll
   for (int k = 0; k < 27; ++k) acc[k] = 0.0;
@@ -423,7 +425,7 @@
   constexpr int RW = (SLIM ? kWSlim : kWStride) / 2;
   double2 *stgW = (double2 *)(cbw + 64 * 9);
   double2 *stgW_mine = stgW + (ilw * dd + jj) * RW;
-  constexpr int kLgPass = (7 * 10 * RW + 63) / 64;
+  constexpr int kLgPass = REC == 2 ? 1 : (7 * 10 * RW + 63) / 64;
   int il0p = nl;
   double vv[8];
   double2 wvv[kLgPass];
@@ -432,11 +434,13 @@
 #define LING_FLUSH_ISSUE()                                                          \
   {                                                                                 \
     _Pragma("unroll") for (int u_ = 0; u_ < 8; ++u_) vv[u_] = sum_p[(u_ < no ? u_ : 0) * 9]; \
-    const int nls_ = nl - il0p < nlw ? nl - il0p : nlw;                             \
-    const int n2_ = nls_ * dd * RW;                                                 \
-    dstWp = n2_ > 0 ? (double2 *)(Wg + (size_t)(p0 + (int64_t)il0p * dd) * (2 * RW)) : dumpW; \
-    lastp = n2_ > 0 ? n2_ - 1 : 0;                                                  \
-    _Pragma("unroll") for (int k_ = 0; k_ < kLgPass; ++k_) wvv[k_] = stgW[min(lane + 64 * k_, lastp)]; \
+    if (REC != 2) {                                                                 \
+      const int nls_ = nl - il0p < nlw ? nl - il0p : nlw;                           \
+      const int n2_ = nls_ * dd * RW;                                               \
+      dstWp = n2_ > 0 ? (double2 *)(Wg + (size_t)(p0 + (int64_t)il0p * dd) * (2 * RW)) : dumpW; \
+      lastp = n2_ > 0 ? n2_ - 1 : 0;                                                \
+      _Pragma("unroll") for (int k_ = 0; k_ < kLgPass; ++k_) wvv[k_] = stgW[min(lane + 64 * k_, lastp)]; \
+    }                                                                               \
   }
 #define LING_FLUSH_FINISH()                                                         \
   {                                                                                 \
@@ -446,7 +450,9 @@
     const int ils_ = il0p + sum_li;                                                 \
     double *dst_ = (sum_on && ils_ < nl) ? sum_g + (size_t)ils_ * sum_stride : dumpC; \
     *dst_ = sum_neg ? -sacc_ : sacc_;                                               \
-    _Pragma("unroll") for (int k_ = 0; k_ < kLgPass; ++k_) dstWp[min(lane + 64 * k_, lastp)] = wvv[k_]; \
+    if (REC != 2) {                                                                 \
+      _Pragma("unroll") for (int k_ = 0; k_ < kLgPass; ++k_) dstWp[min(lane + 64 * k_, lastp)] = wvv[k_]; \
+    }                                                                               \
   }
 #define LING_STEP(CUR, NXT2)                                                        \
   {                                                                                 \
@@ -497,7 +503,8 @@
        \
        \
        \
-      if (SLIM) {                                                                   \
+      if (REC == 2) {                                                               \
+      } else if (SLIM) {                                                            \
         _Pragma("unroll") for (int e_ = 0; e_ < 6; ++e_) kk[e_] = (!MASKED || valid_) ? G[e_] : 0.0; \
         kk[6] = w;                                                                  \
         kk[7] = 0.0;                                                                \
@@ -532,7 +539,7 @@
     {                                                                               \
       double *cb = cbw + lane * 9;                                                  \
       _Pragma("unroll") for (int e_ = 0; e_ < 9; ++e_) cb[e_] = cbv[e_];            \
-      if (wr_ && lane_on) {                                                         \
+      if (REC != 2 && wr_ && lane_on) {                                             \
         _Pragma("unroll") for (int r = 0; r < RW; ++r)                              \
           stgW_mine[r] = make_double2(kk[2 * r], kk[2 * r + 1]);                    \
       }                                                                             \
@@ -576,7 +583,7 @@
       double sacc = 0.0;
       for (int w4 = 0; w4 < 4; ++w4)
         for (int li = 0; li < nlw; ++li)
-          for (int q = sb; q < se; ++q) sacc += red[w4 * kLgArea<SLIM> + k * 64 + li * no + q];
+          for (int q = sb; q < se; ++q) sacc += red[w4 * kLgArea<REC> + k * 64 + li * no + q];
       d.Apart2[(size_t)(apart0 + pj) * 27 + e] = sacc;
     }
   }
@@ -586,13 +593,13 @@
 #endif
 }
 
-template <bool LDSCAM, bool MASKED, bool SLIM>
+template <bool LDSCAM, bool MASKED, int REC>
 __global__ __launch_bounds__(kBlock, 2) void k_lin_grp(DevProblem d, int sel, int piece0) {
-  __shared__ __attribute__((aligned(16))) double red[4 * kLgArea<SLIM>];
+  __shared__ __attribute__((aligned(16))) double red[4 * kLgArea<REC>];
   __shared__ double cams_s[kCamLds * 16];
   __shared__ double smc[4];
   __shared__ int slot_b[kGrpMaxPoses], slot_e[kGrpMaxPoses];
-  lin_grp_body<LDSCAM, MASKED, SLIM>(d, sel, piece0 + blockIdx.x, red, cams_s, smc, slot_b, slot_e);
+  lin_grp_body<LDSCAM, MASKED, REC>(d, sel, piece0 + blockIdx.x, red, cams_s, smc, slot_b, slot_e);
 }
 
 __global__ __launch_bounds__(kBlock) void k_damp_invert(DevProblem d, int store_cd) {
@@ -998,8 +1005,10 @@
 #else
 #define GRP_STAMP()
 #endif
-template <int NT, bool SLIM>
+template <int NT, int REC, bool LDSCAM = true>
 __global__ __launch_bounds__(kBlock, (NT == 2 && BA_GRP_KRW <= 24) ? 3 : 2) void k_schur_grp(DevProblem d, const DevProblem::GrpDesc *grps) {
+  constexpr bool OBS = REC == 2, SLIM = REC >= 1;
+  static_assert(!OBS || NT == 2, "from the observation: 32-wide groups only");
   constexpr int TW = 16 * NT;
 #ifndef BA_GRP_KRW
 #define BA_GRP_KRW 36
@@ -1011,6 +1020,7 @@
   __shared__ __attribute__((aligned(16))) double VA[4][IMG];
   __shared__ __attribute__((aligned(16))) double WB[4][IMG];
   static_assert(IMG >= 256, "the final reduction uses VA as 4 x 256 doubles");
+  __shared__ double cams_s[(OBS && LDSCAM) ? kCamLds * 16 : 1];
 #ifdef BA_GRP_DBG
   __shared__ long long gdbg_s[256];
   const bool gdbg_on = blockIdx.x == 600 && threadIdx.x == 0;
@@ -1038,7 +1048,7 @@
     wb[e] = 0.0;
   }
   constexpr int RD = (SLIM && NT == 4) ? 1 : 2;
-  constexpr int RW = (SLIM ? kWSlim : kWStride) / 2;
+  constexpr int RW = OBS ? 1 : (SLIM ? kWSlim : kWStride) / 2;
   double2 rw[2][6], rc[2][3];
   double rb[2][3], rx[2][3];
   double T[12];
@@ -1048,11 +1058,27 @@
 #pragma unroll
     for (int k = 0; k < 12; ++k) T[k] = Tp[k];
   }
+  const double2 *__restrict__ uvp = nullptr;
+  int ono = 0, ocam = 0;
+  double huber = 0.0;
+  if (OBS) {
+    const PairObs *po = d.grp_obs + blockIdx.x;
+    const int sc = po->sc[jj];
+    ono = po->no;
+    uvp = d.obs_uv + po->o0 + (sc & 0xff);
+    ocam = sc >> 8;
+    huber = d.ctrl->huber;
+    if (LDSCAM) {
+      stage_cams(d, cams_s);
+      __syncthreads();
+    }
+  }
 #define GRP_PREFETCH(B, ch_)                                                        \
   {                                                                                 \
     const int c0_ = (ch_) * nlw;                                                    \
     const bool on_ = il < min(nlw, gd.nl - c0_);                                    \
-    const double2 *wp_ = (const double2 *)(Wg + (size_t)(gd.p0 + (int64_t)c0_ * dd + (on_ ? lane : 0)) * (2 * RW)); \
+    const double2 *wp_ = OBS ? uvp + (int64_t)(c0_ + (on_ ? il : 0)) * ono          \
+                             : (const double2 *)(Wg + (size_t)(gd.p0 + (int64_t)c0_ * dd + (on_ ? lane : 0)) * (2 * RW)); \
     const int lm_ = gd.l0 + c0_ + (on_ ? il : 0);                                   \
     const double2 *cp_ = (const double2 *)(Cug + (size_t)lm_ * 6);                  \
     _Pragma("unroll") for (int k_ = 0; k_ < RW; ++k_) rw[B][k_] = wp_[k_];          \
@@ -1076,7 +1102,12 @@
        \
       _Pragma("clang fp contract(fast)")                                            \
       double k9[9], xij[3];                                                         \
-      if (SLIM) {                                                                   \
+      if (OBS) {                                                                    \
+        double cam_[16], G_[6], w_;                                                 \
+        load_cam<LDSCAM>(d, cams_s, ocam, cam_);                                    \
+        pair_G_from_obs(cam_, T, rx[B][0], rx[B][1], rx[B][2], rw[B][0].x, rw[B][0].y, huber, G_, w_); \
+        pair_from_G(G_, w_, T, rx[B][0], rx[B][1], rx[B][2], k9, xij);              \
+      } else if (SLIM) {                                                            \
         const double G_[6] = {rw[B][0].x, rw[B][0].y, rw[B][1].x, rw[B][1].y, rw[B][2].x, rw[B][2].y}; \
         pair_from_G(G_, rw[B][3].x, T, rx[B][0], rx[B][1], rx[B][2], k9, xij);      \
       } else {                                                                      \
@@ -1800,9 +1831,10 @@
 #endif
 }
 
-template <bool SLIM>
+template <int REC>
 __device__ __forceinline__ void backsub_grp_body(const DevProblem &d, const int piece, const int part, double *lds,
                                                  double *sm) {
+  constexpr bool OBS = REC == 2, SLIM = REC >= 1;
   const DevProblem::LinDesc *gp = d.lin_desc + piece;
   const int64_t p0 = gp->p0;
   const int l0 = gp->l0, nl = gp->nl, dd = gp->d;
@@ -1832,6 +1864,19 @@
 #pragma unroll
     for (int k = 0; k < 12; ++k) T[k] = Tp[k];
   }
+  const double2 *__restrict__ uvp = d.obs_uv;
+  int ono = 0;
+  double cam[16], huber = 0.0;
+  if (OBS) {
+    const PairObs *po = d.lin_obs + piece;
+    const int sc = po->sc[jj < kPairObsPoses ? jj : 0];
+    ono = po->no;
+    uvp = d.obs_uv + po->o0 + (sc & 0xff);
+    huber = d.ctrl->huber;
+    const double *cp = d.cams + (size_t)(sc >> 8) * 16;
+#pragma unroll
+    for (int k = 0; k < 16; ++k) cam[k] = cp[k];
+  }
   double *Wim = lds + wv * kBgArea;
   double *Us = Wim + 64 * 2 * RW;
   double *Lm = Us + 64 * 3;
@@ -1864,10 +1909,14 @@
     const int ilb_ = nls_ > 0 ? il0_ : 0;                                           \
     const int lml_ = max(0, nls_ - 1);                                              \
     const double2 *src_ = Wg2 + (dd > 0 ? (size_t)(p0 + (int64_t)ilb_ * dd) * RW : (size_t)0); \
-    R##0 = src_[min(lane, last_)];                                                  \
-    R##1 = src_[min(lane + 64, last_)];                                             \
-    R##2 = src_[min(lane + 128, last_)];                                            \
-    R##3 = src_[min(lane + 192, last_)];                                            \
+    if (OBS) {                                                                      \
+      R##0 = uvp[(int64_t)(ilb_ + min(ilw, lml_)) * ono];                           \
+    } else {                                                                        \
+      R##0 = src_[min(lane, last_)];                                                \
+      R##1 = src_[min(lane + 64, last_)];                                           \
+      R##2 = src_[min(lane + 128, last_)];                                          \
+      R##3 = src_[min(lane + 192, last_)];                                          \
+    }                                                                               \
     if (!SLIM) {                                                                    \
       R##4 = src_[min(lane + 256, last_)];                                          \
       R##5 = src_[min(lane + 320, last_)];                                          \
@@ -1892,10 +1941,13 @@
                                   \
     asm volatile("; k_backsub_update group step " TAG);                             \
                                    \
-    ((double2 *)Wim)[lane] = R##0;                                                  \
-    ((double2 *)Wim)[lane + 64] = R##1;                                             \
-    ((double2 *)Wim)[lane + 128] = R##2;                                            \
-    ((double2 *)Wim)[lane + 192] = R##3;                                            \
+    const double2 uv_ = R##0;                                                       \
+    if (!OBS) {                                                                     \
+      ((double2 *)Wim)[lane] = R##0;                                                \
+      ((double2 *)Wim)[lane + 64] = R##1;                                           \
+      ((double2 *)Wim)[lane + 128] = R##2;                                          \
+      ((double2 *)Wim)[lane + 192] = R##3;                                          \
+    }                                                                               \
     if (!SLIM) {                                                                    \
       ((double2 *)Wim)[lane + 256] = R##4;                                          \
       ((double2 *)Wim)[lane + 320] = R##5;                                          \
@@ -1907,12 +1959,17 @@
     BSG_WAVE_SYNC()                                                                 \
     if (SLIM && lane_on) {                                                          \
        \
-      const double2 *w2 = (const double2 *)(Wim + lane * kWSlim);                   \
-      const double2 g01 = w2[0], g23 = w2[1], g45 = w2[2], w_ = w2[3];              \
-      const double G_[6] = {g01.x, g01.y, g23.x, g23.y, g45.x, g45.y};              \
       const double *Xi_ = Lm + sb * nlwb * 12 + nlwb * 9 + ilw * 3;                 \
-      double k_[9], x_[3];                                                          \
-      pair_from_G(G_, w_.x, T, Xi_[0], Xi_[1], Xi_[2], k_, x_);                     \
+      double G_[6], gw_, k_[9], x_[3];                                              \
+      if (OBS) {                                                                    \
+        pair_G_from_obs(cam, T, Xi_[0], Xi_[1], Xi_[2], uv_.x, uv_.y, huber, G_, gw_); \
+      } else {                                                                      \
+        const double2 *w2 = (const double2 *)(Wim + lane * kWSlim);                 \
+        const double2 g01 = w2[0], g23 = w2[1], g45 = w2[2], w_ = w2[3];            \
+        G_[0] = g01.x; G_[1] = g01.y; G_[2] = g23.x; G_[3] = g23.y; G_[4] = g45.x; G_[5] = g45.y; \
+        gw_ = w_.x;                                                                 \
+      }                                                                             \
+      pair_from_G(G_, gw_, T, Xi_[0], Xi_[1], Xi_[2], k_, x_);                      \
       const double X0 = x_[0], X1 = x_[1], X2 = x_[2];                              \
       const double e0 = xj[0] + (xj[4] * X2 - xj[5] * X1);                          \
       const double e1 = xj[1] + (xj[5] * X0 - xj[3] * X2);                          \
@@ -2020,7 +2077,7 @@
   }
 }
 
-template <bool GROUPS, bool SLIM>
+template <bool GROUPS, int REC>
 __global__ __launch_bounds__(kBlock, GROUPS ? 2 : 4) void k_backsub_update(DevProblem d) {
   __shared__ __attribute__((aligned(16))) double lds[GROUPS ? kBsLds : kSchurPairs * (kWStride + 6 + 3)];
   __shared__ double sm[8];
@@ -2042,9 +2099,34 @@
     return;
   }
   if (GROUPS && part < d.n_bs_grp)
-    backsub_grp_body<SLIM>(d, part, part, lds, sm);
+    backsub_grp_body<REC>(d, part, part, lds, sm);
   else
     backsub_chunk_body(d, part - d.n_bs_grp, part, lds, sm, recs);
+}
+
+__global__ __launch_bounds__(kBlock) void k_pair_records(DevProblem d) {
+  const DevProblem::LinDesc *gp = d.lin_desc + blockIdx.x;
+  const PairObs *po = d.lin_obs + blockIdx.x;
+  const int dd = gp->d, np = gp->nl * dd;
+  const double huber = d.ctrl->huber;
+  const double *__restrict__ poses = d.poses[d.ctrl->cur];
+  const double *__restrict__ pts = d.pts[d.ctrl->cur];
+  double *__restrict__ Wg = d.W[d.ctrl->lcur];
+  for (int q = threadIdx.x; q < np; q += kBlock) {
+    const int il = q / dd, jj = q - il * dd;
+    const int sc = po->sc[jj];
+    const double2 uv = d.obs_uv[po->o0 + (int64_t)il * po->no + (sc & 0xff)];
+    const double *cam = d.cams + (size_t)(sc >> 8) * 16;
+    const double *T = poses + (size_t)d.pair_pose[gp->p0 + jj] * 12;
+    const double *X = pts + (size_t)(gp->l0 + il) * 3;
+    double G[6], w;
+    pair_G_from_obs(cam, T, X[0], X[1], X[2], uv.x, uv.y, huber, G, w);
+    double *o = Wg + (size_t)(gp->p0 + q) * kWSlim;
+#pragma unroll
+    for (int e = 0; e < 6; ++e) o[e] = G[e];
+    o[6] = w;
+    o[7] = 0.0;
+  }
 }
 
 #ifdef BA_BS_DBG
@@ -2451,15 +2533,17 @@
 void launch_lin_landmarks(const DevProblem &d, int sel, hipStream_t s) {
   if (d.lin_chunk0 > 0) {
     const int n_plain = d.n_lin_plain, n_mask = d.n_lin_desc - d.n_lin_plain;
-#define BA_LIN_GRP_LAUNCH(LDS, SLIM)                                                                                  \
+#define BA_LIN_GRP_LAUNCH(LDS, REC)                                                                                   \
   {                                                                                                                   \
-    if (n_plain > 0) BA_LAUNCH(K_LIN_GRP, (k_lin_grp<LDS, false, SLIM>), dim3(n_plain), dim3(kBlock), s, d, sel, 0);   \
-    if (n_mask > 0) BA_LAUNCH(K_LIN_GRP, (k_lin_grp<LDS, true, SLIM>), dim3(n_mask), dim3(kBlock), s, d, sel, n_plain); \
+    if (n_plain > 0) BA_LAUNCH(K_LIN_GRP, (k_lin_grp<LDS, false, REC>), dim3(n_plain), dim3(kBlock), s, d, sel, 0);    \
+    if (n_mask > 0) BA_LAUNCH(K_LIN_GRP, (k_lin_grp<LDS, true, REC>), dim3(n_mask), dim3(kBlock), s, d, sel, n_plain); \
   }
     if (d.n_cam <= kCamLds) {
-      if (d.pair_slim) BA_LIN_GRP_LAUNCH(true, true) else BA_LIN_GRP_LAUNCH(true, false)
+      if (d.pair_obs) BA_LAUNCH(K_LIN_GRP, (k_lin_grp<true, false, 2>), dim3(n_plain), dim3(kBlock), s, d, sel, 0);
+      else if (d.pair_slim) BA_LIN_GRP_LAUNCH(true, 1) else BA_LIN_GRP_LAUNCH(true, 0)
     } else {
-      if (d.pair_slim) BA_LIN_GRP_LAUNCH(false, true) else BA_LIN_GRP_LAUNCH(false, false)
+      if (d.pair_obs) BA_LAUNCH(K_LIN_GRP, (k_lin_grp<false, false, 2>), dim3(n_plain), dim3(kBlock), s, d, sel, 0);
+      else if (d.pair_slim) BA_LIN_GRP_LAUNCH(false, 1) else BA_LIN_GRP_LAUNCH(false, 0)
     }
 #undef BA_LIN_GRP_LAUNCH
   }
@@ -2486,6 +2570,9 @@
   if (d.M > 0 && (d.n_sup > 0 || d.n_tchunk > 0))
     BA_LAUNCH(K_DAMP_INVERT, k_damp_invert, dim3(cdiv(d.M, kBlock)), dim3(kBlock), s, d, 0);
 }
+void launch_pair_records(const DevProblem &d, hipStream_t s) {
+  if (d.pair_obs && d.n_lin_desc > 0) hipLaunchKernelGGL(k_pair_records, dim3(d.n_lin_desc), dim3(kBlock), 0, s, d);
+}
 void launch_damp_invert_export(const DevProblem &d, hipStream_t s) {
   if (d.M > 0)
     hipLaunchKernelGGL(k_damp_invert, dim3(cdiv(d.M, kBlock)), dim3(kBlock), 0, s, d, 1);
@@ -2512,18 +2599,23 @@
 }
 #endif
 void launch_schur_accumulate(const DevProblem &d, hipStream_t s) {
-  if (d.pair_slim) {
+  if (d.pair_obs) {
+    if (d.n_grp32 > 0 && d.n_cam <= kCamLds)
+      BA_LAUNCH(K_SCHUR_GRP, (k_schur_grp<2, 2, true>), dim3(d.n_grp32), dim3(kBlock), s, d, d.grp32);
+    else if (d.n_grp32 > 0)
+      BA_LAUNCH(K_SCHUR_GRP, (k_schur_grp<2, 2, false>), dim3(d.n_grp32), dim3(kBlock), s, d, d.grp32);
+  } else if (d.pair_slim) {
     if (d.n_grp32 > 0)
-      BA_LAUNCH(K_SCHUR_GRP, (k_schur_grp<2, true>), dim3(d.n_grp32), dim3(kBlock), s, d, d.grp32);
+      BA_LAUNCH(K_SCHUR_GRP, (k_schur_grp<2, 1>), dim3(d.n_grp32), dim3(kBlock), s, d, d.grp32);
     if (d.n_grp64 > 0)
-      BA_LAUNCH(K_SCHUR_GRP, (k_schur_grp<4, true>), dim3(d.n_grp64), dim3(kBlock), s, d, d.grp64);
+      BA_LAUNCH(K_SCHUR_GRP, (k_schur_grp<4, 1>), dim3(d.n_grp64), dim3(kBlock), s, d, d.grp64);
     if (d.n_grp128 > 0)
       BA_LAUNCH(K_SCHUR_GRP, k_schur_grp_wide<true>, dim3(d.n_grp128), dim3(kBlock), s, d, d.grp128);
   } else {
     if (d.n_grp32 > 0)
-      BA_LAUNCH(K_SCHUR_GRP, (k_schur_grp<2, false>), dim3(d.n_grp32), dim3(kBlock), s, d, d.grp32);
+      BA_LAUNCH(K_SCHUR_GRP, (k_schur_grp<2, 0>), dim3(d.n_grp32), dim3(kBlock), s, d, d.grp32);
     if (d.n_grp64 > 0)
-      BA_LAUNCH(K_SCHUR_GRP, (k_schur_grp<4, false>), dim3(d.n_grp64), dim3(kBlock), s, d, d.grp64);
+      BA_LAUNCH(K_SCHUR_GRP, (k_schur_grp<4, 0>), dim3(d.n_grp64), dim3(kBlock), s, d, d.grp64);
     if (d.n_grp128 > 0)
       BA_LAUNCH(K_SCHUR_GRP, k_schur_grp_wide<false>, dim3(d.n_grp128), dim3(kBlock), s, d, d.grp128);
   }
@@ -2556,12 +2648,14 @@
 
 void launch_backsub_update(const DevProblem &d, hipStream_t s, bool zero_tiles) {
   const dim3 grid(kPoseGrid + d.n_lm_part + (zero_tiles ? d.n_zt : 0));
-  if (d.n_bs_grp > 0 && d.pair_slim)
-    BA_LAUNCH(K_BACKSUB_UPDATE, (k_backsub_update<true, true>), grid, dim3(kBlock), s, d);
+  if (d.n_bs_grp > 0 && d.pair_obs)
+    BA_LAUNCH(K_BACKSUB_UPDATE, (k_backsub_update<true, 2>), grid, dim3(kBlock), s, d);
+  else if (d.n_bs_grp > 0 && d.pair_slim)
+    BA_LAUNCH(K_BACKSUB_UPDATE, (k_backsub_update<true, 1>), grid, dim3(kBlock), s, d);
   else if (d.n_bs_grp > 0)
-    BA_LAUNCH(K_BACKSUB_UPDATE, (k_backsub_update<true, false>), grid, dim3(kBlock), s, d);
+    BA_LAUNCH(K_BACKSUB_UPDATE, (k_backsub_update<true, 0>), grid, dim3(kBlock), s, d);
   else
-    BA_LAUNCH(K_BACKSUB_UPDATE, (k_backsub_update<false, false>), grid, dim3(kBlock), s, d);
+    BA_LAUNCH(K_BACKSUB_UPDATE, (k_backsub_update<false, 0>), grid, dim3(kBlock), s, d);
 }
 
 void launch_scalars(const DevProblem &d, int cost_src, hipStream_t s) {
diff --git a/bundle_adjustment_solver_amd/csrc/ba_knobs.h b/bundle_adjustment_solver_amd/csrc/ba_knobs.h
--- a/bundle_adjustment_solver_amd/csrc/ba_knobs.h
+++ b/bundle_adjustment_solver_amd/csrc/ba_knobs.h
@@ -32,6 +32,7 @@
 
 struct LayoutKnobs {
   bool pair_slim = true;
+  bool pair_obs = true;
 };
 
 struct Knobs {
@@ -72,6 +73,8 @@
   {
     const char *v = getenv("BA_PAIR_SLIM");
     k.layout.pair_slim = !(v && v[0] == '0');
+    const char *o = getenv("BA_PAIR_OBS");
+    k.layout.pair_obs = !(o && o[0] == '0');
   }
   return k;
 }
diff --git a/bundle_adjustment_solver_amd/solver.py b/bundle_adjustment_solver_amd/solver.py
--- a/bundle_adjustment_solver_amd/solver.py
+++ b/bundle_adjustment_solver_amd/solver.py
@@ -576,6 +576,20 @@
         v = (C.c_int64 * 2)()
         check(self.lib.ba_get_pair_record_info(self.h, v), "ba_get_pair_record_info")
         return dict(slim_pairs=int(v[0]), pairs=int(v[1]))
+
+    def get_pair_form(self):
+        f = self.lib.ba_get_pair_form(self.h)
+        if f < 0:
+            check(f, "ba_get_pair_form")
+        return int(f)
+
+    def get_slim_records(self):
+        n = self.get_pair_record_info()["slim_pairs"]
+        pose, lm, cam = (np.zeros(n, np.int32) for _ in range(3))
+        uv, rec = np.zeros((n, 2)), np.zeros((n, 8))
+        check(self.lib.ba_get_slim_records(self.h, _ip(pose), _ip(lm), _ip(cam), _dp(uv), _dp(rec)),
+              "ba_get_slim_records")
+        return dict(pose=pose, lm=lm, cam=cam, uv=uv, rec=rec)
 
     def get_mask_info(self):
         v = (C.c_int64 * 4)()
diff --git a/include/ba_hip.h b/include/ba_hip.h
--- a/include/ba_hip.h
+++ b/include/ba_hip.h
@@ -140,6 +140,10 @@
 
 int ba_get_lin_info(ba_handle *h, int64_t out4[4]);
 int ba_get_pair_record_info(ba_handle *h, int64_t out2[2]);
+int ba_get_pair_form(ba_handle *h);
+int ba_get_slim_records(ba_handle *h, int32_t *pose, int32_t *lm, int32_t *cam, double *uv2, double *rec8);
+void ba_pair_G_from_obs(const double *cam16, const double *T12, const double *X3, const double *uv2, double huber,
+                        double *rec8);
 
 int ba_get_mask_info(ba_handle *h, int64_t out4[4]);
 
```

Result: faster. 2685 it/s, median of 6 (+8.6%).
